# rsinghlab/GNN-Tumor-Seg

Hardware: AMD Instinct MI355X
Metric: supervoxel-graphs/sec training, 7xSAGE-pool-256, 15k-node graphs (higher is better)
Workload: dtype f32; 1 GPU; C2: 7xGraphSAGE-pool-256 (8 SAGEConv), fwd+weighted-CE+bwd+AdamW, 4 x 15000-node/86350-edge lattice graphs per GPU, 4-chan feat, fp32; global_batch=4, nodes_per_batch=60000, edges_per_batch=345400, parallelism=dp1

## Files before the change

### gnn-tumor-seg_amd/csrc/gts_gemm.hip

```cpp
#include "gts_gemm_tiles.h"
#include "gts_gemm_panel.h"
#include "gts_gemm_wgrad.h"
#include "gts_gemm_small.h"

namespace gts {
namespace {

template <bool AKC, bool BKC>
int pick_plain_variant(const GemmArgs& p) {
  int variant = BKC ? g_fwd_variant : g_igrad_variant;
  if (p.rb <= 128 && variant < 9) return 0;
  const bool row_count_invariant = variant == -2;
  if (variant < 0) {
    const int64_t cols = (p.rb + 255) / 256;
    const int64_t big_tiles = static_cast<int64_t>((p.ra + 255) / 256) * cols;
    variant = big_tiles >= 192 ? 8 : 3;
    if constexpr (AKC && BKC) {
      const int h = panel_rows_for(p.ra, cols);
      const int64_t panels = static_cast<int64_t>((p.ra + h - 1) / h) * cols;
      const int64_t rows256 = (big_tiles + 255) / 256 * 256, rows_panel = (panels + 255) / 256 * h;
      if (variant == 8 && rows_panel < rows256 && !row_count_invariant) variant = 10;
      if (variant == 3 && panels >= 192 && panels <= 256 && !row_count_invariant) variant = 10;
    }
  }
  return variant;
}

template <bool BKC>
inline bool skinny_forward(const GemmArgs& p) {
  const bool automatic = BKC ? g_fwd_variant < 0 : g_igrad_variant <= 1;
  return automatic && (p.rb == 4 || p.rb == 8) && p.ldc == p.rb && p.kseg[0] + p.kseg[1] >= 64 && p.mask == nullptr &&
         p.c2 == nullptr && p.sc_l == nullptr && p.bits_out == nullptr &&
         (BKC || (p.ldb[0] == p.rb && (p.kseg[1] == 0 || p.ldb[1] == p.rb)));
}

inline bool tiny_forward(const GemmArgs& p) {
  return (p.rb == 4 || p.rb == 8) && p.ldc == p.rb && p.kseg[0] + p.kseg[1] <= 16 && p.mask == nullptr && p.c2 == nullptr &&
         p.sc_l == nullptr && p.bits_out == nullptr && g_fwd_variant < 0;
}

template <bool AKC, bool BKC>
int launch_plain_tiles(const GemmArgs& p, int variant, hipStream_t st) {
  if constexpr (AKC && BKC) {
    if (tiny_forward(p)) {
      const unsigned blocks = static_cast<unsigned>((p.ra + 255) / 256);
      if (p.rb == 4) tiny_fwd_kernel<4><<<blocks, 256, 0, st>>>(p);
      else tiny_fwd_kernel<8><<<blocks, 256, 0, st>>>(p);
      return launch_status();
    }
  }
  if constexpr (AKC) {
    if (skinny_forward<BKC>(p)) {
      const unsigned blocks = static_cast<unsigned>((p.ra + 15) / 16);
      if (p.rb == 4) skinny_fwd_kernel<4, BKC><<<blocks, 256, 0, st>>>(p);
      else skinny_fwd_kernel<8, BKC><<<blocks, 256, 0, st>>>(p);
      return launch_status();
    }
  }
  if (p.rb <= 64) return launch_tiles<128, 64, 2, 2, AKC, BKC>(p, 1, 1, st);
  if (p.rb <= 128) return launch_tiles<128, 128, 2, 2, AKC, BKC>(p, 1, 1, st);
  switch (variant) {
    case 3: return launch_tiles<64, 256, 2, 4, AKC, BKC>(p, 1, 1, st);
    case 5: return launch_tiles<256, 128, 4, 2, AKC, BKC>(p, 1, 1, st);
    case 8: return launch_tiles<256, 256, 4, 4, AKC, BKC, true>(p, 1, 1, st);
    default: return launch_tiles<128, 256, 2, 4, AKC, BKC>(p, 1, 1, st);
  }
}

template <bool AKC, bool BKC>
int launch_plain(const GemmArgs& p, hipStream_t st) {
  const int variant = pick_plain_variant<AKC, BKC>(p);
  if constexpr (AKC && BKC) {
    if (p.c2 != nullptr && !(variant == 10 && p.rb <= kC240 && p.rb2 <= kC240 && p.rb2 > 128)) {
      GemmArgs first = p, next{};
      first.c2 = nullptr;
      int rc = launch_plain<true, true>(first, st);
      if (rc != GTS_OK) return rc;
      next.a[0] = next.a[1] = p.c, next.b[0] = next.b[1] = p.b2, next.bp[0] = p.bp2;
      first.bp2 = nullptr;
      next.lda[0] = next.lda[1] = p.ldc, next.ldb[0] = next.ldb[1] = p.ldb2;
      next.kseg[0] = p.rb, next.kseg[1] = 0;
      next.ra = p.ra, next.rb = p.rb2, next.c = p.c2, next.ldc = p.ldc2, next.bias = p.bias2, next.relu = p.relu2;
      next.tiles_per_split = (p.rb + kBK - 1) / kBK;
      return launch_plain<true, true>(next, st);
    }
    if (variant == 10) {
      switch (panel_rows_for(p.ra, (p.rb + kC240 - 1) / kC240)) {
        case 144: return launch_panel_direct<3, 4, 1, NoProbe, 144>(p, st);
        case 192: return launch_panel_direct<3, 4, 1, NoProbe, 192>(p, st);
        default: return launch_panel_direct<3, 4, 1>(p, st);
      }
    }
  }
  int rc = launch_plain_tiles<AKC, BKC>(p, variant, st);
  if (rc != GTS_OK || p.bits_out == nullptr) return rc;
  const long long words = static_cast<long long>((p.ra + 3) / 4) * (p.rb >> 6);
  relu_bits_kernel<<<static_cast<unsigned>((words + 3) / 4), 256, 0, st>>>(p.c, p.bits_out, p.ra, p.rb);
  return launch_status();
}

struct PlainProblem {
  const float *a0, *b0, *a1, *b1;
  float* c;
  int64_t m, rb, k0, k1;
  bool missing() const { return !a0 || !b0 || !c || ((a1 == nullptr) != (b1 == nullptr)); }
  bool bad_shape() const {
    return m < 0 || rb <= 0 || k0 <= 0 || k1 < 0 || m >= (1LL << 31) || rb >= (1 << 20) || k0 >= (1 << 20) || k1 >= (1 << 20) ||
           !aligned4(k0) || !aligned4(k1) || (a1 && k1 == 0);
  }
  GemmArgs args(int64_t ldb0, int64_t ldb1, const float* const* packed) const {
    GemmArgs p{};
    p.a[0] = a0, p.b[0] = b0, p.lda[0] = p.kseg[0] = static_cast<int>(k0), p.ldb[0] = static_cast<int>(ldb0);
    p.a[1] = a1 ? a1 : a0, p.b[1] = b1 ? b1 : b0, p.lda[1] = static_cast<int>(k1), p.ldb[1] = static_cast<int>(ldb1);
    p.kseg[1] = a1 ? static_cast<int>(k1) : 0;
    p.ra = static_cast<int>(m), p.rb = static_cast<int>(rb), p.c = c, p.ldc = static_cast<int>(rb);
    p.tiles_per_split = (p.kseg[0] + kBK - 1) / kBK + (p.kseg[1] + kBK - 1) / kBK;
    if (packed != nullptr) p.bp[0] = packed[0], p.bp[1] = a1 ? packed[1] : nullptr;
    return p;
  }
};

void chain_second(GemmArgs* p, const float* b2, const float* bias2, float* c2, int64_t rb2, int relu2,
                  const float* const* packed) {
  p->b2 = b2, p->bias2 = bias2, p->c2 = c2, p->rb2 = static_cast<int>(rb2), p->ldb2 = p->rb;
  p->ldc2 = static_cast<int>(rb2), p->relu2 = relu2;
  if (packed != nullptr) p->bp2 = packed[2];
}

__global__ __launch_bounds__(kBlock) void sum_parts_kernel(const float* __restrict__ in_l, const float* __restrict__ in_r,
                                                           float* __restrict__ out_l, float* __restrict__ out_r,
                                                           int64_t n, int parts) {
  const int64_t i = static_cast<int64_t>(blockIdx.x) * kBlock + threadIdx.x;
  if (i >= n) return;
  float sl = 0.f, sr = 0.f;
  for (int q = 0; q < parts; ++q) sl += in_l[i * parts + q], sr += in_r[i * parts + q];
  out_l[i] = sl, out_r[i] = sr;
}

}
}

extern "C" int32_t gts_linear_fwd_f32(const float* a0, const float* w0, const float* a1, const float* w1, const float* bias,
                                      float* out, int64_t m, int64_t n, int64_t k0, int64_t k1, int32_t relu,
                                      uint64_t* relu_bits, const float* const* packed, void* stream) {
  using namespace gts;
  const PlainProblem q{a0, w0, a1, w1, out, m, n, k0, k1};
  if (q.missing()) return GTS_ERR_NULL;
  if (q.bad_shape() || (relu_bits && n % 64 != 0)) return GTS_ERR_SHAPE;
  if (m == 0) return GTS_OK;
  GemmArgs p = q.args(k0, k1, packed);
  p.bias = bias, p.relu = relu, p.bits_out = reinterpret_cast<unsigned long long*>(relu_bits);
  return launch_plain<true, true>(p, static_cast<hipStream_t>(stream));
}

extern "C" int32_t gts_relu_bits_pay(int64_t m, int64_t n) {
  using namespace gts;
  if (m <= 0 || n <= 0 || n % 64 != 0 || m >= (1LL << 31) || n >= (1 << 20)) return 0;
  GemmArgs p{};
  p.ra = static_cast<int>(m), p.rb = static_cast<int>(n);
  const int variant = pick_plain_variant<true, true>(p);
  return variant >= 10 && variant <= 12 ? 1 : 0;
}

extern "C" int64_t gts_relu_bits_bytes(int64_t m, int64_t n) {
  if (m < 0 || n <= 0 || n % 64 != 0) return 0;
  return (m + 3) / 4 * (n / 64) * 4 * static_cast<int64_t>(sizeof(uint64_t));
}

extern "C" int64_t gts_gat_fc_scores_workspace(int64_t m, int64_t heads, int64_t dim) {
  if (m <= 0 || heads <= 0 || dim <= 0 || dim % 64 != 0) return 0;
  return 2 * m * heads * (dim / 64) * static_cast<int64_t>(sizeof(float));
}

extern "C" int32_t gts_gat_fc_scores_f32(const float* h, const float* w_fc, const float* attn_l, const float* attn_r,
                                         float* ft, float* el, float* er, float* workspace, int64_t workspace_bytes,
                                         int64_t m, int64_t heads, int64_t dim, int64_t k, const float* w_fc_packed,
                                         void* stream) {
  using namespace gts;
  const int64_t n = heads * dim;
  const float* const packed[2] = {w_fc_packed, nullptr};
  const PlainProblem q{h, w_fc, nullptr, nullptr, ft, m, n, k, 0};
  if (q.missing() || !attn_l || !attn_r || !el || !er) return GTS_ERR_NULL;
  if (q.bad_shape() || heads <= 0 || dim <= 0) return GTS_ERR_SHAPE;
  if (m == 0) return GTS_OK;
  GemmArgs p = q.args(k, 0, packed);
  hipStream_t st = static_cast<hipStream_t>(stream);
  const int parts = static_cast<int>(dim / 64);
  const bool fuse = dim % 64 == 0 && pick_plain_variant<true, true>(p) == 10 &&
                    (parts == 1 || (workspace && workspace_bytes >= gts_gat_fc_scores_workspace(m, heads, dim)));
  if (!fuse) {
    const int rc = launch_plain<true, true>(p, st);
    return rc != GTS_OK ? rc : gts_gat_scores_f32(ft, attn_l, attn_r, el, er, m, heads, dim, stream);
  }
  p.sc_l = attn_l, p.sc_r = attn_r;
  p.sc_el = parts == 1 ? el : workspace, p.sc_er = parts == 1 ? er : workspace + m * heads * parts;
  const int rc = launch_plain<true, true>(p, st);
  if (rc != GTS_OK || parts == 1) return rc;
  const int64_t rows = m * heads;
  sum_parts_kernel<<<static_cast<unsigned>((rows + kBlock - 1) / kBlock), kBlock, 0, st>>>(p.sc_el, p.sc_er, el, er, rows, parts);
  return launch_status();
}

extern "C" int32_t gts_linear_fwd_chain_f32(const float* a0, const float* w0, const float* a1, const float* w1,
                                            const float* bias, float* out, const float* w2, const float* bias2, float* out2,
                                            int64_t m, int64_t n, int64_t k0, int64_t k1, int32_t relu, int64_t n2,
                                            int32_t relu2, uint64_t* relu_bits, const float* const* packed, void* stream) {
  using namespace gts;
  const PlainProblem q{a0, w0, a1, w1, out, m, n, k0, k1};
  if (q.missing() || !w2 || !out2) return GTS_ERR_NULL;
  if (q.bad_shape() || n2 <= 0 || n2 >= (1 << 20) || !aligned4(n) || (relu_bits && n % 64 != 0)) return GTS_ERR_SHAPE;
  if (m == 0) return GTS_OK;
  GemmArgs p = q.args(k0, k1, packed);
  p.bias = bias, p.relu = relu, p.bits_out = reinterpret_cast<unsigned long long*>(relu_bits);
  chain_second(&p, w2, bias2, out2, n2, relu2, packed);
  return launch_plain<true, true>(p, static_cast<hipStream_t>(stream));
}

extern "C" int32_t gts_linear_bwd_input_chain_t_f32(const float* g0, const float* w0t, const float* g1, const float* w1t,
                                                    const float* relu_mask, const uint64_t* relu_bits, float* gin,
                                                    const float* w2t, float* gin2, int64_t m, int64_t k, int64_t n0,
                                                    int64_t n1, int64_t k2, const float* const* packed, void* stream) {
  using namespace gts;
  const PlainProblem q{g0, w0t, g1, w1t, gin, m, k, n0, n1};
  if (q.missing() || !w2t || !gin2 || (relu_bits && !relu_mask)) return GTS_ERR_NULL;
  if (q.bad_shape() || k2 <= 0 || k2 >= (1 << 20) || !aligned4(k) || (relu_bits && k % 64 != 0)) return GTS_ERR_SHAPE;
  if (m == 0) return GTS_OK;
  GemmArgs p = q.args(n0, n1, packed);
  p.mask = relu_mask, p.bits_in = reinterpret_cast<const unsigned long long*>(relu_bits);
  chain_second(&p, w2t, nullptr, gin2, k2, 0, packed);
  return launch_plain<true, true>(p, static_cast<hipStream_t>(stream));
}

extern "C" int32_t gts_linear_bwd_input_f32(const float* g0, const float* w0, const float* g1, const float* w1,
                                            const float* relu_mask, float* gin, int64_t m, int64_t k, int64_t n0,
                                            int64_t n1, void* stream) {
  using namespace gts;
  const PlainProblem q{g0, w0, g1, w1, gin, m, k, n0, n1};
  if (q.missing()) return GTS_ERR_NULL;
  if (q.bad_shape() || !aligned4(k)) return GTS_ERR_SHAPE;
  if (m == 0) return GTS_OK;
  GemmArgs p = q.args(k, k, nullptr);
  p.mask = relu_mask;
  return launch_plain<true, false>(p, static_cast<hipStream_t>(stream));
}

extern "C" int32_t gts_linear_bwd_input_t_f32(const float* g0, const float* w0t, const float* g1, const float* w1t,
                                              const float* relu_mask, const uint64_t* relu_bits, float* gin, int64_t m,
                                              int64_t k, int64_t n0, int64_t n1, const float* const* packed, void* stream) {
  using namespace gts;
  const PlainProblem q{g0, w0t, g1, w1t, gin, m, k, n0, n1};
  if (q.missing() || (relu_bits && !relu_mask)) return GTS_ERR_NULL;
  if (q.bad_shape() || !aligned4(k) || (relu_bits && k % 64 != 0)) return GTS_ERR_SHAPE;
  if (m == 0) return GTS_OK;
  GemmArgs p = q.args(n0, n1, packed);
  p.mask = relu_mask, p.bits_in = reinterpret_cast<const unsigned long long*>(relu_bits);
  return launch_plain<true, true>(p, static_cast<hipStream_t>(stream));
}

static bool act_fold_in_epilogue(const gts::GemmArgs& p) {
  return gts::pick_plain_variant<true, true>(p) == 10 && p.rb % gts::kC240 == 0;
}

extern "C" int64_t gts_linear_bwd_input_t_act_workspace(int64_t m, int64_t k) {
  if (m <= 0 || k <= 0) return 0;
  const int64_t row_blocks = (m + 143) / 144 * 3;
  const int64_t pass = gts_gat_reduce_workspace(m, k) / 2;
  const int64_t fold = row_blocks * k * static_cast<int64_t>(sizeof(float));
  return fold > pass ? fold : pass;
}

extern "C" int32_t gts_linear_bwd_input_t_act_f32(const float* g0, const float* w0t, const float* g1, const float* w1t,
                                                  const float* act_out, int32_t activation, float* gin, float* g_bias,
                                                  float* workspace, int64_t workspace_bytes, int64_t m, int64_t k,
                                                  int64_t n0, int64_t n1, const float* const* packed, void* stream) {
  using namespace gts;
  const PlainProblem q{g0, w0t, g1, w1t, gin, m, k, n0, n1};
  if (q.missing() || !act_out || (g_bias && !workspace)) return GTS_ERR_NULL;
  if (activation != 1 && activation != 2) return GTS_ERR_ARGKIND;
  if (q.bad_shape() || !aligned4(k)) return GTS_ERR_SHAPE;
  if (g_bias && workspace_bytes < gts_linear_bwd_input_t_act_workspace(m, k)) return GTS_ERR_SHAPE;
  if (m == 0) return GTS_OK;
  hipStream_t st = static_cast<hipStream_t>(stream);
  GemmArgs p = q.args(n0, n1, packed);
  if (activation == 1 && g_bias && act_fold_in_epilogue(p)) {
    const int rows = panel_rows_for(p.ra, p.rb / kC240);
    const int row_blocks = (p.ra + rows - 1) / rows * 3;
    p.mask = act_out, p.mask_kind = 1, p.col_partial = workspace;
    const int rc = launch_plain<true, true>(p, st);
    if (rc != GTS_OK) return rc;
    return sum_chunks(workspace, g_bias, p.rb, row_blocks, st);
  }
  const int rc = launch_plain<true, true>(p, st);
  if (rc != GTS_OK) return rc;
  return gts_gat_act_bwd_f32(gin, act_out, activation, gin, g_bias, workspace, workspace_bytes, m, k, stream);
}

extern "C" int64_t gts_linear_bwd_weight_workspace(int64_t m, int64_t n, int64_t k, int32_t n_problems) {
  using namespace gts;
  if (m <= 0 || n <= 0 || k <= 0 || n_problems < 1 || n_problems > kMaxProblems) return 0;
  const int64_t splits = wgrad_plan(m, n, k, n_problems).splits;
  const int64_t slabs = n_problems * splits * (n * k + n);
  const int64_t skinny = skinny_workspace_floats(m, n, k) + kSkinnyChunks * (n < k ? n : 0);
  return (slabs > skinny ? slabs : skinny) * static_cast<int64_t>(sizeof(float));
}

extern "C" int32_t gts_linear_bwd_weight_f32(const float* const* g, const float* const* a, float* const* gw,
                                             float* const* gb, int32_t n_problems, float* workspace,
                                             int64_t workspace_bytes, int64_t m, int64_t n, int64_t k, void* stream) {
  using namespace gts;
  if (!g || !a || !gw || !workspace) return GTS_ERR_NULL;
  if (n_problems < 1 || n_problems > kMaxProblems) return GTS_ERR_ARGKIND;
  if (m <= 0 || n <= 0 || k <= 0 || m >= (1LL << 31) || n >= (1 << 20) || k >= (1 << 20) || !aligned4(n) || !aligned4(k))
    return GTS_ERR_SHAPE;
  if (workspace_bytes < gts_linear_bwd_weight_workspace(m, n, k, n_problems)) return GTS_ERR_SHAPE;
  bool any_bias = false;
  for (int q = 0; q < n_problems; ++q) {
    if (!g[q] || !a[q] || !gw[q]) return GTS_ERR_NULL;
    any_bias = any_bias || (gb && gb[q]);
  }
  hipStream_t st = static_cast<hipStream_t>(stream);
  if (skinny_workspace_floats(m, n, k) > 0) {
    for (int q = 0; q < n_problems; ++q)
      skinny_wgrad(g[q], a[q], gw[q], gb ? gb[q] : nullptr, workspace, m, n, k, st);
    return launch_status();
  }
  const WgradPlan plan = wgrad_plan(m, n, k, n_problems);
  const int splits = plan.splits;
  const int tiles = static_cast<int>((m + kBK - 1) / kBK);
  GemmArgs p{};
  for (int q = 0; q < n_problems; ++q) p.pa[q] = g[q], p.pb[q] = a[q];
  p.a[0] = p.a[1] = g[0], p.b[0] = p.b[1] = a[0];
  p.lda[0] = p.lda[1] = static_cast<int>(n), p.ldb[0] = p.ldb[1] = static_cast<int>(k);
  p.kseg[0] = static_cast<int>(m), p.kseg[1] = 0;
  p.ra = static_cast<int>(n), p.rb = static_cast<int>(k);
  p.c = workspace, p.ldc = static_cast<int>(k);
  p.colsum = any_bias ? workspace + static_cast<size_t>(n_problems) * splits * n * k : nullptr;
  for (int q = 0; q < n_problems && any_bias; ++q)
    if (gb[q]) p.colsum_mask |= 1u << q;
  p.n_problems = n_problems, p.n_splits = splits;
  p.tiles_per_split = (tiles + splits - 1) / splits;
  int rc = launch_wgrad(p, plan, st);
  if (rc != GTS_OK) return rc;
  ReduceArgs r{};
  r.splits = splits;
  int jobs = 0;
  for (int q = 0; q < n_problems; ++q, ++jobs) {
    r.slabs[jobs] = workspace + static_cast<size_t>(q) * splits * n * k;
    r.out[jobs] = gw[q], r.n4[jobs] = static_cast<int>(n * k / 4);
  }
  for (int q = 0; q < n_problems && any_bias; ++q) {
    if (!gb[q]) continue;
    r.slabs[jobs] = p.colsum + static_cast<size_t>(q) * splits * n;
    r.out[jobs] = gb[q], r.n4[jobs] = static_cast<int>(n / 4);
    ++jobs;
  }
  reduce_slabs_kernel<<<dim3(static_cast<unsigned>((n * k / 4 + 63) / 64), jobs), kBlock, 0, st>>>(r);
  return launch_status();
}
```

### gnn-tumor-seg_amd/csrc/gts_gemm_wgrad.h

```cpp
#pragma once
#include <type_traits>

#include "gts_gemm_tiles.h"

namespace gts {
namespace {

typedef float v2f __attribute__((ext_vector_type(2)));

template <int O0, int O1>
__device__ __forceinline__ v2f lds_read2st64(unsigned addr) {
  static_assert(O0 >= 0 && O1 <= 255, "ds_read2st64_b32 offsets are 8 bits");
  v2f r;
  asm volatile("ds_read2st64_b32 %0, %1 offset0:%2 offset1:%3" : "=v"(r) : "v"(addr), "n"(O0), "n"(O1));
  return r;
}

template <class Probe = NoProbe>
__global__ __launch_bounds__(1024, 4) void wgrad_stream_kernel(const GemmArgs p) {
  constexpr int BM = 256, BN = 256, WM = 4, WN = 4, WTM = 64, WTN = 64, TM = 2, TN = 2;
  constexpr int kPlane = kBK * BM;
  static_assert(BM == BN && kPlane * 4 == 128 * 256, "image I of an operand sits 128 offset units above image 0");
  __shared__ float lds[4 * kPlane];
  const int lane = threadIdx.x & 63, wave = __builtin_amdgcn_readfirstlane(threadIdx.x >> 6);
  const int wm = wave / WN, wn = wave % WN;
  const int i = lane & 31, h = lane >> 5;
  const int problem = blockIdx.y / p.tiles_n, tile_n = blockIdx.y % p.tiles_n;
  const int m0 = blockIdx.x * BM, n0 = tile_n * BN;
  const float* g = kernarg_entry<const float*>(offsetof(GemmArgs, pa), problem);
  const float* act = kernarg_entry<const float*>(offsetof(GemmArgs, pb), problem);
  const int ldg = p.lda[0], lda = p.ldb[0];
  const int n_tiles_all = (p.kseg[0] + kBK - 1) / kBK;
  const int t_beg = min(n_tiles_all, static_cast<int>(blockIdx.z) * p.tiles_per_split);
  const int t_end = min(n_tiles_all, t_beg + p.tiles_per_split);
  const int row_beg = t_beg * kBK, rows = min(p.kseg[0], t_end * kBK) - row_beg;
  const int n_tiles = t_end - t_beg;
  const bool g_ok = m0 + 4 * lane < p.ra, a_ok = n0 + 4 * lane < p.rb;
  const unsigned vg0 = g_ok ? static_cast<unsigned>(wave * ldg + m0 + 4 * lane) * 4 : kOutOfRange;
  const unsigned vg1 = g_ok ? static_cast<unsigned>((wave + 16) * ldg + m0 + 4 * lane) * 4 : kOutOfRange;
  const unsigned va0 = a_ok ? static_cast<unsigned>(wave * lda + n0 + 4 * lane) * 4 : kOutOfRange;
  const unsigned va1 = a_ok ? static_cast<unsigned>((wave + 16) * lda + n0 + 4 * lane) * 4 : kOutOfRange;
  auto dma = [&](int t, int image) __attribute__((always_inline)) {
    const int r0 = row_beg + t * kBK, nr = min(kBK, rows - t * kBK);
    __amdgpu_buffer_rsrc_t rg = __builtin_amdgcn_make_buffer_rsrc(const_cast<float*>(g + static_cast<size_t>(r0) * ldg), 0,
                                                                  nr * ldg * 4, 0x00020000);
    __amdgpu_buffer_rsrc_t ract = __builtin_amdgcn_make_buffer_rsrc(const_cast<float*>(act + static_cast<size_t>(r0) * lda), 0,
                                                                    nr * lda * 4, 0x00020000);
    float* ia = lds + image * kPlane + wave * BM;
    float* ib = lds + (2 + image) * kPlane + wave * BN;
    __builtin_amdgcn_raw_ptr_buffer_load_lds(rg, ia, 16, vg0, 0, 0, 0);
    __builtin_amdgcn_raw_ptr_buffer_load_lds(rg, ia + 16 * BM, 16, vg1, 0, 0, 0);
    __builtin_amdgcn_raw_ptr_buffer_load_lds(ract, ib, 16, va0, 0, 0, 0);
    __builtin_amdgcn_raw_ptr_buffer_load_lds(ract, ib + 16 * BN, 16, va1, 0, 0, 0);
  };

  v16f acc[TM][TN];
#pragma unroll
  for (int tm = 0; tm < TM; ++tm)
#pragma unroll
    for (int tn = 0; tn < TN; ++tn)
#pragma unroll
      for (int r = 0; r < 16; ++r) acc[tm][tn][r] = 0.f;
  float csum[TM] = {0.f, 0.f};
  const bool want_colsum = p.colsum != nullptr && tile_n == 0 && wn == wm && ((p.colsum_mask >> problem) & 1u) != 0;

  const unsigned lds0 = static_cast<unsigned>(reinterpret_cast<uintptr_t>((__attribute__((address_space(3))) float*)lds));
  const unsigned a_addr0 = lds0 + static_cast<unsigned>(4 * h * BM + wm * WTM + i) * 4, a_addr1 = a_addr0 + 128;
  const unsigned b_addr0 = lds0 + static_cast<unsigned>(2 * kPlane + 4 * h * BN + wn * WTN + i) * 4, b_addr1 = b_addr0 + 128;
  v2f fa[2][TM], fb[2][TN];
  fa[0][0] = fa[0][1] = fa[1][0] = fa[1][1] = v2f{0.f, 0.f};
  fb[0][0] = fb[0][1] = fb[1][0] = fb[1][1] = v2f{0.f, 0.f};

  auto issue = [&](auto img_c, auto pair_c) __attribute__((always_inline)) {
    constexpr int IMG = decltype(img_c)::value, Q = decltype(pair_c)::value;
    constexpr int O = 4 * (8 * (Q / 2) + 2 * (Q % 2)) + 128 * IMG;
    fa[Q & 1][0] = lds_read2st64<O, O + 4>(a_addr0);
    fa[Q & 1][1] = lds_read2st64<O, O + 4>(a_addr1);
    fb[Q & 1][0] = lds_read2st64<O, O + 4>(b_addr0);
    fb[Q & 1][1] = lds_read2st64<O, O + 4>(b_addr1);
  };
  auto multiply = [&](int slot) __attribute__((always_inline)) {
#pragma unroll
    for (int e = 0; e < 2; ++e)
#pragma unroll
      for (int tm = 0; tm < TM; ++tm)
#pragma unroll
        for (int tn = 0; tn < TN; ++tn)
          acc[tm][tn] = __builtin_amdgcn_mfma_f32_32x32x2f32(fa[slot][tm][e], fb[slot][tn][e], acc[tm][tn], 0, 0, 0);
  };
  float half_sum[TM] = {0.f, 0.f};
  auto tile = [&](auto img_c, auto cs_c, int t) __attribute__((always_inline)) {
    constexpr int IMG = decltype(img_c)::value;
    constexpr bool CS = decltype(cs_c)::value;
    auto pair = [&](auto pair_c) __attribute__((always_inline)) {
      constexpr int Q = decltype(pair_c)::value, S = Q & 1;
      if constexpr (Q < 7) {
        issue(img_c, std::integral_constant<int, Q + 1>{});
        asm volatile("s_waitcnt lgkmcnt(4)" : "+v"(fa[S][0]), "+v"(fa[S][1]), "+v"(fb[S][0]), "+v"(fb[S][1]));
      } else {
        asm volatile("s_waitcnt vmcnt(0) lgkmcnt(0)\n\ts_barrier"
                     : "+v"(fa[S][0]), "+v"(fa[S][1]), "+v"(fb[S][0]), "+v"(fb[S][1]) : : "memory");
        if (t + 2 < n_tiles) dma(t + 2, IMG);
        if (t + 1 < n_tiles) issue(std::integral_constant<int, IMG ^ 1>{}, std::integral_constant<int, 0>{});
      }
      if constexpr (Q % 2 == 0) {
        if constexpr (Q == 0) __builtin_amdgcn_s_setprio(3);
        else if constexpr (Q == 2) __builtin_amdgcn_s_setprio(2);
        else if constexpr (Q == 4) __builtin_amdgcn_s_setprio(1);
        else __builtin_amdgcn_s_setprio(0);
      }
      if constexpr (CS) {
#pragma unroll
        for (int tm = 0; tm < TM; ++tm) {
          if constexpr (Q % 2 == 0) {
            asm volatile("v_add_f32 %0, %1, %2" : "=v"(half_sum[tm]) : "v"(fa[S][tm][0]), "v"(fa[S][tm][1]));
          } else {
            float upper;
            asm volatile("v_add_f32 %0, %1, %2" : "=v"(upper) : "v"(fa[S][tm][0]), "v"(fa[S][tm][1]));
            asm volatile("v_add_f32 %0, %1, %2" : "=v"(upper) : "v"(half_sum[tm]), "v"(upper));
            asm volatile("v_add_f32 %0, %1, %2" : "+v"(csum[tm]) : "v"(csum[tm]), "v"(upper));
          }
        }
      }
      multiply(S);
    };
    pair(std::integral_constant<int, 0>{}), pair(std::integral_constant<int, 1>{}), pair(std::integral_constant<int, 2>{}),
        pair(std::integral_constant<int, 3>{}), pair(std::integral_constant<int, 4>{}), pair(std::integral_constant<int, 5>{}),
        pair(std::integral_constant<int, 6>{}), pair(std::integral_constant<int, 7>{});
  };
  auto reduce = [&](auto cs_c) __attribute__((always_inline)) {
    int t = 0;
    for (; t + 1 < n_tiles; t += 2) {
      tile(std::integral_constant<int, 0>{}, cs_c, t);
      tile(std::integral_constant<int, 1>{}, cs_c, t + 1);
    }
    if (t < n_tiles) tile(std::integral_constant<int, 0>{}, cs_c, t);
  };

  Probe::mark(0);
  if (n_tiles > 0) {
    dma(0, 0);
    if (n_tiles > 1) dma(1, 1);
    asm volatile("s_waitcnt vmcnt(0)\n\ts_barrier" ::: "memory");
    issue(std::integral_constant<int, 0>{}, std::integral_constant<int, 0>{});
  }
  Probe::mark(1);
  if (want_colsum) reduce(std::true_type{});
  else reduce(std::false_type{});
  __builtin_amdgcn_s_setprio(0);
  Probe::mark(2);
  const size_t slab = static_cast<size_t>(problem) * p.n_splits + blockIdx.z;
  write_tile<BM, BN, WM, WN>(p, lds, p.c + slab * p.ra * p.ldc, acc, m0, n0);
  Probe::mark(3);
  if (want_colsum) {
#pragma unroll
    for (int tm = 0; tm < TM; ++tm) {
      const float total = csum[tm] + __shfl_xor(csum[tm], 32, kWave);
      const int row = m0 + wm * WTM + tm * 32 + i;
      if (h == 0 && row < p.ra) p.colsum[slab * p.ra + row] = total;
    }
  }
}

struct ReduceArgs {
  const float* slabs[2 * kMaxProblems];
  float* out[2 * kMaxProblems];
  int n4[2 * kMaxProblems];
  int splits;
};

__global__ __launch_bounds__(kBlock) void reduce_slabs_kernel(const ReduceArgs p) {
  __shared__ v4f part[4][64];
  const int col = threadIdx.x & 63, grp = threadIdx.x >> 6;
  const int q = blockIdx.y;
  const float* slabs = kernarg_entry<const float*>(offsetof(ReduceArgs, slabs), q);
  float* out = kernarg_entry<float*>(offsetof(ReduceArgs, out), q);
  const int n4 = kernarg_entry<int>(offsetof(ReduceArgs, n4), q);
  const int i = blockIdx.x * 64 + col;
  if (blockIdx.x * 64 >= n4) return;
  v4f acc = {0.f, 0.f, 0.f, 0.f};
  if (i < n4) {
    const v4f* src = reinterpret_cast<const v4f*>(slabs) + i;
#pragma unroll 8
    for (int s = grp; s < p.splits; s += 4) acc += src[static_cast<size_t>(s) * n4];
  }
  part[grp][col] = acc;
  __syncthreads();
  if (grp == 0 && i < n4) {
    const v4f total = (part[0][col] + part[1][col]) + (part[2][col] + part[3][col]);
    reinterpret_cast<v4f*>(out)[i] = total;
  }
}

constexpr int kSkinnyMax = 9;
constexpr int kSkinnyChunks = 512;

template <int S>
__global__ __launch_bounds__(kBlock) void skinny_wgrad_kernel(const float* __restrict__ skinny, int s_cols,
                                                             const float* __restrict__ wide,
                                                             float* __restrict__ partial, int64_t m,
                                                             int w, int64_t rows_per_chunk) {
  __shared__ v4f red[kBlock];
  const int cols4 = w >> 2;
  const int lanes = cols4 >= kBlock ? 1 : kBlock / cols4;
  const int rl = cols4 >= kBlock ? 0 : threadIdx.x / cols4;
  const int64_t row0 = blockIdx.x * rows_per_chunk, row1 = min(m, row0 + rows_per_chunk);
  for (int q0 = 0; q0 < cols4; q0 += kBlock) {
    const int q = q0 + (cols4 >= kBlock ? threadIdx.x : threadIdx.x % cols4);
    const bool live = q < cols4 && rl < lanes;
    v4f acc[S];
#pragma unroll
    for (int i = 0; i < S; ++i) acc[i] = v4f{0.f, 0.f, 0.f, 0.f};
    if (live) {
#pragma unroll 4
      for (int64_t row = row0 + rl; row < row1; row += lanes) {
        const v4f f = *reinterpret_cast<const v4f*>(wide + static_cast<size_t>(row) * w + 4 * q);
#pragma unroll
        for (int i = 0; i < S; ++i) acc[i] += (i < s_cols ? skinny[row * s_cols + i] : 1.0f) * f;
      }
    }
#pragma unroll
    for (int i = 0; i < S; ++i) {
      v4f total = acc[i];
      if (lanes > 1) {
        __syncthreads();
        red[threadIdx.x] = acc[i];
        __syncthreads();
        if (rl == 0 && live) {
          for (int l = 1; l < lanes; ++l) total += red[l * cols4 + q];
        }
      }
      if (rl == 0 && live)
        *reinterpret_cast<v4f*>(partial + (static_cast<size_t>(blockIdx.x) * S + i) * w + 4 * q) = total;
    }
  }
}

__global__ __launch_bounds__(kBlock) void skinny_sum_kernel(const float* __restrict__ partial,
                                                           float* __restrict__ dst0,
                                                           float* __restrict__ dst1, int rows, int s_cols,
                                                           int w, int chunks, int transposed) {
  __shared__ float part[16][16];
  const int o = threadIdx.x & 15, lane = threadIdx.x >> 4;
  const int idx = blockIdx.x * 16 + o;
  const int total_out = rows * w;
  float acc = 0.f;
  if (idx < total_out) {
#pragma unroll 8
    for (int c = lane; c < chunks; c += 16) acc += partial[static_cast<size_t>(c) * total_out + idx];
  }
  part[lane][o] = acc;
  __syncthreads();
  if (lane != 0 || idx >= total_out) return;
  float sum = part[0][o];
#pragma unroll
  for (int l = 1; l < 16; ++l) sum += part[l][o];
  const int i = idx / w, j = idx - i * w;
  if (i < s_cols)
    dst0[transposed ? j * s_cols + i : i * w + j] = sum;
  else if (dst1 != nullptr)
    dst1[j] = sum;
}

inline int64_t skinny_workspace_floats(int64_t m, int64_t n, int64_t k) {
  const int64_t small = n < k ? n : k, big = n < k ? k : n;
  if (small + 1 > kSkinnyMax || big < 64) return 0;
  return static_cast<int64_t>(kSkinnyChunks) * (small + 1) * big;
}

template <int S>
void launch_skinny(const float* skinny, int s_cols, const float* wide, float* partial, int64_t m, int w,
                   int chunks, int64_t rpc, hipStream_t st) {
  skinny_wgrad_kernel<S><<<chunks, kBlock, 0, st>>>(skinny, s_cols, wide, partial, m, w, rpc);
}

inline bool skinny_wgrad(const float* g, const float* a, float* gw, float* gb, float* workspace, int64_t m,
                  int64_t n, int64_t k, hipStream_t st) {
  if (skinny_workspace_floats(m, n, k) == 0) return false;
  const bool g_is_skinny = n < k;
  const float* skinny = g_is_skinny ? g : a;
  const float* wide = g_is_skinny ? a : g;
  const int s_cols = static_cast<int>(g_is_skinny ? n : k), w = static_cast<int>(g_is_skinny ? k : n);
  const bool ones_row = !g_is_skinny && gb != nullptr;
  const int rows = s_cols + (ones_row ? 1 : 0);
  const int64_t rpc = (m + kSkinnyChunks - 1) / kSkinnyChunks;
  const int chunks = static_cast<int>((m + rpc - 1) / rpc);
  switch (rows) {
    case 1: launch_skinny<1>(skinny, s_cols, wide, workspace, m, w, chunks, rpc, st); break;
    case 2: launch_skinny<2>(skinny, s_cols, wide, workspace, m, w, chunks, rpc, st); break;
    case 3: launch_skinny<3>(skinny, s_cols, wide, workspace, m, w, chunks, rpc, st); break;
    case 4: launch_skinny<4>(skinny, s_cols, wide, workspace, m, w, chunks, rpc, st); break;
    case 5: launch_skinny<5>(skinny, s_cols, wide, workspace, m, w, chunks, rpc, st); break;
    case 6: launch_skinny<6>(skinny, s_cols, wide, workspace, m, w, chunks, rpc, st); break;
    case 7: launch_skinny<7>(skinny, s_cols, wide, workspace, m, w, chunks, rpc, st); break;
    case 8: launch_skinny<8>(skinny, s_cols, wide, workspace, m, w, chunks, rpc, st); break;
    default: launch_skinny<9>(skinny, s_cols, wide, workspace, m, w, chunks, rpc, st); break;
  }
  skinny_sum_kernel<<<(rows * w + 15) / 16, kBlock, 0, st>>>(
      workspace, gw, ones_row ? gb : nullptr, rows, s_cols, w, chunks, g_is_skinny ? 0 : 1);
  if (g_is_skinny && gb != nullptr) {
    float* part = workspace + static_cast<size_t>(chunks) * rows * w;
    skinny_wgrad_kernel<1><<<chunks, kBlock, 0, st>>>(nullptr, 0, g, part, m, static_cast<int>(n), rpc);
    skinny_sum_kernel<<<(static_cast<int>(n) + 15) / 16, kBlock, 0, st>>>(
        part, nullptr, gb, 1, 0, static_cast<int>(n), chunks, 0);
  }
  return true;
}

struct WgradPlan {
  int variant, bm, bn, splits;
};

inline void wgrad_candidate(int variant, int64_t k, int* bm, int* bn, int64_t* slots) {
  *bm = 128, *bn = k <= 64 ? 64 : 128, *slots = 512;
  if (k <= 64) return;
  if (variant == 2) *bn = 256;
  if (variant == 4 || variant == 6) *bm = 256, *bn = 256, *slots = 256;
}

inline WgradPlan wgrad_plan(int64_t m, int64_t n, int64_t k, int n_problems) {
  const int64_t tiles = (m + kBK - 1) / kBK;
  static const int kMany[2] = {6, 2};
  static const int kFewLarge[2] = {6, 1};
  const bool few = n_problems <= 4;
  const bool large = n * k * n_problems >= (1 << 20);
  const int n_candidates = g_wgrad_variant >= 0 || (few && !large) ? 1 : 2;
  WgradPlan best{};
  double best_fill = -1.0;
  for (int c = 0; c < n_candidates; ++c) {
    WgradPlan plan{};
    plan.variant = g_wgrad_variant >= 0 ? g_wgrad_variant : (few ? (large ? kFewLarge[c] : 1) : kMany[c]);
    int64_t slots;
    wgrad_candidate(plan.variant, k, &plan.bm, &plan.bn, &slots);
    const int64_t out_tiles = ((n + plan.bm - 1) / plan.bm) * ((k + plan.bn - 1) / plan.bn) * n_problems;
    int64_t splits = out_tiles >= slots ? 1 : slots / out_tiles;
    if (splits > tiles) splits = tiles;
    plan.splits = static_cast<int>(splits < 1 ? 1 : splits);
    const int64_t groups = out_tiles * plan.splits;
    const int64_t rounds = (groups + slots - 1) / slots;
    const double fill = static_cast<double>(groups) / static_cast<double>(rounds * slots);
    if (fill > best_fill + 1e-9) best = plan, best_fill = fill;
  }
  return best;
}

inline int launch_wgrad(const GemmArgs& p, const WgradPlan& plan, hipStream_t st) {
  const int np = p.n_problems, splits = plan.splits;
  if (p.rb <= 64) return launch_tiles<128, 64, 2, 2, false, false>(p, np, splits, st);
  switch (plan.variant) {
    case 2: return launch_tiles<128, 256, 2, 4, false, false>(p, np, splits, st);
    case 4: return launch_tiles<256, 256, 4, 4, false, false, true>(p, np, splits, st);
    case 6: {
      GemmArgs q = p;
      q.tiles_n = (p.rb + 255) / 256;
      dim3 grid((p.ra + 255) / 256, q.tiles_n * np, splits);
      wgrad_stream_kernel<><<<grid, 1024, 0, st>>>(q);
      return launch_status();
    }
    default: return launch_tiles<128, 128, 2, 4, false, false>(p, np, splits, st);
  }
}

}
}
```

### gnn-tumor-seg_amd/csrc/gts_project.hip

```cpp
#include "gts_rows.h"

namespace gts {
namespace {

template <typename RowT>
__device__ __forceinline__ void store_row(RowT* dst, const RowT& v, int nt) {
  if (!nt) {
    *dst = v;
    return;
  }
  if constexpr (sizeof(RowT) == 16) {
    typedef unsigned u4 __attribute__((ext_vector_type(4)));
    __builtin_nontemporal_store(*reinterpret_cast<const u4*>(&v), reinterpret_cast<u4*>(dst));
  } else if constexpr (sizeof(RowT) == 8) {
    typedef unsigned u2 __attribute__((ext_vector_type(2)));
    __builtin_nontemporal_store(*reinterpret_cast<const u2*>(&v), reinterpret_cast<u2*>(dst));
  } else {
    __builtin_nontemporal_store(v, dst);
  }
}

constexpr int kVoxPerLane = 8;
constexpr int kVoxPerWave = kWave * kVoxPerLane;
constexpr int kVoxPerBlock = kVoxPerWave * kWavesPerBlock;

__device__ __forceinline__ int resolve_row(int id, int n_rows) {
  const int r = id < 0 ? id + n_rows + 1 : id;
  return (r < 0 || r > n_rows) ? n_rows : r;
}

__device__ __forceinline__ void load_tile_ids(const int16_t* __restrict__ svs, int64_t tile_base,
                                              int64_t n_vox, int16_t* lds_wave,
                                              int (&ids)[kVoxPerLane]) {
  const int lane = threadIdx.x & (kWave - 1);
  const int64_t mine = tile_base + static_cast<int64_t>(lane) * kVoxPerLane;
  if (mine + kVoxPerLane <= n_vox && (reinterpret_cast<uintptr_t>(svs + mine) & 15) == 0) {
    *reinterpret_cast<uint4*>(lds_wave + lane * kVoxPerLane) =
        *reinterpret_cast<const uint4*>(svs + mine);
  } else {
#pragma unroll
    for (int j = 0; j < kVoxPerLane; ++j)
      lds_wave[lane * kVoxPerLane + j] = mine + j < n_vox ? svs[mine + j] : int16_t(-1);
  }
  __builtin_amdgcn_wave_barrier();
  __builtin_amdgcn_s_waitcnt(0xC07F);
#pragma unroll
  for (int j = 0; j < kVoxPerLane; ++j) ids[j] = lds_wave[j * kWave + lane];
  __builtin_amdgcn_wave_barrier();
}

template <typename RowT>
__global__ __launch_bounds__(kBlock) void project_rows_kernel(
    const int16_t* __restrict__ svs, const RowT* __restrict__ table,
    const RowT* __restrict__ bg_row, RowT* __restrict__ out, int64_t n_vox, int n_rows, int nt) {
  __shared__ int16_t lds[kVoxPerBlock];
  const int lane = threadIdx.x & (kWave - 1);
  const int wave = threadIdx.x / kWave;
  int16_t* lds_wave = lds + wave * kVoxPerWave;
  const RowT bg = *bg_row;
  const int64_t n_tiles = (n_vox + kVoxPerWave - 1) / kVoxPerWave;
  for (int64_t tile = static_cast<int64_t>(blockIdx.x) * kWavesPerBlock + wave; tile < n_tiles;
       tile += static_cast<int64_t>(gridDim.x) * kWavesPerBlock) {
    const int64_t base = tile * kVoxPerWave;
    int ids[kVoxPerLane];
    load_tile_ids(svs, base, n_vox, lds_wave, ids);
    RowT rows[kVoxPerLane];
#pragma unroll
    for (int j = 0; j < kVoxPerLane; ++j) {
      const int r = resolve_row(ids[j], n_rows);
      rows[j] = r == n_rows ? bg : table[r];
    }
#pragma unroll
    for (int j = 0; j < kVoxPerLane; ++j) {
      const int64_t i = base + j * kWave + lane;
      if (i < n_vox) store_row(out + i, rows[j], nt);
    }
  }
}

__device__ __forceinline__ void store_tile_labels(int16_t* __restrict__ out, int64_t tile_base,
                                                  int64_t n_vox, int16_t* lds_wave,
                                                  const int (&labels)[kVoxPerLane]) {
  const int lane = threadIdx.x & (kWave - 1);
  const int64_t mine = tile_base + static_cast<int64_t>(lane) * kVoxPerLane;
  const bool wide = tile_base + kVoxPerWave <= n_vox &&
                    (reinterpret_cast<uintptr_t>(out + tile_base) & 15) == 0;
  if (wide) {
#pragma unroll
    for (int j = 0; j < kVoxPerLane; ++j) lds_wave[j * kWave + lane] = static_cast<int16_t>(labels[j]);
    __builtin_amdgcn_wave_barrier();
    __builtin_amdgcn_s_waitcnt(0xC07F);
    *reinterpret_cast<uint4*>(out + mine) = *reinterpret_cast<const uint4*>(lds_wave + lane * kVoxPerLane);
    __builtin_amdgcn_wave_barrier();
  } else {
#pragma unroll
    for (int j = 0; j < kVoxPerLane; ++j) {
      const int64_t i = tile_base + j * kWave + lane;
      if (i < n_vox) out[i] = static_cast<int16_t>(labels[j]);
    }
  }
}

template <int CLASSES>
__global__ __launch_bounds__(kBlock) void project_argmax_kernel(
    const int16_t* __restrict__ svs, const float* __restrict__ logits,
    const int16_t* __restrict__ relabel, int16_t* __restrict__ out, int64_t n_vox, int n_rows,
    int n_classes, uint8_t* __restrict__ occ, int dim_x, int dim_y, int dim_z) {
  __shared__ int16_t lds[kVoxPerBlock];
  const int lane = threadIdx.x & (kWave - 1);
  const int wave = threadIdx.x / kWave;
  int16_t* lds_wave = lds + wave * kVoxPerWave;
  const int64_t n_tiles = (n_vox + kVoxPerWave - 1) / kVoxPerWave;
  for (int64_t tile = static_cast<int64_t>(blockIdx.x) * kWavesPerBlock + wave; tile < n_tiles;
       tile += static_cast<int64_t>(gridDim.x) * kWavesPerBlock) {
    const int64_t base = tile * kVoxPerWave;
    int ids[kVoxPerLane];
    load_tile_ids(svs, base, n_vox, lds_wave, ids);
    int labels[kVoxPerLane];
#pragma unroll
    for (int j = 0; j < kVoxPerLane; ++j) {
      const int r = resolve_row(ids[j], n_rows);
      int label = 0;
      if (r != n_rows) {
        if constexpr (CLASSES == 4) {
          const float4 row = reinterpret_cast<const float4*>(logits)[r];
          float best = row.x;
          if (best < row.y) best = row.y, label = 1;
          if (best < row.z) best = row.z, label = 2;
          if (best < row.w) label = 3;
        } else {
          const float* row = logits + static_cast<size_t>(r) * n_classes;
          float best = row[0];
          for (int c = 1; c < n_classes; ++c) {
            const float val = row[c];
            if (best < val) best = val, label = c;
          }
        }
      }
      if (occ != nullptr && label != 0) {
        const unsigned i = static_cast<unsigned>(base) + j * kWave + lane;
        if (i < n_vox) {
          const unsigned plane = i / static_cast<unsigned>(dim_z);
          occ[plane / static_cast<unsigned>(dim_y)] = 1;
          occ[dim_x + plane % static_cast<unsigned>(dim_y)] = 1;
          occ[dim_x + dim_y + i % static_cast<unsigned>(dim_z)] = 1;
        }
      }
      labels[j] = relabel != nullptr ? relabel[label] : label;
    }
    store_tile_labels(out, base, n_vox, lds_wave, labels);
  }
}

inline unsigned stream_grid(int64_t n_vox) {
  const int64_t blocks = (n_vox + kVoxPerBlock - 1) / kVoxPerBlock;
  return static_cast<unsigned>(blocks < 4096 ? (blocks > 0 ? blocks : 1) : 4096);
}

inline void launch_project_argmax(const int16_t* svs, const float* logits, const int16_t* relabel,
                                  int16_t* out, int64_t n_vox, int n_rows, int n_classes,
                                  uint8_t* occ, int dx, int dy, int dz, hipStream_t st) {
  const unsigned grid = stream_grid(n_vox);
  if (n_classes == 4 && (reinterpret_cast<uintptr_t>(logits) & 15) == 0)
    project_argmax_kernel<4><<<grid, kBlock, 0, st>>>(svs, logits, relabel, out, n_vox, n_rows, 4,
                                                      occ, dx, dy, dz);
  else
    project_argmax_kernel<0><<<grid, kBlock, 0, st>>>(svs, logits, relabel, out, n_vox, n_rows,
                                                      n_classes, occ, dx, dy, dz);
}

}
}

extern "C" int32_t gts_abi_version(void) { return 33; }

extern "C" const char* gts_error_string(int32_t code) {
  switch (code) {
    case GTS_OK: return "ok";
    case GTS_ERR_NULL: return "gts: required pointer is NULL";
    case GTS_ERR_SHAPE: return "gts: unsupported or inconsistent shape";
    case GTS_ERR_ARGKIND: return "gts: unsupported arg_bytes/row_bytes/mode";
    default: return code > 0 ? hipGetErrorString(static_cast<hipError_t>(code)) : "gts: unknown error";
  }
}

extern "C" int32_t gts_project_rows_i16(const int16_t* svs, const void* table,
                                        const void* bg_row, void* out, int64_t n_vox,
                                        int64_t n_rows, int32_t row_bytes, void* stream) {
  using namespace gts;
  if (!svs || !bg_row || !out || (n_rows > 0 && !table)) return GTS_ERR_NULL;
  if (n_vox < 0 || n_rows < 0 || n_rows > 32768) return GTS_ERR_SHAPE;
  if (n_vox == 0) return GTS_OK;
  hipStream_t st = static_cast<hipStream_t>(stream);
  const unsigned grid = stream_grid(n_vox);
  const int nr = static_cast<int>(n_rows);
  switch (row_bytes) {
    case 4:
      project_rows_kernel<uint32_t><<<grid, kBlock, 0, st>>>(
          svs, static_cast<const uint32_t*>(table), static_cast<const uint32_t*>(bg_row),
          static_cast<uint32_t*>(out), n_vox, nr, g_project_nt);
      break;
    case 8:
      project_rows_kernel<uint2><<<grid, kBlock, 0, st>>>(
          svs, static_cast<const uint2*>(table), static_cast<const uint2*>(bg_row),
          static_cast<uint2*>(out), n_vox, nr, g_project_nt);
      break;
    case 16:
      project_rows_kernel<uint4><<<grid, kBlock, 0, st>>>(
          svs, static_cast<const uint4*>(table), static_cast<const uint4*>(bg_row),
          static_cast<uint4*>(out), n_vox, nr, g_project_nt);
      break;
    default:
      return GTS_ERR_ARGKIND;
  }
  return launch_status();
}

extern "C" int32_t gts_project_argmax_i16(const int16_t* svs, const float* logits,
                                          const int16_t* relabel, int16_t* out, int64_t n_vox,
                                          int64_t n_rows, int64_t n_classes, void* stream) {
  using namespace gts;
  if (!svs || !out || (n_rows > 0 && !logits)) return GTS_ERR_NULL;
  if (n_vox < 0 || n_rows < 0 || n_rows > 32768 || n_classes < 1 || n_classes > 1024)
    return GTS_ERR_SHAPE;
  if (n_vox == 0) return GTS_OK;
  launch_project_argmax(svs, logits, relabel, out, n_vox, static_cast<int>(n_rows),
                        static_cast<int>(n_classes), nullptr, 1, 1, 1,
                        static_cast<hipStream_t>(stream));
  return launch_status();
}

extern "C" int32_t gts_project_argmax_occupancy_i16(const int16_t* svs, const float* logits,
                                                    int16_t* out, uint8_t* occupancy,
                                                    int64_t dim_x, int64_t dim_y, int64_t dim_z,
                                                    int64_t n_rows, int64_t n_classes,
                                                    void* stream) {
  using namespace gts;
  if (!svs || !out || !occupancy || (n_rows > 0 && !logits)) return GTS_ERR_NULL;
  if (dim_x < 0 || dim_y < 0 || dim_z < 0 || dim_x > 32768 || dim_y > 32768 || dim_z > 32768 ||
      n_rows < 0 || n_rows > 32768 || n_classes < 1 || n_classes > 1024)
    return GTS_ERR_SHAPE;
  const int64_t n_vox = dim_x * dim_y * dim_z;
  if (n_vox >= (1LL << 31)) return GTS_ERR_SHAPE;
  if (n_vox == 0) return GTS_OK;
  launch_project_argmax(svs, logits, nullptr, out, n_vox, static_cast<int>(n_rows),
                        static_cast<int>(n_classes), occupancy, static_cast<int>(dim_x),
                        static_cast<int>(dim_y), static_cast<int>(dim_z),
                        static_cast<hipStream_t>(stream));
  return launch_status();
}
```

### gnn-tumor-seg_amd/csrc/gts_stack.hip

```cpp
#include <algorithm>
#include <vector>

#include "gts_gemm_args.h"

namespace {

constexpr int kMaxLayers = 64;

inline int64_t align256(int64_t bytes) { return (bytes + 255) & ~255LL; }

inline bool bad_stack(int64_t n_rows, const int64_t* widths, int32_t n_layers) {
  if (!widths || n_layers < 1 || n_layers > kMaxLayers || n_rows < 0 || n_rows >= (1LL << 31)) return true;
  for (int i = 0; i <= n_layers; ++i)
    if (widths[i] <= 0 || widths[i] % 4 != 0 || widths[i] >= (1 << 20)) return true;
  return false;
}

struct FwdPlan {
  int64_t m[kMaxLayers], arg[kMaxLayers], out[kMaxLayers], bits[kMaxLayers];
  int64_t p[2];
  int64_t wp[kMaxLayers][3];
  int64_t counters;
  int64_t total;
};

inline bool packs(int64_t out_cols) { return out_cols > 128; }

inline FwdPlan plan_forward(int64_t n, const int64_t* w, int n_layers, bool training, int arg_bytes, bool relu_bits) {
  FwdPlan p{};
  int64_t at = 0, widest = 0;
  auto take = [&](int64_t bytes) { const int64_t o = at; at += align256(bytes); return o; };
  for (int i = 0; i < n_layers; ++i) {
    const bool last = i == n_layers - 1;
    widest = std::max(widest, w[i]);
    p.m[i] = take(4 * n * w[i]);
    p.arg[i] = training ? take(static_cast<int64_t>(arg_bytes) * n * w[i]) : -1;
    p.out[i] = take(4 * n * w[i + 1]);
    const bool bits = relu_bits && training && !last && gts_relu_bits_pay(n, w[i + 1]) == 1;
    p.bits[i] = bits ? take(gts_relu_bits_bytes(n, w[i + 1])) : -1;
  }
  p.p[0] = take(4 * n * widest);
  p.p[1] = take(4 * n * widest);
  for (int i = 0; i < n_layers; ++i) {
    p.wp[i][0] = packs(w[i]) ? take(4 * gts_packed_weight_floats(w[i], w[i])) : -1;
    p.wp[i][1] = packs(w[i + 1]) ? take(4 * gts_packed_weight_floats(w[i + 1], w[i])) : -1;
    p.wp[i][2] = packs(w[i + 1]) ? take(4 * gts_packed_weight_floats(w[i + 1], w[i])) : -1;
  }
  p.counters = take(4 * GTS_CLUSTER_COUNTER_WORDS);
  p.total = at;
  return p;
}

inline bool chainable(int64_t n, int64_t k0, int64_t k1, int64_t n2) {
  return n % 4 == 0 && k0 % 4 == 0 && k1 % 4 == 0 && n <= 256 && n2 <= 256;
}

inline bool turns(int64_t rows, int64_t cols) { return cols >= 128 && rows % 4 == 0 && cols % 4 == 0; }

struct BwdPlan {
  int64_t wt[kMaxLayers][3];
  int64_t wtp[kMaxLayers][3];
  int64_t g[kMaxLayers], gp[kMaxLayers];
  int64_t gm[2];
  int64_t workspace, workspace_bytes;
  int64_t counters;
  int64_t total;
};

struct ByShape {
  struct Group {
    int64_t rows, cols;
    std::vector<const float*> in[2];
    std::vector<float*> out[2];
    int count() const { return static_cast<int>(in[0].size()); }
  };
  std::vector<Group> groups;
  void add(int64_t rows, int64_t cols, const float* in0, const float* in1, float* out0, float* out1) {
    auto it = std::find_if(groups.begin(), groups.end(), [&](const Group& c) { return c.rows == rows && c.cols == cols; });
    if (it == groups.end()) it = groups.insert(it, Group{rows, cols, {}, {}});
    it->in[0].push_back(in0), it->in[1].push_back(in1), it->out[0].push_back(out0), it->out[1].push_back(out1);
  }
};

constexpr int kWeightSlot[3] = {0, 2, 3};
inline int64_t weight_rows(const int64_t* w, int i, int q) { return q == 0 ? w[i] : w[i + 1]; }

inline BwdPlan plan_backward(int64_t n, const int64_t* w, int n_layers) {
  BwdPlan p{};
  int64_t at = 0, widest = 0;
  auto take = [&](int64_t bytes) { const int64_t o = at; at += align256(bytes); return o; };
  ByShape wgrads;
  for (int i = 0; i < n_layers; ++i) {
    const int64_t fin = w[i];
    widest = std::max(widest, fin);
    for (int q = 0; q < 3; ++q) p.wt[i][q] = turns(weight_rows(w, i, q), fin) ? take(4 * weight_rows(w, i, q) * fin) : -1;
    for (int q = 0; q < 3; ++q)
      p.wtp[i][q] = p.wt[i][q] >= 0 ? take(4 * gts_packed_weight_floats(fin, weight_rows(w, i, q))) : -1;
    p.g[i] = i > 0 ? take(4 * n * fin) : -1;
    p.gp[i] = take(4 * n * fin);
    for (int q = 0; q < 3; ++q) wgrads.add(weight_rows(w, i, q), fin, nullptr, nullptr, nullptr, nullptr);
  }
  p.gm[0] = take(4 * n * widest);
  p.gm[1] = take(4 * n * widest);
  int64_t ws = 0;
  if (n > 0)
    for (const auto& grp : wgrads.groups)
      for (int first = 0; first < grp.count(); first += gts::kMaxProblems)
        ws = std::max(ws, gts_linear_bwd_weight_workspace(n, grp.rows, grp.cols, std::min(gts::kMaxProblems, grp.count() - first)));
  p.workspace_bytes = ws;
  p.workspace = take(ws);
  p.counters = take(4 * GTS_CLUSTER_COUNTER_WORDS);
  p.total = at;
  return p;
}

inline int32_t zero_counters(const int32_t* sched_rec, int64_t clusters, int32_t rows, int32_t srcs, int32_t loc_words,
                             int32_t backward, void* at, void* stream, uint32_t** counters) {
  *counters = nullptr;
  if (sched_rec == nullptr || gts_cluster_uses_counters(clusters, rows, srcs, loc_words, backward) == 0) return GTS_OK;
  if (hipMemsetAsync(at, 0, 4 * GTS_CLUSTER_COUNTER_WORDS, static_cast<hipStream_t>(stream)) != hipSuccess) return gts::launch_status();
  *counters = static_cast<uint32_t*>(at);
  return GTS_OK;
}

#define GTS_TRY(call)                    \
  do {                                   \
    const int32_t code_ = (call);        \
    if (code_ != GTS_OK) return code_;   \
  } while (0)

}

extern "C" int64_t gts_sage_pool_stack_fwd_arena(int64_t n_rows, const int64_t* widths, int32_t n_layers, int32_t training,
                                                 int32_t arg_bytes, int32_t relu_bits, int64_t* offsets) {
  if (bad_stack(n_rows, widths, n_layers) || (training && arg_bytes != 1 && arg_bytes != 4)) return -1;
  const FwdPlan p = plan_forward(n_rows, widths, n_layers, training != 0, arg_bytes, relu_bits != 0);
  if (offsets != nullptr) {
    for (int i = 0; i < n_layers; ++i)
      offsets[4 * i] = p.m[i], offsets[4 * i + 1] = p.arg[i], offsets[4 * i + 2] = p.out[i], offsets[4 * i + 3] = p.bits[i];
    offsets[4 * n_layers] = p.p[0], offsets[4 * n_layers + 1] = p.p[1];
  }
  return p.total;
}

extern "C" int32_t gts_sage_pool_stack_fwd_f32(const int32_t* indptr, const int32_t* indices, const int32_t* sched_rec,
                                               int64_t sched_clusters, int32_t sched_rows, int32_t sched_srcs,
                                               int32_t sched_loc_words, const float* x, const float* const* params,
                                               int64_t n_rows, const int64_t* widths, int32_t n_layers, int32_t training,
                                               int32_t arg_bytes, int32_t relu_bits, void* arena, int64_t arena_bytes,
                                               void* stream) {
  if (!indptr || !x || !params || !arena) return GTS_ERR_NULL;
  if (bad_stack(n_rows, widths, n_layers)) return GTS_ERR_SHAPE;
  if (training && arg_bytes != 1 && arg_bytes != 4) return GTS_ERR_ARGKIND;
  for (int i = 0; i < 5 * n_layers; ++i)
    if (!params[i]) return GTS_ERR_NULL;
  const bool train = training != 0;
  const FwdPlan plan = plan_forward(n_rows, widths, n_layers, train, arg_bytes, relu_bits != 0);
  if (arena_bytes < plan.total) return GTS_ERR_SHAPE;
  if (n_rows == 0) return GTS_OK;
  char* base = static_cast<char*>(arena);
  auto f32 = [&](int64_t off) { return reinterpret_cast<float*>(base + off); };
  uint32_t* counters;
  GTS_TRY(zero_counters(sched_rec, sched_clusters, sched_rows, sched_srcs, sched_loc_words, 0, base + plan.counters, stream, &counters));
  {
    ByShape packs;
    for (int i = 0; i < n_layers; ++i)
      for (int q = 0; q < 3; ++q)
        if (plan.wp[i][q] >= 0)
          packs.add(weight_rows(widths, i, q), widths[i], params[5 * i + kWeightSlot[q]], nullptr, f32(plan.wp[i][q]), nullptr);
    for (const auto& b : packs.groups)
      GTS_TRY(gts_pack_weights_f32(b.in[0].data(), b.out[0].data(), nullptr, b.count(), b.rows, b.cols, 0, stream));
  }
  auto wp = [&](int i, int q) -> const float* { return plan.wp[i][q] >= 0 ? f32(plan.wp[i][q]) : nullptr; };
  const float* h = x;
  float* p = nullptr;
  int cur = 0;
  for (int i = 0; i < n_layers; ++i) {
    const float* w_pool = params[5 * i];
    const float* b_pool = params[5 * i + 1];
    const float* w_self = params[5 * i + 2];
    const float* w_neigh = params[5 * i + 3];
    const float* bias = params[5 * i + 4];
    const int64_t fin = widths[i], fout = widths[i + 1];
    const bool last = i == n_layers - 1;
    if (p == nullptr) {
      p = f32(plan.p[cur]);
      const float* packed[2] = {wp(i, 0), nullptr};
      GTS_TRY(gts_linear_fwd_f32(h, w_pool, nullptr, nullptr, b_pool, p, n_rows, fin, fin, 0, 1, nullptr, packed, stream));
    }
    float* m = f32(plan.m[i]);
    void* arg = train ? static_cast<void*>(base + plan.arg[i]) : nullptr;
    const int ab = train ? arg_bytes : 0;
    if (sched_rec != nullptr && fin == 256 && ab != 4 && n_rows * 1024 < (1LL << 32)) {
      GTS_TRY(gts_spmm_max_fwd_cluster_f32(sched_rec, sched_clusters, sched_rows, sched_srcs, sched_loc_words, p, m, arg, ab,
                                           1, n_rows, fin, counters, stream));
    } else {
      GTS_TRY(gts_spmm_max_fwd_f32(indptr, indices, p, m, arg, ab, 1, n_rows, fin, stream));
    }
    uint64_t* bits = plan.bits[i] >= 0 ? reinterpret_cast<uint64_t*>(base + plan.bits[i]) : nullptr;
    float* out = f32(plan.out[i]);
    if (!last && chainable(fout, fin, fin, fout)) {
      float* p_next = f32(plan.p[cur ^ 1]);
      const float* packed[3] = {wp(i, 1), wp(i, 2), wp(i + 1, 0)};
      GTS_TRY(gts_linear_fwd_chain_f32(h, w_self, m, w_neigh, bias, out, params[5 * (i + 1)], params[5 * (i + 1) + 1], p_next,
                                       n_rows, fout, fin, fin, 1, fout, 1, bits, packed, stream));
      p = p_next, cur ^= 1;
    } else {
      const float* packed[2] = {wp(i, 1), wp(i, 2)};
      GTS_TRY(gts_linear_fwd_f32(h, w_self, m, w_neigh, bias, out, n_rows, fout, fin, fin, last ? 0 : 1, bits, packed, stream));
      p = nullptr;
    }
    h = out;
  }
  return GTS_OK;
}

extern "C" int64_t gts_sage_pool_stack_bwd_scratch(int64_t n_rows, const int64_t* widths, int32_t n_layers,
                                                   int32_t ) {
  if (bad_stack(n_rows, widths, n_layers)) return -1;
  return plan_backward(n_rows, widths, n_layers).total;
}

extern "C" int32_t gts_sage_pool_stack_bwd_f32(const int32_t* t_indptr, const int32_t* t_indices, const int32_t* t_slot,
                                               const int32_t* sched_rec, int64_t sched_clusters, int32_t sched_rows,
                                               int32_t sched_srcs, int32_t sched_loc_words, const float* gout, const float* x,
                                               const float* const* params, int64_t n_rows, const int64_t* widths,
                                               int32_t n_layers, int32_t arg_bytes, int32_t relu_bits, const void* fwd_arena,
                                               float* const* grads, float* gx, void* scratch, int64_t scratch_bytes,
                                               void* stream) {
  if (!t_indptr || !gout || !x || !params || !fwd_arena || !grads || !scratch) return GTS_ERR_NULL;
  if (bad_stack(n_rows, widths, n_layers)) return GTS_ERR_SHAPE;
  if (arg_bytes != 1 && arg_bytes != 4) return GTS_ERR_ARGKIND;
  for (int i = 0; i < 5 * n_layers; ++i)
    if (!params[i] || !grads[i]) return GTS_ERR_NULL;
  hipStream_t st = static_cast<hipStream_t>(stream);
  if (n_rows == 0) {
    for (int i = 0; i < n_layers; ++i) {
      const int64_t fin = widths[i], fout = widths[i + 1];
      const int64_t sizes[5] = {fin * fin, fin, fout * fin, fout * fin, fout};
      for (int q = 0; q < 5; ++q)
        if (hipMemsetAsync(grads[5 * i + q], 0, 4 * sizes[q], st) != hipSuccess) return gts::launch_status();
    }
    return GTS_OK;
  }
  const FwdPlan fwd = plan_forward(n_rows, widths, n_layers, true, arg_bytes, relu_bits != 0);
  const BwdPlan plan = plan_backward(n_rows, widths, n_layers);
  if (scratch_bytes < plan.total) return GTS_ERR_SHAPE;
  const char* acts = static_cast<const char*>(fwd_arena);
  char* base = static_cast<char*>(scratch);
  auto f32 = [&](int64_t off) { return reinterpret_cast<float*>(base + off); };
  uint32_t* counters;
  GTS_TRY(zero_counters(sched_rec, sched_clusters, sched_rows, sched_srcs, sched_loc_words, 1, base + plan.counters, stream, &counters));
  auto act = [&](int64_t off) { return reinterpret_cast<const float*>(acts + off); };
  auto input_of = [&](int i) { return i == 0 ? x : act(fwd.out[i - 1]); };

  {
    ByShape turned;
    for (int i = 0; i < n_layers; ++i)
      for (int q = 0; q < 3; ++q)
        if (plan.wt[i][q] >= 0)
          turned.add(weight_rows(widths, i, q), widths[i], params[5 * i + kWeightSlot[q]], nullptr, f32(plan.wt[i][q]),
                     f32(plan.wtp[i][q]));
    for (const auto& b : turned.groups)
      GTS_TRY(gts_pack_weights_f32(b.in[0].data(), b.out[1].data(), b.out[0].data(), b.count(), b.rows, b.cols, 1, stream));
  }
  auto wt = [&](int i, int q) -> const float* { return plan.wt[i][q] >= 0 ? f32(plan.wt[i][q]) : nullptr; };
  auto wtp = [&](int i, int q) -> const float* { return plan.wtp[i][q] >= 0 ? f32(plan.wtp[i][q]) : nullptr; };

  auto igrad = [&](const float* g0, const float* w0, const float* w0t, int64_t n0, const float* g1, const float* w1,
                   const float* w1t, int64_t n1, const float* relu_mask, const uint64_t* relu_bits, float* gin,
                   int64_t k, const float* w0tp, const float* w1tp) -> int32_t {
    if (w0t != nullptr && (g1 == nullptr || w1t != nullptr)) {
      const float* packed[2] = {w0tp, g1 ? w1tp : nullptr};
      return gts_linear_bwd_input_t_f32(g0, w0t, g1, g1 ? w1t : nullptr, relu_mask, relu_mask ? relu_bits : nullptr, gin,
                                        n_rows, k, n0, g1 ? n1 : 0, packed, stream);
    }
    return gts_linear_bwd_input_f32(g0, w0, g1, g1 ? w1 : nullptr, relu_mask, gin, n_rows, k, n0, g1 ? n1 : 0, stream);
  };

  ByShape wgrads;

  const float* g = gout;
  const float* gm = nullptr;
  int cur = 0;
  for (int i = n_layers - 1; i >= 0; --i) {
    const float* w_pool = params[5 * i];
    const float* w_self = params[5 * i + 2];
    const float* w_neigh = params[5 * i + 3];
    const int64_t fin = widths[i], fout = widths[i + 1];
    const float* h = input_of(i);
    const float* m = act(fwd.m[i]);
    const void* arg = acts + fwd.arg[i];
    if (gm == nullptr) {
      float* buf = f32(plan.gm[cur]);
      GTS_TRY(igrad(g, w_neigh, wt(i, 2), fout, nullptr, nullptr, nullptr, 0, nullptr, nullptr, buf, fin, wtp(i, 2), nullptr));
      gm = buf;
    }
    float* gp = f32(plan.gp[i]);
    if (sched_rec != nullptr && fin == 256 && arg_bytes == 1 && n_rows * 1024 < (1LL << 32)) {
      GTS_TRY(gts_spmm_max_bwd_cluster_f32(sched_rec, sched_clusters, sched_rows, sched_srcs, sched_loc_words, gm, arg, 1, gp,
                                           n_rows, fin, counters, stream));
    } else {
      GTS_TRY(gts_spmm_max_bwd_f32(t_indptr, t_indices, t_slot, gm, arg, arg_bytes, nullptr, gp, n_rows, fin, stream));
    }
    gm = nullptr;
    wgrads.add(fin, fin, gp, h, grads[5 * i], grads[5 * i + 1]);
    wgrads.add(fout, fin, g, h, grads[5 * i + 2], grads[5 * i + 4]);
    wgrads.add(fout, fin, g, m, grads[5 * i + 3], nullptr);
    if (i > 0) {
      const int64_t below_in = widths[i - 1];
      const uint64_t* hbits = fwd.bits[i - 1] >= 0 ? reinterpret_cast<const uint64_t*>(acts + fwd.bits[i - 1]) : nullptr;
      float* g_next = f32(plan.g[i]);
      const float* below_t = wt(i - 1, 2);
      if (wt(i, 1) && wt(i, 0) && below_t && chainable(fin, fout, fin, below_in)) {
        float* gm_next = f32(plan.gm[cur ^ 1]);
        const float* packed[3] = {wtp(i, 1), wtp(i, 0), wtp(i - 1, 2)};
        GTS_TRY(gts_linear_bwd_input_chain_t_f32(g, wt(i, 1), gp, wt(i, 0), h, hbits, g_next, below_t, gm_next, n_rows, fin,
                                                 fout, fin, below_in, packed, stream));
        gm = gm_next, cur ^= 1;
      } else {
        GTS_TRY(igrad(g, w_self, wt(i, 1), fout, gp, w_pool, wt(i, 0), fin, h, hbits, g_next, fin, wtp(i, 1), wtp(i, 0)));
      }
      g = g_next;
    } else if (gx != nullptr) {
      GTS_TRY(igrad(g, w_self, wt(i, 1), fout, gp, w_pool, wt(i, 0), fin, nullptr, nullptr, gx, fin, wtp(i, 1), wtp(i, 0)));
    }
  }
  for (const auto& grp : wgrads.groups)
    for (int first = 0; first < grp.count(); first += gts::kMaxProblems)
      GTS_TRY(gts_linear_bwd_weight_f32(grp.in[0].data() + first, grp.in[1].data() + first, grp.out[0].data() + first,
                                        grp.out[1].data() + first, std::min(gts::kMaxProblems, grp.count() - first),
                                        f32(plan.workspace), plan.workspace_bytes, n_rows, grp.rows, grp.cols, stream));
  return GTS_OK;
}
```

### gnn-tumor-seg_amd/gts/_lib.py

```python
import ctypes
import os
import re

_HERE = os.path.dirname(os.path.abspath(__file__))
LIB_PATH = os.environ.get("GTS_LIB_PATH") or os.path.join(_HERE, "libgts_hip.so")
HEADER_PATH = os.path.join(os.path.dirname(os.path.dirname(_HERE)), "include", "gts_hip.h")
ABI_VERSION = 33

_p = ctypes.c_void_p
_i32 = ctypes.c_int32
_i64 = ctypes.c_int64


class GtsError(RuntimeError):
    pass


_BY_VALUE = {"int32_t": ctypes.c_int32, "int64_t": ctypes.c_int64, "uint32_t": ctypes.c_uint32,
             "uint64_t": ctypes.c_uint64, "float": ctypes.c_float, "double": ctypes.c_double}
_DEFINE = re.compile(r"^[ \t]*#[ \t]*define[ \t]+(GTS_\w+)[ \t]+\(?[ \t]*(-?\d+)[ \t]*\)?[ \t]*$", re.M)
_STRUCT = re.compile(r"\btypedef\s+struct\b[^{;]*\{[^{}]*\}\s*\w+\s*;")
_PROTOTYPE = re.compile(r"(?P<ret>[\w\s*]+?)\b(?P<name>\w+)\s*\((?P<args>[^()]*)\)")


def _ctype(decl, statement, returned=False):
    words = decl.replace("*", " * ").split()
    if "*" in words:
        return ctypes.c_char_p if returned and words == ["const", "char", "*"] else _p
    words = [w for w in words if w != "const"]
    if returned and words == ["void"]:
        return None
    if not returned and len(words) > 1:
        words = words[:-1]
    if len(words) == 1 and words[0] in _BY_VALUE:
        return _BY_VALUE[words[0]]
    raise GtsError(f"gts_hip.h: cannot bind `{decl.strip()}` of `{statement}`: by value only "
                   f"{', '.join(_BY_VALUE)} are taken (a struct goes by pointer)")


def parse_header(text):
    text = re.sub(r"/\*.*?\*/", " ", text, flags=re.S)
    text = re.sub(r"//[^\n]*", " ", text)
    constants = {name: int(value) for name, value in _DEFINE.findall(text)}
    text = re.sub(r"^[ \t]*#[^\n]*$", " ", text, flags=re.M)
    text = _STRUCT.sub(" ", text)
    text = re.sub(r'\bextern\s+"C"\s*\{', " ", text)
    *statements, tail = text.split(";")
    if tail.strip() not in ("", "}"):
        raise GtsError(f"gts_hip.h: cannot parse `{' '.join(tail.split())}`")
    signatures = {}
    for statement in statements:
        statement = " ".join(statement.split())
        m = _PROTOTYPE.fullmatch(statement)
        if m is None:
            raise GtsError(f"gts_hip.h: cannot parse `{statement}`")
        params = [a.strip() for a in m["args"].split(",")]
        if params in ([""], ["void"]):
            params = []
        if "..." in params or "" in params or "[" in m["args"]:
            raise GtsError(f"gts_hip.h: cannot bind `{statement}`: variadic, array or empty parameter")
        signatures[m["name"]] = (_ctype(m["ret"], statement, returned=True), [_ctype(a, statement) for a in params])
    return signatures, constants


_parsed = {}


def _header(path):
    if path not in _parsed:
        with open(path) as f:
            _parsed[path] = parse_header(f.read())
    return _parsed[path]


def signatures(header_path=HEADER_PATH):
    return _header(header_path)[0]


def const(name):
    try:
        return _header(HEADER_PATH)[1][name]
    except KeyError:
        raise GtsError(f"gts_hip.h defines no integer constant {name}") from None


def declared_symbols(header_path=HEADER_PATH):
    return sorted(signatures(header_path))


COLLATE_MAX_SCHEDULES = const("GTS_COLLATE_MAX_SCHEDULES")


class CollateMember(ctypes.Structure):
    _fields_ = [("n_nodes", _i64), ("n_edges", _i64),
                ("indptr", _p), ("indices", _p), ("t_indptr", _p), ("t_indices", _p), ("t_slot", _p), ("t_pos", _p),
                ("features", _p), ("labels", _p), ("feat_bytes", _i32), ("label_bytes", _i32),
                ("sched_rec", _p * COLLATE_MAX_SCHEDULES), ("sched_clusters", _i64 * COLLATE_MAX_SCHEDULES),
                ("sched_loc_words", _i32 * COLLATE_MAX_SCHEDULES)]


class CollateKind(ctypes.Structure):
    _fields_ = [("max_rows", _i32), ("max_srcs", _i32), ("tagged", _i32), ("reserved", _i32)]


class CollatePlan(ctypes.Structure):
    _fields_ = [("total_bytes", _i64), ("n_nodes", _i64), ("n_edges", _i64), ("features", _i64), ("labels", _i64),
                ("csr", _i64 * 8), ("sched", _i64 * COLLATE_MAX_SCHEDULES),
                ("sched_clusters", _i64 * COLLATE_MAX_SCHEDULES), ("sched_loc_words", _i32 * COLLATE_MAX_SCHEDULES),
                ("sched_record_words", _i32 * COLLATE_MAX_SCHEDULES)]


_lib = None


def load():
    global _lib
    if _lib is not None:
        return _lib
    if not os.path.exists(LIB_PATH):
        raise GtsError(
            f"{LIB_PATH} is missing: build it with `python __graft_entry__.py` (hipcc, gfx950). "
            "The gts operators have no CPU or PyTorch fallback.")
    lib = ctypes.CDLL(LIB_PATH)
    for name, (restype, argtypes) in signatures().items():
        fn = getattr(lib, name)
        fn.argtypes, fn.restype = argtypes, restype
    if lib.gts_abi_version() != ABI_VERSION:
        raise GtsError(f"libgts_hip.so ABI {lib.gts_abi_version()} != expected {ABI_VERSION}: rebuild")
    for pair in filter(None, os.environ.get("GTS_OPTIONS", "").split(",")):
        opt, val = pair.split("=")
        if lib.gts_set_option(int(opt), int(val)) != 0:
            raise GtsError(f"GTS_OPTIONS: unknown option {opt}")
    _lib = lib
    return lib


def check(code, what):
    if code != 0:
        msg = load().gts_error_string(code)
        raise GtsError(f"{what} failed with code {code}: {msg.decode() if msg else '?'}")


def require_device(*tensors):
    dev = None
    for t in tensors:
        if t is None:
            continue
        if not t.is_cuda:
            raise GtsError("gts operators run on MI355X only: got a CPU tensor "
                           "(there is no CPU fallback; use the oracle in tests)")
        if not t.is_contiguous():
            raise GtsError("gts operators need contiguous tensors")
        if dev is None:
            dev = t.device
        elif t.device != dev:
            raise GtsError(f"tensors on different devices: {dev} vs {t.device}")
    return dev


def ptr(t):
    return None if t is None else t.data_ptr()


def current_stream():
    import torch

    return torch.cuda.current_stream().cuda_stream
```

### gnn-tumor-seg_amd/gts/dense.py

```python
import torch
import torch.nn.functional as F

from . import _lib
from ._lib import check, current_stream, ptr, require_device
from ._operands import StreamBuffers, f32

GEMM_TIMER = None
_OPT_GEMM_TILE = _lib.const("GTS_OPT_GEMM_TILE")


class row_count_invariant:

    _depth = 0
    _saved = -1
    _lock = __import__("threading").Lock()

    def __enter__(self):
        with row_count_invariant._lock:
            if row_count_invariant._depth == 0:
                lib = _lib.load()
                row_count_invariant._saved = int(lib.gts_get_option(_OPT_GEMM_TILE))
                check(lib.gts_set_option(_OPT_GEMM_TILE, -2), "gts_set_option")
            row_count_invariant._depth += 1
        return self

    def __exit__(self, *exc):
        with row_count_invariant._lock:
            row_count_invariant._depth -= 1
            if row_count_invariant._depth == 0:
                check(_lib.load().gts_set_option(_OPT_GEMM_TILE, row_count_invariant._saved), "gts_set_option")
        return False


def _timed(kind, flops, launch):
    return GEMM_TIMER(kind, flops, launch) if GEMM_TIMER is not None else launch()


_gemm_ws = StreamBuffers()


def _pad4_cols(t):
    pad = (-t.shape[1]) % 4
    return t.contiguous() if pad == 0 else F.pad(t, (0, pad)).contiguous()


def _pad4_rows(t):
    pad = (-t.shape[0]) % 4
    return t.contiguous() if pad == 0 else F.pad(t, (0, 0, 0, pad)).contiguous()


def _mat(t, name):
    if t.dim() != 2:
        raise _lib.GtsError(f"{name} must be a matrix, got shape {tuple(t.shape)}")
    return t


def _same(a, b, what):
    if a != b:
        raise _lib.GtsError(f"shapes do not match: {what} ({a} vs {b})")


def _operands(*tensors):
    f32(*tensors)
    return require_device(*tensors)


def _dense(*tensors):
    return tuple(t if t is None or t.is_contiguous() else t.contiguous() for t in tensors)


def relu_bits_empty(m, n, device):
    nbytes = _lib.load().gts_relu_bits_bytes(m, n)
    if nbytes == 0 and m > 0:
        raise _lib.GtsError(f"relu bits need a width that is a multiple of 64, got {n}")
    return torch.empty(nbytes // 8, dtype=torch.int64, device=device)


def relu_bits_pay(m, n):
    return _lib.load().gts_relu_bits_pay(m, n) == 1


def _chk_bits(bits, m, n, what):
    if bits is None:
        return
    if bits.dtype != torch.int64 or not bits.is_contiguous() or bits.numel() * 8 != _lib.load().gts_relu_bits_bytes(m, n):
        raise _lib.GtsError(f"shapes do not match: {what} must come from relu_bits_empty({m}, {n})")


def unpack_relu_bits(bits, m, n):
    words = bits.view(n // 64, (m + 3) // 4, 4)
    lanes = torch.arange(64, device=bits.device, dtype=torch.int64)
    on = ((words.unsqueeze(-1) >> lanes) & 1).bool()
    on = on.view(n // 64, -1, 4, 4, 16).permute(1, 3, 0, 4, 2)
    return on.reshape(-1, n)[:m]


def _packed_array(packed, weights):
    import ctypes

    if packed is None or all(q is None for q in packed):
        return None
    if len(packed) != len(weights):
        raise _lib.GtsError(f"packed= takes one entry per weight operand ({len(weights)}), got {len(packed)}")
    for q, w in zip(packed, weights):
        if q is None:
            continue
        if w is None:
            raise _lib.GtsError("a fragment-order copy was passed for a weight operand that is absent")
        want = _lib.load().gts_packed_weight_floats(w.shape[0], w.shape[1])
        if q.dtype != torch.float32 or not q.is_contiguous() or q.numel() != want or q.device != w.device:
            raise _lib.GtsError(f"shapes do not match: fragment-order copy of a {tuple(w.shape)} operand holds {want} floats")
    return (ctypes.c_void_p * len(packed))(*[ptr(q) for q in packed])


def pack_weights(mats, transposed=False, want_plain=False):
    import ctypes

    if not mats:
        return ([], []) if want_plain else []
    rows, cols = mats[0].shape
    mats = [m.contiguous() for m in mats]
    dev = _operands(*mats)
    for m in mats:
        _same(tuple(m.shape), (rows, cols), "matrices of one pack batch")
    lib = _lib.load()
    n, k = (cols, rows) if transposed else (rows, cols)
    each = lib.gts_packed_weight_floats(n, k)
    out = torch.empty((len(mats), each), dtype=torch.float32, device=dev)
    plain = torch.empty((len(mats), cols, rows), dtype=torch.float32, device=dev) if (want_plain and transposed) else None
    arr = ctypes.c_void_p * len(mats)
    check(lib.gts_pack_weights_f32(arr(*[ptr(m) for m in mats]), arr(*[ptr(out[q]) for q in range(len(mats))]),
                                   arr(*[ptr(plain[q]) for q in range(len(mats))]) if plain is not None else None,
                                   len(mats), rows, cols, 1 if transposed else 0, current_stream()), "gts_pack_weights_f32")
    packed = list(out.unbind(0))
    return (list(plain.unbind(0)), packed) if plain is not None else packed


def linear_fwd(a0, w0, a1=None, w1=None, bias=None, relu=False, relu_bits=None, packed=None):
    _same(_mat(a0, "a0").shape[1], _mat(w0, "w0").shape[1], "inner dims of a0 @ w0^T")
    if (a1 is None) != (w1 is None):
        raise _lib.GtsError("a1 and w1 go together")
    if a1 is not None:
        _same(_mat(a1, "a1").shape[1], _mat(w1, "w1").shape[1], "inner dims of a1 @ w1^T")
        _same(a1.shape[0], a0.shape[0], "rows of a0 / a1")
        _same(w1.shape[0], w0.shape[0], "rows of w0 / w1")
    if bias is not None:
        _same(tuple(bias.shape), (w0.shape[0],), "bias vs output columns")
    a0, w0 = _pad4_cols(a0), _pad4_cols(w0)
    if a1 is not None:
        a1, w1 = _pad4_cols(a1), _pad4_cols(w1)
    dev = _operands(a0, w0, a1, w1, bias)
    m, n = a0.shape[0], w0.shape[0]
    _chk_bits(relu_bits, m, n, "relu_bits")
    out = torch.empty((m, n), dtype=torch.float32, device=dev)
    k0, k1 = a0.shape[1], a1.shape[1] if a1 is not None else 0
    bias = bias.contiguous() if bias is not None else None
    table = _packed_array(packed, (w0, w1))

    def launch():
        check(_lib.load().gts_linear_fwd_f32(ptr(a0), ptr(w0), ptr(a1), ptr(w1), ptr(bias), ptr(out),
                                             m, n, k0, k1, 1 if relu else 0, ptr(relu_bits), table, current_stream()),
              "gts_linear_fwd_f32")

    _timed("fwd", 2.0 * m * n * (k0 + k1), launch)
    return out


def linear_fwd_chain(a0, w0, a1, w1, bias, relu, w2, bias2, relu2, relu_bits=None, packed=None):
    _same(_mat(a0, "a0").shape[1], _mat(w0, "w0").shape[1], "inner dims of a0 @ w0^T")
    if (a1 is None) != (w1 is None):
        raise _lib.GtsError("a1 and w1 go together")
    if a1 is not None:
        _same(_mat(a1, "a1").shape[1], _mat(w1, "w1").shape[1], "inner dims of a1 @ w1^T")
        _same(a1.shape[0], a0.shape[0], "rows of a0 / a1")
        _same(w1.shape[0], w0.shape[0], "rows of w0 / w1")
    m, n, n2 = a0.shape[0], w0.shape[0], w2.shape[0]
    _same(_mat(w2, "w2").shape[1], n, "inner dims of out @ w2^T")
    if bias is not None:
        _same(tuple(bias.shape), (n,), "bias vs output columns")
    if bias2 is not None:
        _same(tuple(bias2.shape), (n2,), "bias2 vs output columns")
    k0, k1 = a0.shape[1], a1.shape[1] if a1 is not None else 0
    if n % 4 or k0 % 4 or k1 % 4:
        raise _lib.GtsError("linear_fwd_chain needs widths that are multiples of 4")
    a0, w0, a1, w1, bias, w2, bias2 = _dense(a0, w0, a1, w1, bias, w2, bias2)
    dev = _operands(a0, w0, a1, w1, bias, w2, bias2)
    _chk_bits(relu_bits, m, n, "relu_bits")
    out = torch.empty((m, n), dtype=torch.float32, device=dev)
    out2 = torch.empty((m, n2), dtype=torch.float32, device=dev)
    table = _packed_array(packed, (w0, w1, w2))
    _timed("fwd", 2.0 * m * n * (k0 + k1) + 2.0 * m * n2 * n, lambda: check(
        _lib.load().gts_linear_fwd_chain_f32(ptr(a0), ptr(w0), ptr(a1), ptr(w1), ptr(bias), ptr(out), ptr(w2),
                                             ptr(bias2), ptr(out2), m, n, k0, k1, 1 if relu else 0, n2,
                                             1 if relu2 else 0, ptr(relu_bits), table, current_stream()),
        "gts_linear_fwd_chain_f32"))
    return out, out2


def linear_bwd_input_chain_t(g0, w0t, g1, w1t, relu_mask, w2t, relu_bits=None, packed=None):
    _same(_mat(g0, "g0").shape[1], _mat(w0t, "w0t").shape[1], "inner dims of g0 @ w0t^T")
    if (g1 is None) != (w1t is None):
        raise _lib.GtsError("g1 and w1t go together")
    if g1 is not None:
        _same(_mat(g1, "g1").shape[1], _mat(w1t, "w1t").shape[1], "inner dims of g1 @ w1t^T")
        _same(g1.shape[0], g0.shape[0], "rows of g0 / g1")
        _same(w1t.shape[0], w0t.shape[0], "rows of w0t / w1t")
    m, k, k2 = g0.shape[0], w0t.shape[0], w2t.shape[0]
    _same(_mat(w2t, "w2t").shape[1], k, "inner dims of gin @ w2t^T")
    if relu_mask is not None:
        _same(tuple(relu_mask.shape), (m, k), "relu_mask vs result")
    n0, n1 = g0.shape[1], g1.shape[1] if g1 is not None else 0
    if k % 4 or n0 % 4 or n1 % 4:
        raise _lib.GtsError("linear_bwd_input_chain_t needs widths that are multiples of 4")
    g0, w0t, g1, w1t, relu_mask, w2t = _dense(g0, w0t, g1, w1t, relu_mask, w2t)
    dev = _operands(g0, w0t, g1, w1t, relu_mask, w2t)
    _chk_bits(relu_bits if relu_mask is not None else None, m, k, "relu_bits")
    relu_bits = relu_bits if relu_mask is not None else None
    gin = torch.empty((m, k), dtype=torch.float32, device=dev)
    gin2 = torch.empty((m, k2), dtype=torch.float32, device=dev)
    table = _packed_array(packed, (w0t, w1t, w2t))
    _timed("igrad", 2.0 * m * k * (n0 + n1) + 2.0 * m * k2 * k, lambda: check(
        _lib.load().gts_linear_bwd_input_chain_t_f32(ptr(g0), ptr(w0t), ptr(g1), ptr(w1t), ptr(relu_mask),
                                                     ptr(relu_bits), ptr(gin), ptr(w2t), ptr(gin2), m, k, n0, n1, k2,
                                                     table, current_stream()),
        "gts_linear_bwd_input_chain_t_f32"))
    return gin, gin2


def linear_bwd_input(g0, w0, g1=None, w1=None, relu_mask=None):
    _same(_mat(g0, "g0").shape[1], _mat(w0, "w0").shape[0], "inner dims of g0 @ w0")
    if (g1 is None) != (w1 is None):
        raise _lib.GtsError("g1 and w1 go together")
    if g1 is not None:
        _same(_mat(g1, "g1").shape[1], _mat(w1, "w1").shape[0], "inner dims of g1 @ w1")
        _same(g1.shape[0], g0.shape[0], "rows of g0 / g1")
        _same(w1.shape[1], w0.shape[1], "columns of w0 / w1")
    if relu_mask is not None:
        _same(tuple(relu_mask.shape), (g0.shape[0], w0.shape[1]), "relu_mask vs result")
    k = w0.shape[1]
    kp = k + (-k) % 4
    g0, w0 = _pad4_cols(g0), _pad4_cols(_pad4_rows(w0))
    if g1 is not None:
        g1, w1 = _pad4_cols(g1), _pad4_cols(_pad4_rows(w1))
    if relu_mask is not None:
        relu_mask = _pad4_cols(relu_mask)
    dev = _operands(g0, w0, g1, w1, relu_mask)
    m = g0.shape[0]
    gin = torch.empty((m, kp), dtype=torch.float32, device=dev)
    n0, n1 = g0.shape[1], g1.shape[1] if g1 is not None else 0
    _timed("igrad", 2.0 * m * kp * (n0 + n1), lambda: check(
        _lib.load().gts_linear_bwd_input_f32(ptr(g0), ptr(w0), ptr(g1), ptr(w1), ptr(relu_mask), ptr(gin),
                                             m, kp, n0, n1, current_stream()), "gts_linear_bwd_input_f32"))
    return gin if kp == k else gin[:, :k].contiguous()


def transpose_batch(mats):
    import ctypes

    if not mats:
        return []
    rows, cols = mats[0].shape
    mats = [m.contiguous() for m in mats]
    dev = _operands(*mats)
    for m in mats:
        _same(tuple(m.shape), (rows, cols), "matrices of one transpose batch")
    out = torch.empty((len(mats), cols, rows), dtype=torch.float32, device=dev)
    arr = ctypes.c_void_p * len(mats)
    check(_lib.load().gts_transpose_batch_f32(arr(*[ptr(m) for m in mats]), arr(*[ptr(out[q]) for q in range(len(mats))]),
                                              len(mats), rows, cols, current_stream()), "gts_transpose_batch_f32")
    return list(out.unbind(0))


def linear_bwd_input_t(g0, w0t, g1=None, w1t=None, relu_mask=None, relu_bits=None, packed=None):
    _same(_mat(g0, "g0").shape[1], _mat(w0t, "w0t").shape[1], "inner dims of g0 @ w0t^T")
    if (g1 is None) != (w1t is None):
        raise _lib.GtsError("g1 and w1t go together")
    if g1 is not None:
        _same(_mat(g1, "g1").shape[1], _mat(w1t, "w1t").shape[1], "inner dims of g1 @ w1t^T")
        _same(g1.shape[0], g0.shape[0], "rows of g0 / g1")
        _same(w1t.shape[0], w0t.shape[0], "rows of w0t / w1t")
    m, k = g0.shape[0], w0t.shape[0]
    if relu_mask is not None:
        _same(tuple(relu_mask.shape), (m, k), "relu_mask vs result")
    n0, n1 = g0.shape[1], g1.shape[1] if g1 is not None else 0
    if k % 4 or n0 % 4 or n1 % 4:
        raise _lib.GtsError("linear_bwd_input_t needs widths that are multiples of 4 (use linear_bwd_input)")
    g0, w0t, g1, w1t, relu_mask = _dense(g0, w0t, g1, w1t, relu_mask)
    dev = _operands(g0, w0t, g1, w1t, relu_mask)
    relu_bits = relu_bits if relu_mask is not None else None
    _chk_bits(relu_bits, m, k, "relu_bits")
    gin = torch.empty((m, k), dtype=torch.float32, device=dev)
    table = _packed_array(packed, (w0t, w1t))
    _timed("igrad", 2.0 * m * k * (n0 + n1), lambda: check(
        _lib.load().gts_linear_bwd_input_t_f32(ptr(g0), ptr(w0t), ptr(g1), ptr(w1t), ptr(relu_mask), ptr(relu_bits),
                                               ptr(gin), m, k, n0, n1, table, current_stream()), "gts_linear_bwd_input_t_f32"))
    return gin


def linear_bwd_input_t_act(g0, w0t, act_out, activation, g1=None, w1t=None, want_bias_grad=True, packed=None):
    _same(_mat(g0, "g0").shape[1], _mat(w0t, "w0t").shape[1], "inner dims of g0 @ w0t^T")
    if (g1 is None) != (w1t is None):
        raise _lib.GtsError("g1 and w1t go together")
    if g1 is not None:
        _same(_mat(g1, "g1").shape[1], _mat(w1t, "w1t").shape[1], "inner dims of g1 @ w1t^T")
        _same(g1.shape[0], g0.shape[0], "rows of g0 / g1")
        _same(w1t.shape[0], w0t.shape[0], "rows of w0t / w1t")
    m, k = g0.shape[0], w0t.shape[0]
    _same(tuple(_mat(act_out, "act_out").shape), (m, k), "act_out vs result")
    n0, n1 = g0.shape[1], g1.shape[1] if g1 is not None else 0
    if k % 4 or n0 % 4 or n1 % 4:
        raise _lib.GtsError("linear_bwd_input_t_act needs widths that are multiples of 4")
    g0, w0t, g1, w1t, act_out = _dense(g0, w0t, g1, w1t, act_out)
    dev = _operands(g0, w0t, g1, w1t, act_out)
    lib = _lib.load()
    gin = torch.empty((m, k), dtype=torch.float32, device=dev)
    g_bias = torch.empty(k, dtype=torch.float32, device=dev) if want_bias_grad else None
    nbytes = lib.gts_linear_bwd_input_t_act_workspace(m, k) if want_bias_grad else 0
    ws = _gemm_ws.get(dev, nbytes) if want_bias_grad else None
    table = _packed_array(packed, (w0t, w1t))
    _timed("igrad", 2.0 * m * k * (n0 + n1), lambda: check(
        lib.gts_linear_bwd_input_t_act_f32(ptr(g0), ptr(w0t), ptr(g1), ptr(w1t), ptr(act_out), activation, ptr(gin),
                                           ptr(g_bias), ptr(ws), nbytes, m, k, n0, n1, table, current_stream()),
        "gts_linear_bwd_input_t_act_f32"))
    return gin, g_bias


MAX_WGRAD_PROBLEMS = 32


def linear_bwd_weight_multi(problems):
    import ctypes

    if len(problems) > MAX_WGRAD_PROBLEMS:
        return (linear_bwd_weight_multi(problems[:MAX_WGRAD_PROBLEMS])
                + linear_bwd_weight_multi(problems[MAX_WGRAD_PROBLEMS:]))

    n, k = problems[0][0].shape[1], problems[0][1].shape[1]
    gs = [_pad4_cols(g) for g, _, _ in problems]
    acts = [_pad4_cols(a) for _, a, _ in problems]
    dev = _operands(*gs, *acts)
    m, n_p, k_p = gs[0].shape[0], gs[0].shape[1], acts[0].shape[1]
    for g, a in zip(gs, acts):
        if g.shape != (m, n_p) or a.shape != (m, k_p):
            raise _lib.GtsError("batched weight gradients need identical shapes")
    q = len(problems)
    gws = [torch.empty((n_p, k_p), dtype=torch.float32, device=dev) for _ in range(q)]
    gbs = [torch.empty(n_p, dtype=torch.float32, device=dev) if want else None for _, _, want in problems]
    if m == 0:
        for t in gws + [b for b in gbs if b is not None]:
            t.zero_()
    else:
        lib = _lib.load()
        nbytes = lib.gts_linear_bwd_weight_workspace(m, n_p, k_p, q)
        ws = _gemm_ws.get(dev, nbytes)
        arr = ctypes.c_void_p * q
        _timed("wgrad", 2.0 * m * n_p * k_p * q, lambda: check(
            lib.gts_linear_bwd_weight_f32(arr(*[ptr(t) for t in gs]), arr(*[ptr(t) for t in acts]),
                                          arr(*[ptr(t) for t in gws]), arr(*[ptr(t) for t in gbs]), q,
                                          ptr(ws), ws.numel() * 4, m, n_p, k_p, current_stream()),
            "gts_linear_bwd_weight_f32"))
    out = []
    for gw, gb in zip(gws, gbs):
        if (n_p, k_p) != (n, k):
            gw = gw[:n, :k].contiguous()
            gb = gb[:n].contiguous() if gb is not None else None
        out.append((gw, gb))
    return out


def linear_bwd_weight(g, a, want_bias_grad=False):
    return linear_bwd_weight_multi([(g, a, want_bias_grad)])[0]


def relu_bwd(g, out):
    return g * (out > 0)


class _Linear(torch.autograd.Function):

    @staticmethod
    def forward(ctx, x, w, bias):
        ctx.save_for_backward(x, w)
        ctx.has_bias = bias is not None
        return linear_fwd(x, w, bias=bias)

    @staticmethod
    def backward(ctx, gy):
        x, w = ctx.saved_tensors
        gy = gy.contiguous()
        gx = linear_bwd_input(gy, w) if ctx.needs_input_grad[0] else None
        gw = gb = None
        if ctx.needs_input_grad[1] or (ctx.has_bias and ctx.needs_input_grad[2]):
            gw, gb = linear_bwd_weight(gy, x, want_bias_grad=ctx.has_bias)
        return gx, gw, gb if ctx.has_bias else None


def linear(x, w, bias=None):
    return _Linear.apply(x, w, bias)
```

### gnn-tumor-seg_amd/gts/nn.py

```python
import os

import torch
import torch.nn as nn
import torch.nn.functional as F

from . import dense, ops
from .graph import _DeviceSchedule


class GraphError(RuntimeError):
    """Counterpart of dgl.DGLError for the checks the layers make."""


def _is_relu(fn):
    return fn in (F.relu, torch.relu, torch.nn.functional.relu)


class _SagePoolLayer(torch.autograd.Function):

    @staticmethod
    def forward(ctx, g, h, w_pool, b_pool, w_self, w_neigh, bias, relu_out, need_bwd):
        h = h.contiguous()
        p = dense.linear_fwd(h, w_pool, bias=b_pool, relu=True)
        m, arg = ops.spmm_max_fwd(g, p, want_arg=need_bwd, relu_input=True)
        out = dense.linear_fwd(h, w_self, m, w_neigh, bias=bias, relu=relu_out)
        if need_bwd:
            ctx.g, ctx.relu_out = g, relu_out
            ctx.save_for_backward(h, m, arg, out if relu_out else None, w_pool, w_self, w_neigh)
        return out

    @staticmethod
    def backward(ctx, gout):
        h, m, arg, out, w_pool, w_self, w_neigh = ctx.saved_tensors
        if not ctx.relu_out:
            g = gout.contiguous()
        elif out.shape[1] % 4 == 0 and out.shape[0] > 0:
            g, _ = ops.gat_act_bwd(gout.contiguous(), out, 2, want_bias_grad=False)
        else:
            g = dense.relu_bwd(gout, out)
        need = ctx.needs_input_grad
        gm = dense.linear_bwd_input(g, w_neigh)
        gp = ops.spmm_max_bwd(ctx.g, gm, arg)
        g_ws, g_wn, g_wp, g_bias, g_bp = _pool_layer_weight_grads(g, gp, h, m, w_pool, w_self)
        gh = dense.linear_bwd_input(g, w_self, gp, w_pool) if need[1] else None
        return None, gh, g_wp, g_bp, g_ws, g_wn, g_bias, None, None


class _SageSumLayer(torch.autograd.Function):

    @staticmethod
    def forward(ctx, g, h, w_self, w_neigh, bias, mode, relu_out, need_bwd):
        h = h.contiguous()
        d = g.dev()
        fin, fout = w_neigh.shape[1], w_neigh.shape[0]
        lin_first = fin > fout
        div = d.deg_clamped if mode == "mean" else d.deg_plus1
        src = dense.linear_fwd(h, w_neigh) if lin_first else h
        neigh = ops.spmm_sum_raw(g, src, div_out=div, add_self=(mode == "gcn"))
        last_w = _identity(fout, h.device) if lin_first else w_neigh
        if w_self is not None:
            out = dense.linear_fwd(h, w_self, neigh, last_w, bias=bias, relu=relu_out)
        else:
            out = dense.linear_fwd(neigh, last_w, bias=bias, relu=relu_out)
        if need_bwd:
            ctx.g, ctx.mode, ctx.relu_out, ctx.lin_first = g, mode, relu_out, lin_first
            ctx.has_bias = bias is not None
            ctx.save_for_backward(h, neigh if not lin_first else None, out if relu_out else None, w_self, w_neigh)
        return out

    @staticmethod
    def backward(ctx, gout):
        h, neigh, out, w_self, w_neigh = ctx.saved_tensors
        g, mode = ctx.g, ctx.mode
        d = g.dev()
        div = d.deg_clamped if mode == "mean" else d.deg_plus1
        need = ctx.needs_input_grad
        g_pre, g_bias = ops.gat_act_bwd(gout.contiguous(), out, 2 if ctx.relu_out else 0, want_bias_grad=ctx.has_bias)

        def reduce_bwd(t, accum=None):
            return ops.spmm_sum_raw(g, t, transposed=True, div_in=div, add_self=(mode == "gcn"), accum=accum)

        g_ws = None
        if ctx.lin_first:
            gt = reduce_bwd(g_pre)
            if w_self is not None:
                (g_ws, _), (g_wn, _) = dense.linear_bwd_weight_multi([(g_pre, h, False), (gt, h, False)])
                gh = dense.linear_bwd_input(g_pre, w_self, gt, w_neigh) if need[1] else None
            else:
                g_wn, _ = dense.linear_bwd_weight(gt, h)
                gh = dense.linear_bwd_input(gt, w_neigh) if need[1] else None
        else:
            if w_self is not None:
                (g_ws, _), (g_wn, _) = dense.linear_bwd_weight_multi([(g_pre, h, False), (g_pre, neigh, False)])
            else:
                g_wn, _ = dense.linear_bwd_weight(g_pre, neigh)
            gh = None
            if need[1]:
                gneigh = dense.linear_bwd_input(g_pre, w_neigh)
                gself = dense.linear_bwd_input(g_pre, w_self) if w_self is not None else None
                gh = reduce_bwd(gneigh, accum=gself)
        return None, gh, g_ws, g_wn, g_bias, None, None, None


_identities = {}


def _identity(n, device):
    key = (n, device)
    if key not in _identities:
        _identities[key] = torch.eye(n, dtype=torch.float32, device=device)
    return _identities[key]


RELU_MASK_BITS = os.environ.get("GTS_RELU_BITS", "1") != "0"


def _chainable(a0, w0, a1, w2):
    n, k0, k1, n2 = w0.shape[0], a0.shape[1], a1.shape[1], w2.shape[0]
    return n % 4 == 0 and k0 % 4 == 0 and k1 % 4 == 0 and n <= 256 and n2 <= 256 and w2.shape[1] == n


def _pool_layer_weight_grads(g, gp, h, m, w_pool, w_self):
    if w_pool.shape == w_self.shape:
        (g_ws, g_bias), (g_wn, _), (g_wp, g_bp) = dense.linear_bwd_weight_multi(
            [(g, h, True), (g, m, False), (gp, h, True)])
    else:
        (g_ws, g_bias), (g_wn, _) = dense.linear_bwd_weight_multi([(g, h, True), (g, m, False)])
        g_wp, g_bp = dense.linear_bwd_weight(gp, h, want_bias_grad=True)
    return g_ws, g_wn, g_wp, g_bias, g_bp


def _pack_by_shape(weights, transposed, want_plain=False):
    by_shape, plain, fragment = {}, {}, {}
    for w in weights:
        by_shape.setdefault(tuple(w.shape), []).append(w)
    for ws in by_shape.values():
        copies = dense.pack_weights(ws, transposed=transposed, want_plain=want_plain)
        if want_plain:
            plain.update((id(w), wt) for w, wt in zip(ws, copies[0]))
            copies = copies[1]
        fragment.update((id(w), wp) for w, wp in zip(ws, copies))
    return (plain, fragment) if want_plain else fragment


class _SagePoolStack(torch.autograd.Function):

    @staticmethod
    def forward(ctx, g, x, need_bwd, *params):
        n_layers = len(params) // 5
        h = x.contiguous()
        saved = []
        hbits = None
        p = None
        fragment = _pack_by_shape([w for i in range(n_layers) for w in (params[5 * i], params[5 * i + 2], params[5 * i + 3])
                                   if w.shape[0] > 128 and w.shape[1] % 4 == 0], transposed=False)
        for i in range(n_layers):
            w_pool, b_pool, w_self, w_neigh, bias = params[5 * i:5 * i + 5]
            last = i == n_layers - 1
            if p is None:
                p = dense.linear_fwd(h, w_pool, bias=b_pool, relu=True, packed=(fragment.get(id(w_pool)), None))
            m, arg = ops.spmm_max_fwd(g, p, want_arg=need_bwd, relu_input=True)
            p = None
            nxt = params[5 * (i + 1):5 * (i + 1) + 2] if not last else None
            obits = dense.relu_bits_empty(h.shape[0], w_self.shape[0], h.device) \
                if RELU_MASK_BITS and need_bwd and not last and dense.relu_bits_pay(h.shape[0], w_self.shape[0]) else None
            if nxt is not None and _chainable(h, w_self, m, nxt[0]):
                out, p = dense.linear_fwd_chain(h, w_self, m, w_neigh, bias, True, nxt[0], nxt[1], True, relu_bits=obits,
                                                packed=(fragment.get(id(w_self)), fragment.get(id(w_neigh)), fragment.get(id(nxt[0]))))
            else:
                out = dense.linear_fwd(h, w_self, m, w_neigh, bias=bias, relu=not last, relu_bits=obits,
                                       packed=(fragment.get(id(w_self)), fragment.get(id(w_neigh))))
            saved += [h, m, arg, hbits]
            h, hbits = out, obits
        if need_bwd:
            ctx.g, ctx.n_layers = g, n_layers
            ctx.save_for_backward(*saved, *params)
        return h

    @staticmethod
    def backward(ctx, gout):
        n = ctx.n_layers
        tensors = ctx.saved_tensors
        acts, params = tensors[:4 * n], tensors[4 * n:]
        grads = [None] * (5 * n)
        g = gout.contiguous()
        gx = None
        deferred = {}

        turned, turned_fragment = _pack_by_shape(
            [w for w in (params[5 * i + j] for i in range(n) for j in (0, 2, 3))
             if w.shape[1] >= 128 and w.shape[0] % 4 == 0 and w.shape[1] % 4 == 0], transposed=True, want_plain=True)

        def igrad(g0, w0, g1=None, w1=None, relu_mask=None, relu_bits=None):
            if id(w0) in turned and (w1 is None or id(w1) in turned) and g0.is_contiguous():
                return dense.linear_bwd_input_t(g0, turned[id(w0)], g1, turned[id(w1)] if w1 is not None else None,
                                                relu_mask=relu_mask, relu_bits=relu_bits,
                                                packed=(turned_fragment[id(w0)], turned_fragment[id(w1)] if w1 is not None else None))
            return dense.linear_bwd_input(g0, w0, g1, w1, relu_mask=relu_mask)

        def defer(grad_out, act, slot, bias_slot):
            key = (grad_out.shape[1], act.shape[1])
            deferred.setdefault(key, []).append((grad_out, act, bias_slot is not None, slot, bias_slot))

        gm = None
        for i in reversed(range(n)):
            h, m, arg, hbits = acts[4 * i:4 * i + 4]
            w_pool, _b_pool, w_self, w_neigh, _bias = params[5 * i:5 * i + 5]
            if gm is None:
                gm = igrad(g, w_neigh)
            gp = ops.spmm_max_bwd(ctx.g, gm, arg)
            gm = None
            defer(gp, h, 5 * i, 5 * i + 1)
            defer(g, h, 5 * i + 2, 5 * i + 4)
            defer(g, m, 5 * i + 3, None)
            if i > 0:
                below = params[5 * (i - 1) + 3]
                if all(id(w) in turned for w in (w_self, w_pool, below)) and _chainable(g, w_self.t(), gp, below.t()):
                    g, gm = dense.linear_bwd_input_chain_t(g, turned[id(w_self)], gp, turned[id(w_pool)], h,
                                                           turned[id(below)], relu_bits=hbits,
                                                           packed=(turned_fragment[id(w_self)], turned_fragment[id(w_pool)],
                                                                   turned_fragment[id(below)]))
                else:
                    g = igrad(g, w_self, gp, w_pool, relu_mask=h, relu_bits=hbits)
            elif ctx.needs_input_grad[1]:
                gx = igrad(g, w_self, gp, w_pool)
        for problems in deferred.values():
            results = dense.linear_bwd_weight_multi([(go, act, want) for go, act, want, _, _ in problems])
            for (gw, gb), (_, _, _, slot, bias_slot) in zip(results, problems):
                grads[slot] = gw
                if bias_slot is not None:
                    grads[bias_slot] = gb
        return (None, gx, None, *grads)


STACK_IN_ONE_CALL = os.environ.get("GTS_STACK_C", "1") != "0"


class GradSink:

    def __init__(self, params, extra=0):
        self.params = list(params)
        self.offsets, at = {}, 0
        for p in self.params:
            self.offsets[id(p)] = at
            at += p.numel()
        self.n, self.extra = at, int(extra)
        self.flat, self.filled = None, False

    def new_buffer(self):
        self.flat = torch.empty(self.n + self.extra, dtype=torch.float32, device=self.params[0].device)
        self.filled = False
        return self.flat


_active_sink = None


class grad_sink:
    def __init__(self, sink):
        self.sink = sink

    def __enter__(self):
        global _active_sink
        self.previous, _active_sink = _active_sink, self.sink
        return self.sink

    def __exit__(self, *exc):
        global _active_sink
        _active_sink = self.previous
        return False


_stack_tables = {}


def _stack_table(params, in_feats):
    import ctypes

    ptrs = [p.data_ptr() for p in params]
    key = (in_feats, *ptrs, *[tuple(p.shape) for p in params])
    hit = _stack_tables.get(key)
    if hit is None:
        n_layers = len(params) // 5
        widths = [in_feats] + [params[5 * i + 2].shape[0] for i in range(n_layers)]
        hit = ((ctypes.c_void_p * (5 * n_layers))(*ptrs), (ctypes.c_int64 * (n_layers + 1))(*widths), widths)
        if len(_stack_tables) > 64:
            _stack_tables.clear()
        _stack_tables[key] = hit
    return hit


class _SagePoolStackCall(torch.autograd.Function):

    @staticmethod
    def forward(ctx, g, x, need_bwd, *params):
        import ctypes

        from . import _lib
        from ._lib import check, current_stream, ptr

        lib = _lib.load()
        x = x.contiguous()
        n, n_layers = x.shape[0], len(params) // 5
        table, c_widths, widths = _stack_table(params, x.shape[1])
        relu_bits, ab = 1 if RELU_MASK_BITS else 0, g.arg_bytes
        d = g.dev()
        offsets = (ctypes.c_int64 * (4 * n_layers + 2))()
        total = lib.gts_sage_pool_stack_fwd_arena(n, c_widths, n_layers, 1 if need_bwd else 0, ab, relu_bits, offsets)
        if total < 0:
            raise _lib.GtsError("gts_sage_pool_stack_fwd_arena rejected the stack's shape")
        arena = torch.empty(max(int(total), 16), dtype=torch.uint8, device=x.device)
        ds = ops._cluster_schedule(g, "in", n, 256, ab if need_bwd else 0) if 256 in widths[:-1] else None
        check(lib.gts_sage_pool_stack_fwd_f32(
            ptr(d.indptr), ptr(d.indices), *_DeviceSchedule.launch_args(ds), ptr(x), table, n, c_widths, n_layers,
            1 if need_bwd else 0, ab, relu_bits, arena.data_ptr(), int(total), current_stream()),
            "gts_sage_pool_stack_fwd_f32")
        at = int(offsets[4 * (n_layers - 1) + 2])
        out = arena[at:at + 4 * n * widths[-1]].view(torch.float32).view(n, widths[-1])
        if need_bwd:
            ctx.g, ctx.widths, ctx.relu_bits, ctx.ab = g, widths, relu_bits, ab
            ctx.param_ids = [id(p) for p in params]
            ctx.save_for_backward(x, arena, *params)
        return out

    @staticmethod
    def backward(ctx, gout):
        import ctypes

        from . import _lib
        from ._lib import check, current_stream, ptr

        lib = _lib.load()
        x, arena, *params = ctx.saved_tensors
        g, widths, relu_bits, ab = ctx.g, ctx.widths, ctx.relu_bits, ctx.ab
        n, n_layers = x.shape[0], len(params) // 5
        gout = gout.contiguous()
        d = g.dev()
        sink = _active_sink
        if sink is not None and (len(ctx.param_ids) != len(sink.params) or
                                 not all(i in sink.offsets for i in ctx.param_ids)):
            sink = None
        sizes = [p.numel() for p in params]
        if sink is not None:
            flat, starts = sink.flat, [sink.offsets[i] for i in ctx.param_ids]
        else:
            flat = torch.empty(sum(sizes), dtype=torch.float32, device=x.device)
            starts = [0] * len(sizes)
            for q in range(1, len(sizes)):
                starts[q] = starts[q - 1] + sizes[q - 1]
        base = flat.data_ptr()
        grads = (ctypes.c_void_p * (5 * n_layers))(*[base + 4 * s for s in starts])
        table, c_widths, _ = _stack_table(params, x.shape[1])
        need = lib.gts_sage_pool_stack_bwd_scratch(n, c_widths, n_layers, relu_bits)
        scratch = torch.empty(max(int(need), 16), dtype=torch.uint8, device=x.device)
        gx = torch.empty_like(x) if ctx.needs_input_grad[1] else None
        ds = ops._cluster_schedule(g, "out", n, 256, ab) if 256 in widths[:-1] else None
        check(lib.gts_sage_pool_stack_bwd_f32(
            ptr(d.t_indptr), ptr(d.t_indices), ptr(d.t_slot), *_DeviceSchedule.launch_args(ds), ptr(gout), ptr(x), table, n,
            c_widths, n_layers, ab, relu_bits, arena.data_ptr(), grads, ptr(gx), scratch.data_ptr(), int(need),
            current_stream()), "gts_sage_pool_stack_bwd_f32")
        if sink is not None:
            sink.filled = True
            return (None, gx, None, *([None] * len(params)))
        return (None, gx, None, *[flat[s:s + k].view_as(p) for s, k, p in zip(starts, sizes, params)])


def sage_pool_stack(graph, features, layers):
    for i, layer in enumerate(layers):
        last = i == len(layers) - 1
        if not isinstance(layer, SAGEConv) or layer._aggre_type != "pool" or layer.bias is None \
                or layer.norm is not None or (layer.feat_drop.p > 0 and layer.training):
            return None
        if (layer.activation is not None) if last else (not _is_relu(layer.activation)):
            return None
    params = []
    for layer in layers:
        params += [layer.fc_pool.weight, layer.fc_pool.bias, layer.fc_self.weight,
                   layer.fc_neigh.weight, layer.bias]
    need_bwd = torch.is_grad_enabled() and (features.requires_grad or any(p.requires_grad for p in params))
    one_call = STACK_IN_ONE_CALL and not ops.INSTRUMENTED and features.shape[1] % 4 == 0 \
        and all(p.shape[-1] % 4 == 0 and p.shape[0] % 4 == 0 and p.is_contiguous() for p in params) \
        and features.dtype == torch.float32 and features.is_cuda
    return (_SagePoolStackCall if one_call else _SagePoolStack).apply(graph, features, need_bwd, *params)


class SAGEConv(nn.Module):

    def __init__(self, in_feats, out_feats, aggregator_type, feat_drop=0.0, bias=True, norm=None,
                 activation=None):
        super().__init__()
        if aggregator_type not in ("mean", "gcn", "pool"):
            raise KeyError(f"Invalid aggregator_type. Must be one of mean, gcn, pool. "
                           f"But got {aggregator_type!r} instead.")
        self._in_src_feats = self._in_dst_feats = int(in_feats)
        self._out_feats = int(out_feats)
        self._aggre_type = aggregator_type
        self.norm = norm
        self.feat_drop = nn.Dropout(feat_drop)
        self.activation = activation
        if aggregator_type == "pool":
            self.fc_pool = nn.Linear(in_feats, in_feats)
        if aggregator_type != "gcn":
            self.fc_self = nn.Linear(in_feats, out_feats, bias=False)
        self.fc_neigh = nn.Linear(in_feats, out_feats, bias=False)
        if bias:
            self.bias = nn.Parameter(torch.zeros(out_feats))
        else:
            self.register_buffer("bias", None)
        self.reset_parameters()

    def reset_parameters(self):
        gain = nn.init.calculate_gain("relu")
        if self._aggre_type == "pool":
            nn.init.xavier_uniform_(self.fc_pool.weight, gain=gain)
        if self._aggre_type != "gcn":
            nn.init.xavier_uniform_(self.fc_self.weight, gain=gain)
        nn.init.xavier_uniform_(self.fc_neigh.weight, gain=gain)

    def _load_from_state_dict(self, state_dict, prefix, *args, **kwargs):
        legacy = [prefix + "fc_self.bias", prefix + "fc_neigh.bias"]
        if prefix + "bias" not in state_dict and any(k in state_dict for k in legacy):
            folded = sum(state_dict.pop(k) for k in legacy if k in state_dict)
            state_dict[prefix + "bias"] = folded
        super()._load_from_state_dict(state_dict, prefix, *args, **kwargs)

    def forward(self, graph, feat):
        h = self.feat_drop(feat)
        fused_relu = _is_relu(self.activation)
        if self._aggre_type == "pool":
            bias = self.bias if self.bias is not None else torch.zeros(
                self._out_feats, dtype=h.dtype, device=h.device)
            need_bwd = torch.is_grad_enabled() and (
                h.requires_grad or any(p.requires_grad for p in self.parameters()))
            rst = _SagePoolLayer.apply(graph, h, self.fc_pool.weight, self.fc_pool.bias,
                                       self.fc_self.weight, self.fc_neigh.weight, bias,
                                       fused_relu, need_bwd)
        elif self._out_feats % 4 == 0 and h.shape[0] > 0:
            need_bwd = torch.is_grad_enabled() and (
                h.requires_grad or any(p.requires_grad for p in self.parameters()))
            w_self = self.fc_self.weight if self._aggre_type != "gcn" else None
            rst = _SageSumLayer.apply(graph, h, w_self, self.fc_neigh.weight, self.bias, self._aggre_type,
                                      fused_relu, need_bwd)
        else:
            lin_before_mp = self._in_src_feats > self._out_feats
            src = dense.linear(h, self.fc_neigh.weight) if lin_before_mp else h
            neigh = ops.spmm_reduce(graph, src, self._aggre_type)
            if not lin_before_mp:
                neigh = dense.linear(neigh, self.fc_neigh.weight)
            rst = neigh if self._aggre_type == "gcn" else dense.linear(h, self.fc_self.weight) + neigh
            if self.bias is not None:
                rst = rst + self.bias
            if fused_relu:
                rst = torch.relu(rst)
        if self.activation is not None and not fused_relu:
            rst = self.activation(rst)
        if self.norm is not None:
            rst = self.norm(rst)
        return rst


FUSE_GAT_LAYER = os.environ.get("GTS_FUSE_GAT", "1") != "0"
FUSE_GAT_SCORES = os.environ.get("GTS_FUSE_GAT_SCORES", "1") != "0"


FOLD_GAT_ACT_BWD = os.environ.get("GTS_FOLD_GAT_ACT", "1") != "0"


PACK_GAT_WEIGHTS = os.environ.get("GTS_PACK_GAT", "1") != "0"


def _turn(ws):
    if PACK_GAT_WEIGHTS:
        plain, packed = dense.pack_weights(ws, transposed=True, want_plain=True)
        return plain, tuple(packed) if len(packed) > 1 else (packed[0], None)
    return dense.transpose_batch(ws), (None, None)


class ActLink:
    __slots__ = ("folded", "g_bias", "armed")

    def __init__(self):
        self.folded, self.g_bias, self.armed = False, None, 0


class _GATLayer(torch.autograd.Function):

    @staticmethod
    def forward(ctx, g, h, w_fc, attn_l, attn_r, bias, w_res, identity_res, slope, act_code, heads, dim,
                need_bwd, below=None, above=None):
        h = h.contiguous()
        n = h.shape[0]
        al, ar = attn_l.reshape(heads, dim), attn_r.reshape(heads, dim)
        if FUSE_GAT_SCORES and h.shape[1] % 4 == 0:
            ft, el, er = ops.gat_fc_scores(h, w_fc, al, ar, heads, dim)
        else:
            ft = dense.linear_fwd(h, w_fc).view(n, heads, dim)
            el, er = ops.gat_scores(ft, al, ar)
        if w_res is not None:
            res = dense.linear_fwd(h, w_res)
        elif identity_res:
            res = h
        else:
            res = None
        out, attn = ops._gat_fwd(g, ft, el, er, slope, bias, res, act_code)
        if need_bwd:
            ctx.g, ctx.slope, ctx.act, ctx.identity_res = g, slope, act_code, identity_res
            ctx.save_for_backward(h, ft, el, er, attn, out if act_code else None, w_fc, al, ar, w_res)
            ctx.attn_shape = attn_l.shape
            ctx.below, ctx.above = below, above if act_code == 1 else None
            if ctx.above is not None:
                ctx.above.armed = act_code
        return out

    @staticmethod
    def backward(ctx, gout):
        h, ft, el, er, attn, out, w_fc, al, ar, w_res = ctx.saved_tensors
        n, heads, dim = ft.shape
        need = ctx.needs_input_grad
        if ctx.above is not None and ctx.above.folded:
            g_pre, g_bias = gout.reshape(n, heads * dim), ctx.above.g_bias if need[5] else None
            ctx.above.folded, ctx.above.g_bias, ctx.above.armed = False, None, 0
        else:
            g_pre, g_bias = ops.gat_act_bwd(gout.reshape(n, heads * dim),
                                            out.view(n, heads * dim) if out is not None else None, ctx.act,
                                            want_bias_grad=need[5])
        gft, gel, ger = ops._gat_bwd(ctx.g, ft, el, er, attn, g_pre.view(n, heads, dim), ctx.slope, al, ar)
        g_al, g_ar = ops.gat_param_grad(ft, gel, ger)
        gft2 = gft.view(n, heads * dim)
        g_wres = None
        turn = need[1] and w_fc.shape[1] >= 128 and w_fc.shape[0] % 4 == 0 \
            and w_fc.shape[1] % 4 == 0 and n >= 4096
        fold = turn and ctx.below is not None and ctx.below.armed == 1 and not ctx.identity_res and FOLD_GAT_ACT_BWD
        act_below = ctx.below.armed if fold else 0
        if w_res is not None:
            (g_wfc, _), (g_wres, _) = dense.linear_bwd_weight_multi([(gft2, h, False), (g_pre, h, False)])
            if fold:
                wt, wtp = _turn([w_fc, w_res])
                gh, ctx.below.g_bias = dense.linear_bwd_input_t_act(gft2, wt[0], h, act_below, g_pre, wt[1], packed=wtp)
                ctx.below.folded = True
            elif turn:
                wt, wtp = _turn([w_fc, w_res])
                gh = dense.linear_bwd_input_t(gft2, wt[0], g_pre, wt[1], packed=wtp)
            else:
                gh = dense.linear_bwd_input(gft2, w_fc, g_pre, w_res) if need[1] else None
        else:
            g_wfc, _ = dense.linear_bwd_weight(gft2, h)
            if fold:
                wt, wtp = _turn([w_fc])
                gh, ctx.below.g_bias = dense.linear_bwd_input_t_act(gft2, wt[0], h, act_below, packed=(wtp[0], None))
                ctx.below.folded = True
            elif turn:
                wt, wtp = _turn([w_fc])
                gh = dense.linear_bwd_input_t(gft2, wt[0], packed=(wtp[0], None))
            else:
                gh = dense.linear_bwd_input(gft2, w_fc) if need[1] else None
            if gh is not None and ctx.identity_res:
                gh = gh + g_pre
        return (None, gh, g_wfc, g_al.view(ctx.attn_shape), g_ar.view(ctx.attn_shape), g_bias, g_wres,
                None, None, None, None, None, None, None, None)


class GATConv(nn.Module):

    def __init__(self, in_feats, out_feats, num_heads, feat_drop=0.0, attn_drop=0.0,
                 negative_slope=0.2, residual=False, activation=None,
                 allow_zero_in_degree=False, bias=True):
        super().__init__()
        self._in_feats, self._out_feats, self._num_heads = int(in_feats), int(out_feats), int(num_heads)
        self._allow_zero_in_degree = allow_zero_in_degree
        self.fc = nn.Linear(in_feats, out_feats * num_heads, bias=False)
        self.attn_l = nn.Parameter(torch.empty(1, num_heads, out_feats))
        self.attn_r = nn.Parameter(torch.empty(1, num_heads, out_feats))
        self.feat_drop = nn.Dropout(feat_drop)
        self.attn_drop = nn.Dropout(attn_drop)
        self.negative_slope = negative_slope
        if bias:
            self.bias = nn.Parameter(torch.empty(num_heads * out_feats))
        else:
            self.register_buffer("bias", None)
        if residual:
            if in_feats != out_feats * num_heads:
                self.res_fc = nn.Linear(in_feats, num_heads * out_feats, bias=False)
            else:
                self.res_fc = nn.Identity()
        else:
            self.register_buffer("res_fc", None)
        self.activation = activation
        self.reset_parameters()

    def reset_parameters(self):
        gain = nn.init.calculate_gain("relu")
        nn.init.xavier_normal_(self.fc.weight, gain=gain)
        nn.init.xavier_normal_(self.attn_l, gain=gain)
        nn.init.xavier_normal_(self.attn_r, gain=gain)
        if self.bias is not None:
            nn.init.constant_(self.bias, 0)
        if isinstance(self.res_fc, nn.Linear):
            nn.init.xavier_normal_(self.res_fc.weight, gain=gain)

    def forward(self, graph, feat, below=None, above=None):
        if not self._allow_zero_in_degree and graph.min_in_degree == 0:
            raise GraphError(
                "There are 0-in-degree nodes in the graph, output for those nodes will be invalid. "
                "Adding self-loop on the input graph resolves the issue; setting "
                "allow_zero_in_degree=True suppresses the check.")
        if self.attn_drop.p > 0 and self.training:
            raise NotImplementedError("attention dropout is not built (the reference never sets it: "
                                      "model/networks.py:77-78 passes no dropout to GAT)")
        n = feat.shape[0]
        h = self.feat_drop(feat)
        if above is not None:
            above.armed = 0
        act_code = 0 if self.activation is None else 1 if self.activation in (F.elu, torch.nn.functional.elu) else -1
        if FUSE_GAT_LAYER and act_code >= 0 and self._out_feats % 4 == 0 and feat.dim() == 2:
            w_res = self.res_fc.weight if isinstance(self.res_fc, nn.Linear) else None
            identity_res = isinstance(self.res_fc, nn.Identity)
            need_bwd = torch.is_grad_enabled() and (
                h.requires_grad or any(p.requires_grad for p in self.parameters()))
            if self.feat_drop.p > 0 and self.training:
                below = None
            return _GATLayer.apply(graph, h, self.fc.weight, self.attn_l, self.attn_r, self.bias, w_res,
                                   identity_res, self.negative_slope, act_code, self._num_heads,
                                   self._out_feats, need_bwd, below, above)
        ft = dense.linear(h, self.fc.weight).view(n, self._num_heads, self._out_feats)
        el = (ft * self.attn_l).sum(dim=-1)
        er = (ft * self.attn_r).sum(dim=-1)
        rst = ops.gat_aggregate(graph, ft, el, er, self.negative_slope)
        if self.res_fc is not None:
            res = dense.linear(h, self.res_fc.weight) if isinstance(self.res_fc, nn.Linear) else h
            rst = rst + res.view(n, -1, self._out_feats)
        if self.bias is not None:
            rst = rst + self.bias.view(1, self._num_heads, self._out_feats)
        if self.activation is not None:
            rst = self.activation(rst)
        return rst
```

### include/gts_hip.h

```cpp
#ifndef GTS_HIP_H
#define GTS_HIP_H

#include <stdint.h>

#ifdef __cplusplus
extern "C" {
#endif

#define GTS_OK 0
#define GTS_ERR_NULL (-1)
#define GTS_ERR_SHAPE (-2)
#define GTS_ERR_ARGKIND (-3)

int32_t gts_abi_version(void);
const char* gts_error_string(int32_t code);

int32_t gts_spmm_max_fwd_f32(const int32_t* indptr, const int32_t* indices, const float* x,
                             float* out, void* arg, int32_t arg_bytes, int32_t relu_input,
                             int64_t n_dst, int64_t n_feat, void* stream);

int32_t gts_spmm_max_bwd_f32(const int32_t* t_indptr, const int32_t* t_indices,
                             const int32_t* t_slot, const float* gout, const void* arg,
                             int32_t arg_bytes, const float* relu_src, float* gx,
                             int64_t n_src, int64_t n_feat, void* stream);

int64_t gts_cluster_record_words(int32_t max_rows, int32_t max_srcs, int32_t loc_words, int32_t with_tag);
int32_t gts_cluster_schedule(const int32_t* indptr, const int32_t* indices, const int32_t* t_indptr,
                             const int32_t* t_indices, const int32_t* edge_tag, int64_t n_rows,
                             int32_t max_rows, int32_t max_srcs, int32_t max_edges, int32_t* rec,
                             int64_t rec_capacity, int64_t* n_clusters, int64_t* n_staged,
                             int32_t* max_cluster_edges);
int64_t gts_cluster_lds_bytes(int32_t max_rows, int32_t max_srcs, int32_t loc_words, int32_t kind);
int32_t gts_spmm_max_fwd_cluster_f32(const int32_t* rec, int64_t n_clusters, int32_t max_rows, int32_t max_srcs,
                                     int32_t loc_words, const float* x, float* out, void* arg,
                                     int32_t arg_bytes, int32_t relu_input, int64_t n_rows, int64_t n_feat,
                                     uint32_t* counters, void* stream);
int32_t gts_spmm_max_bwd_cluster_f32(const int32_t* rec, int64_t n_clusters, int32_t max_rows, int32_t max_srcs,
                                     int32_t loc_words, const float* gout, const void* arg, int32_t arg_bytes,
                                     float* gx, int64_t n_rows, int64_t n_feat, uint32_t* counters, void* stream);
#define GTS_CLUSTER_COUNTER_WORDS 256
int32_t gts_cluster_uses_counters(int64_t n_clusters, int32_t max_rows, int32_t max_srcs, int32_t loc_words, int32_t backward);

int32_t gts_spmm_sum_f32(const int32_t* indptr, const int32_t* indices, const float* x,
                         float* out, const float* div_in, const float* div_out, const float* accum,
                         int32_t add_self, int64_t n_out, int64_t n_feat, void* stream);

int32_t gts_gat_fwd_f32(const int32_t* indptr, const int32_t* indices, const float* ft,
                        const float* el, const float* er, float negative_slope, const float* bias,
                        const float* residual, int32_t activation, float* out, float* attn,
                        int64_t n, int64_t heads, int64_t dim, void* stream);
int32_t gts_gat_scores_f32(const float* ft, const float* attn_l, const float* attn_r, float* el,
                           float* er, int64_t n, int64_t heads, int64_t dim, void* stream);

int32_t gts_gat_bwd_edge_f32(const int32_t* indptr, const int32_t* indices, const float* ft,
                             const float* el, const float* er, const float* attn,
                             const float* gout, float negative_slope, float* ge, float* ger,
                             int64_t n, int64_t heads, int64_t dim, void* stream);
int32_t gts_gat_bwd_src_f32(const int32_t* t_indptr, const int32_t* t_indices,
                            const int32_t* t_pos, const float* attn, const float* ge,
                            const float* gout, const float* attn_l, const float* attn_r,
                            const float* ger, float* gft, float* gel, int64_t n, int64_t heads,
                            int64_t dim, void* stream);
int64_t gts_gat_reduce_workspace(int64_t n, int64_t cols);
int32_t gts_gat_act_bwd_f32(const float* gout, const float* out, int32_t activation, float* g_pre,
                            float* g_bias, float* workspace, int64_t workspace_bytes, int64_t n,
                            int64_t cols, void* stream);
int32_t gts_gat_param_grad_f32(const float* ft, const float* gel, const float* ger, float* g_attn_l,
                               float* g_attn_r, float* workspace, int64_t workspace_bytes, int64_t n,
                               int64_t heads, int64_t dim, void* stream);

int64_t gts_gat_cluster_workspace(int64_t n_clusters, int32_t max_rows, int32_t loc_words, int64_t heads, int32_t backward);
int32_t gts_gat_attn_f32(const int32_t* indptr, const int32_t* indices, const float* el, const float* er,
                         float negative_slope, float* attn, int64_t n, int64_t heads, int64_t max_degree, void* stream);
int32_t gts_gat_fwd_cluster_f32(const int32_t* indptr, const int32_t* indices, const int32_t* rec, int64_t n_clusters,
                                int32_t max_rows, int32_t max_srcs, int32_t loc_words, int32_t tagged, const float* ft,
                                const float* el, const float* er, float negative_slope, const float* bias,
                                int32_t activation, float* out, float* attn, float* workspace, int64_t workspace_bytes,
                                int64_t n, int64_t heads, int64_t dim, int64_t max_degree, void* stream);
int32_t gts_gat_bwd_edge_cluster_f32(const int32_t* indptr, const int32_t* indices, const int32_t* rec, int64_t n_clusters,
                                     int32_t max_rows, int32_t max_srcs, int32_t loc_words, int32_t tagged, const float* ft,
                                     const float* el, const float* er, const float* attn, const float* gout,
                                     float negative_slope, float* ge, float* ger, float* workspace, int64_t workspace_bytes,
                                     int64_t n, int64_t heads, int64_t dim, int64_t max_degree, void* stream);
int32_t gts_gat_bwd_src_cluster_f32(const int32_t* t_indptr, const int32_t* t_pos, const int32_t* rec, int64_t n_clusters,
                                    int32_t max_rows, int32_t max_srcs, int32_t loc_words, int32_t tagged,
                                    const float* attn, const float* ge, const float* gout, const float* attn_lr,
                                    const float* ger, float* gft, float* gel, float* workspace, int64_t workspace_bytes,
                                    int64_t n, int64_t heads, int64_t dim, int64_t max_degree, void* stream);

int32_t gts_project_rows_i16(const int16_t* svs, const void* table, const void* bg_row,
                             void* out, int64_t n_vox, int64_t n_rows, int32_t row_bytes,
                             void* stream);
int32_t gts_project_argmax_i16(const int16_t* svs, const float* logits, const int16_t* relabel,
                               int16_t* out, int64_t n_vox, int64_t n_rows, int64_t n_classes,
                               void* stream);

int32_t gts_project_argmax_occupancy_i16(const int16_t* svs, const float* logits, int16_t* out,
                                         uint8_t* occupancy, int64_t dim_x, int64_t dim_y,
                                         int64_t dim_z, int64_t n_rows, int64_t n_classes,
                                         void* stream);

int32_t gts_crop_concat_f32(const float* img, const int16_t* svs, const float* table,
                            const float* bg_row, const int32_t* xs, const int32_t* ys,
                            const int32_t* zs, float* out, int64_t cx, int64_t cy, int64_t cz,
                            int64_t dim_y, int64_t dim_z, int64_t n_rows, int64_t img_channels,
                            int64_t row_channels, void* stream);
int32_t gts_argmax_scatter_i16(const float* scores, const int16_t* relabel, const int32_t* xs,
                               const int32_t* ys, const int32_t* zs, int16_t* out, int64_t cx,
                               int64_t cy, int64_t cz, int64_t dim_y, int64_t dim_z,
                               int64_t n_classes, void* stream);
int32_t gts_crop_concat_rows_f32(const float* img, const int16_t* svs, const float* table,
                                 const float* bg_row, const int32_t* xs, const int32_t* ys,
                                 const int32_t* zs, float* out, int64_t cx, int64_t cy, int64_t cz,
                                 int64_t dim_y, int64_t dim_z, int64_t n_rows, int64_t img_channels,
                                 int64_t row_channels, void* stream);
int32_t gts_crop_concat_rows_bwd_f32(const float* dx, const int32_t* list_ptr, const int32_t* list_vox,
                                     const int32_t* inv_x, const int32_t* inv_y, const int32_t* inv_z,
                                     float* d_table, int64_t cx, int64_t cy, int64_t cz, int64_t dim_x,
                                     int64_t dim_y, int64_t dim_z, int64_t n_rows, int64_t img_channels,
                                     int64_t row_channels, void* stream);

int32_t gts_adamw_f32(float* param, const float* grad, float* exp_avg, float* exp_avg_sq, int64_t n,
                      double lr, double beta1, double beta2, double eps, double weight_decay,
                      int64_t step, void* stream);

int64_t gts_label_confusion_workspace(int64_t n);
int32_t gts_label_confusion_i16(const int16_t* pred, const int16_t* truth, int64_t* counts,
                                void* workspace, int64_t workspace_bytes, int64_t n, void* stream);

int64_t gts_relu_bits_bytes(int64_t m, int64_t n);
int32_t gts_relu_bits_pay(int64_t m, int64_t n);
int32_t gts_linear_fwd_f32(const float* a0, const float* w0, const float* a1, const float* w1,
                           const float* bias, float* out, int64_t m, int64_t n, int64_t k0,
                           int64_t k1, int32_t relu, uint64_t* relu_bits, const float* const* packed,
                           void* stream);
int64_t gts_packed_weight_floats(int64_t n, int64_t k);
int32_t gts_pack_weights_f32(const float* const* src, float* const* dst, float* const* plain_t, int32_t n_mats,
                             int64_t rows, int64_t cols, int32_t transposed, void* stream);
int32_t gts_linear_bwd_input_f32(const float* g0, const float* w0, const float* g1, const float* w1,
                                 const float* relu_mask, float* gin, int64_t m, int64_t k,
                                 int64_t n0, int64_t n1, void* stream);
int32_t gts_linear_bwd_input_t_f32(const float* g0, const float* w0t, const float* g1, const float* w1t,
                                   const float* relu_mask, const uint64_t* relu_bits, float* gin, int64_t m,
                                   int64_t k, int64_t n0, int64_t n1, const float* const* packed, void* stream);
int64_t gts_linear_bwd_input_t_act_workspace(int64_t m, int64_t k);
int32_t gts_linear_bwd_input_t_act_f32(const float* g0, const float* w0t, const float* g1, const float* w1t,
                                       const float* act_out, int32_t activation, float* gin, float* g_bias,
                                       float* workspace, int64_t workspace_bytes, int64_t m, int64_t k,
                                       int64_t n0, int64_t n1, const float* const* packed,
                                       void* stream);
int64_t gts_gat_fc_scores_workspace(int64_t m, int64_t heads, int64_t dim);
int32_t gts_gat_fc_scores_f32(const float* h, const float* w_fc, const float* attn_l, const float* attn_r,
                              float* ft, float* el, float* er, float* workspace, int64_t workspace_bytes,
                              int64_t m, int64_t heads, int64_t dim, int64_t k, const float* w_fc_packed, void* stream);
int32_t gts_linear_fwd_chain_f32(const float* a0, const float* w0, const float* a1, const float* w1,
                                 const float* bias, float* out, const float* w2, const float* bias2,
                                 float* out2, int64_t m, int64_t n, int64_t k0, int64_t k1, int32_t relu,
                                 int64_t n2, int32_t relu2, uint64_t* relu_bits, const float* const* packed,
                                 void* stream);
int32_t gts_linear_bwd_input_chain_t_f32(const float* g0, const float* w0t, const float* g1,
                                         const float* w1t, const float* relu_mask, const uint64_t* relu_bits,
                                         float* gin, const float* w2t, float* gin2, int64_t m, int64_t k,
                                         int64_t n0, int64_t n1, int64_t k2, const float* const* packed,
                                         void* stream);
int32_t gts_transpose_batch_f32(const float* const* src, float* const* dst, int32_t n_mats,
                                int64_t rows, int64_t cols, void* stream);
int64_t gts_linear_bwd_weight_workspace(int64_t m, int64_t n, int64_t k, int32_t n_problems);
int32_t gts_linear_bwd_weight_f32(const float* const* g, const float* const* a, float* const* gw,
                                  float* const* gb, int32_t n_problems, float* workspace,
                                  int64_t workspace_bytes, int64_t m, int64_t n, int64_t k,
                                  void* stream);

int64_t gts_sage_pool_stack_fwd_arena(int64_t n_rows, const int64_t* widths, int32_t n_layers, int32_t training,
                                      int32_t arg_bytes, int32_t relu_bits, int64_t* offsets);
int32_t gts_sage_pool_stack_fwd_f32(const int32_t* indptr, const int32_t* indices, const int32_t* sched_rec,
                                    int64_t sched_clusters, int32_t sched_rows, int32_t sched_srcs,
                                    int32_t sched_loc_words, const float* x, const float* const* params,
                                    int64_t n_rows, const int64_t* widths, int32_t n_layers, int32_t training,
                                    int32_t arg_bytes, int32_t relu_bits, void* arena, int64_t arena_bytes, void* stream);
int64_t gts_sage_pool_stack_bwd_scratch(int64_t n_rows, const int64_t* widths, int32_t n_layers, int32_t relu_bits);
int32_t gts_sage_pool_stack_bwd_f32(const int32_t* t_indptr, const int32_t* t_indices, const int32_t* t_slot,
                                    const int32_t* sched_rec, int64_t sched_clusters, int32_t sched_rows,
                                    int32_t sched_srcs, int32_t sched_loc_words, const float* gout, const float* x,
                                    const float* const* params, int64_t n_rows, const int64_t* widths,
                                    int32_t n_layers, int32_t arg_bytes, int32_t relu_bits, const void* fwd_arena,
                                    float* const* grads, float* gx, void* scratch, int64_t scratch_bytes,
                                    void* stream);

int64_t gts_weighted_ce_workspace(int64_t n);
int32_t gts_weighted_ce_f32(const float* logits, const int64_t* labels, const float* class_w,
                            float* grad_unscaled, float* workspace, int64_t workspace_bytes,
                            float* out3, int64_t n, int64_t n_classes, void* stream);

#define GTS_DICE_CE_MAX_GROUPS 8
#define GTS_DICE_CE_STATS_FLOATS 40
#define GTS_DICE_CE_STATS_LOSS 0
#define GTS_DICE_CE_STATS_CE 1
#define GTS_DICE_CE_STATS_LDICE 2
#define GTS_DICE_CE_STATS_CE_NUM 3
#define GTS_DICE_CE_STATS_CE_DEN 4
#define GTS_DICE_CE_STATS_DICE 8
#define GTS_DICE_CE_STATS_I 16
#define GTS_DICE_CE_STATS_S 24
#define GTS_DICE_CE_STATS_T 32
int64_t gts_dice_ce_workspace(int64_t n, int32_t n_groups);
int32_t gts_dice_ce_fwd_f32(const float* logits, const int64_t* labels, const float* class_w,
                            const uint32_t* group_masks, int32_t n_groups, double ce_weight,
                            double dice_weight, double smooth, float* stats, void* workspace,
                            int64_t workspace_bytes, int64_t n, int64_t n_classes, void* stream);
int32_t gts_dice_ce_bwd_f32(const float* logits, const int64_t* labels, const float* class_w,
                            const uint32_t* group_masks, int32_t n_groups, double ce_weight,
                            double dice_weight, double smooth, const float* stats,
                            const float* grad_scale, float* grad, int64_t n, int64_t n_classes,
                            void* stream);

int32_t gts_augment_crop_f32(const float* x, const int64_t* labels, const float* params, float* x_out,
                             int64_t* labels_out, int64_t cx, int64_t cy, int64_t cz, int64_t channels,
                             int64_t image_channels, int32_t flip_mask, uint64_t seed, uint64_t step,
                             void* stream);
int32_t gts_augment_features_f32(const float* feats, const int64_t* row_ptr, const int64_t* row_ptr_host,
                                 const float* params, float* out, int64_t n_rows, int64_t n_feats,
                                 int64_t modalities, int64_t n_graphs, double sigma, uint64_t seed,
                                 uint64_t step, void* stream);

int32_t gts_augment_spatial_f32(const float* x, const int64_t* labels, const float* params,
                                const double* matrix, float* x_out, int64_t* labels_out, int64_t cx,
                                int64_t cy, int64_t cz, int64_t channels, int64_t image_channels,
                                int32_t flip_mask, uint64_t seed, uint64_t step, void* stream);
int32_t gts_augment_spatial_bwd_f32(const float* dy, const double* matrix, float* dx, int64_t cx, int64_t cy,
                                    int64_t cz, int64_t channels, int32_t flip_mask, void* stream);

#define GTS_OPT_GEMM_TILE 1
#define GTS_OPT_WGRAD_TILE 2
#define GTS_OPT_IGRAD_TILE 3
#define GTS_OPT_PROJECT_STREAMING 6
#define GTS_OPT_SPMM_ROWS_PER_WAVE 4
#define GTS_OPT_SPMM_STREAMING 5
#define GTS_OPT_GEMM_SCHED 7
#define GTS_OPT_CLUSTER_STREAMING 8
#define GTS_OPT_GAT_WALK 14
#define GTS_OPT_GAT_CLUSTER_WAVES 15
#define GTS_OPT_GAT_CLUSTER_GROUP 16
#define GTS_OPT_GAT_CLUSTER_DEALING 17
#define GTS_OPT_CLUSTER_DEALING 18
#define GTS_OPT_PANEL_ROWS 13
#define GTS_OPT_CLUSTER_RING 10
#define GTS_OPT_CLUSTER_PER_CU 11
#define GTS_OPT_CLUSTER_CONSUMERS 12
int32_t gts_set_option(int32_t option, int32_t value);
int32_t gts_get_option(int32_t option);

#define GTS_COLLATE_MAX_SCHEDULES 6
typedef struct {
  int64_t n_nodes, n_edges;
  const int32_t *indptr, *indices, *t_indptr, *t_indices, *t_slot, *t_pos;
  const void* features;
  const void* labels;
  int32_t feat_bytes;
  int32_t label_bytes;
  const int32_t* sched_rec[GTS_COLLATE_MAX_SCHEDULES];
  int64_t sched_clusters[GTS_COLLATE_MAX_SCHEDULES];
  int32_t sched_loc_words[GTS_COLLATE_MAX_SCHEDULES];
} gts_collate_member_t;
typedef struct {
  int32_t max_rows, max_srcs, tagged, reserved;
} gts_collate_kind_t;
typedef struct {
  int64_t total_bytes, n_nodes, n_edges;
  int64_t features, labels;
  int64_t csr[8];
  int64_t sched[GTS_COLLATE_MAX_SCHEDULES];
  int64_t sched_clusters[GTS_COLLATE_MAX_SCHEDULES];
  int32_t sched_loc_words[GTS_COLLATE_MAX_SCHEDULES];
  int32_t sched_record_words[GTS_COLLATE_MAX_SCHEDULES];
} gts_collate_plan_t;
int32_t gts_collate_plan(const gts_collate_member_t* members, int32_t n_members, int64_t feat_width,
                         const gts_collate_kind_t* kinds, int32_t n_kinds, gts_collate_plan_t* plan);
int32_t gts_collate_batch(const gts_collate_member_t* members, int32_t n_members, int64_t feat_width,
                          const gts_collate_kind_t* kinds, int32_t n_kinds, void* dst, int64_t dst_bytes,
                          int32_t n_threads, gts_collate_plan_t* plan);

#define GTS_GG_MAX_SV 32767
#define GTS_GG_MAX_K 32
#define GTS_GG_MAX_RADIUS 16
int32_t gts_gg_gaussian_f64(const double* in, double* out, double* tmp, const double* weights, int32_t radius,
                            double scale, int64_t d, int64_t h, int64_t w, int64_t c, void* stream);
int32_t gts_gg_slic_assign_f64(const double* img, const double* centres, int32_t n_centres, int64_t d, int64_t h,
                               int64_t w, int64_t c, int32_t step_z, int32_t step_y, int32_t step_x,
                               double spatial_weight, int32_t* labels, uint64_t* best, uint32_t* winner,
                               void* stream);
int32_t gts_gg_slic_update_f64(const double* img, const int32_t* labels, double* centres, int32_t n_centres,
                               int64_t d, int64_t h, int64_t w, int64_t c, int32_t* bbox, void* stream);
int32_t gts_gg_enforce_connectivity(const int32_t* labels, int32_t* out, int64_t d, int64_t h, int64_t w,
                                    int64_t min_size, int64_t max_size, int64_t* queue, int32_t* n_labels);
int64_t gts_gg_sv_stats_workspace(int64_t n_vox, int32_t n_sv);
int32_t gts_gg_sv_stats(const int32_t* partition, const float* intensities, const int16_t* vox_labels, int64_t d,
                        int64_t h, int64_t w, int64_t c, int32_t n_sv, double* feats, double* centroids,
                        int32_t* sv_labels, void* scratch, void* stream);
int32_t gts_gg_discard_f64(const double* feats, const double* centroids, const int32_t* sv_labels, int32_t n_sv,
                           int32_t n_feat, const int32_t* partition, int64_t n_vox, int32_t* remap, int32_t* keep,
                           double* node_feats, double* node_centroids, int32_t* node_labels, int16_t* new_partition,
                           int32_t* n_nodes, void* stream);
int32_t gts_gg_knn_candidates_f64(const double* positions, int32_t n, int32_t k, int32_t* cand, void* stream);
int32_t gts_gg_knn_greedy(const int32_t* cand, int32_t n, int32_t k, int32_t* picks, int32_t* got, int64_t* n_edges);
int64_t gts_gg_touching_workspace(int32_t n);
int32_t gts_gg_touching_count_i16(const int16_t* partition, int64_t d, int64_t h, int64_t w, int32_t n, void* scratch,
                                  int32_t* indptr, void* stream);
int32_t gts_gg_touching_emit(const void* scratch, int32_t n, const int32_t* indptr, int32_t* cols, void* stream);

int64_t gts_conv3d_fwd_workspace(int32_t cin, int32_t cout);
int32_t gts_conv3d_fwd_f32(const float* x, const float* w, const float* bias, float* y, int64_t cx, int64_t cy,
                           int64_t cz, int32_t cin, int32_t cout, int32_t relu, void* workspace,
                           int64_t workspace_bytes, void* stream);
int64_t gts_conv3d_bwd_data_workspace(int64_t cx, int64_t cy, int64_t cz, int32_t cin, int32_t cout);
int32_t gts_conv3d_bwd_data_f32(const float* dy, const float* w, const float* h, float* dx, int64_t cx, int64_t cy,
                                int64_t cz, int32_t cin, int32_t cout, void* workspace, int64_t workspace_bytes,
                                void* stream);
int64_t gts_conv3d_bwd_weight_workspace(int64_t cx, int64_t cy, int64_t cz, int32_t cin, int32_t cout);
int32_t gts_conv3d_bwd_weight_f32(const float* x, const float* dy, float* dw, float* db, int64_t cx, int64_t cy,
                                  int64_t cz, int32_t cin, int32_t cout, void* workspace, int64_t workspace_bytes,
                                  void* stream);

int64_t gts_hd95_workspace(int64_t X, int64_t Y, int64_t Z);
int32_t gts_hd95_order_stats_i16(const int16_t* pred, const int16_t* truth, int64_t X, int64_t Y, int64_t Z,
                                 int32_t all_border, int64_t* out, void* workspace, int64_t workspace_bytes,
                                 void* stream);

int64_t gts_surface_workspace(int64_t X, int64_t Y, int64_t Z, const int64_t* units);
int32_t gts_surface_stats_i16(const int16_t* pred, const int16_t* truth, int64_t X, int64_t Y, int64_t Z,
                              int32_t all_border, const int64_t* units, const int64_t* thresholds,
                              int32_t n_thresholds, int64_t* out, void* workspace, int64_t workspace_bytes,
                              void* stream);

int64_t gts_components_workspace(int64_t X, int64_t Y, int64_t Z);
int32_t gts_components_roots_i16(const int16_t* labels, int64_t X, int64_t Y, int64_t Z, int32_t connectivity,
                                 int32_t* roots_out, void* workspace, int64_t workspace_bytes, void* stream);
int32_t gts_components_filter_i16(const int16_t* labels_in, int64_t X, int64_t Y, int64_t Z, int32_t connectivity,
                                  int64_t min_voxels, int32_t et_label, int64_t et_min_voxels, int32_t et_replacement,
                                  int16_t* labels_out, int64_t* stats, void* workspace, int64_t workspace_bytes,
                                  void* stream);

int64_t gts_lesionwise_workspace(int64_t X, int64_t Y, int64_t Z);
int64_t gts_lesionwise_table_ints(int64_t X, int64_t Y, int64_t Z);
int32_t gts_lesionwise_dilate_i16(const int16_t* labels, int64_t X, int64_t Y, int64_t Z, int32_t region,
                                  int32_t dilation, int16_t* mask_out, void* workspace, int64_t workspace_bytes,
                                  void* stream);
int32_t gts_lesionwise_tables_i16(const int16_t* truth, const int32_t* pred_roots, const int32_t* dilated_roots,
                                  int64_t X, int64_t Y, int64_t Z, int32_t region, int32_t* tables_out,
                                  int64_t tables_ints, void* workspace, int64_t workspace_bytes, void* stream);
int32_t gts_lesionwise_masks_i16(const int16_t* truth, const int32_t* pred_roots, const int32_t* dilated_roots,
                                 int64_t X, int64_t Y, int64_t Z, int32_t region, int32_t lesion_root,
                                 const int32_t* matched_roots, int64_t n_matched, const int64_t* box, int16_t* mask_m,
                                 int16_t* mask_g, void* stream);

int32_t gts_intake_occupancy(const void* src, int32_t dtype, int64_t X, int64_t Y, int64_t Z, int32_t* flag_x,
                             int32_t* flag_y, int32_t* flag_z, uint64_t* nonfinite, void* stream);
int64_t gts_intake_select_workspace(void);
int32_t gts_intake_order_stats(const void* src, int32_t dtype, int64_t X, int64_t Y, int64_t Z, const int32_t* xs,
                               int64_t cx, const int32_t* ys, int64_t cy, const int32_t* zs, int64_t cz,
                               int64_t rank_lo, int64_t rank_hi, float* out, void* workspace, int64_t workspace_bytes,
                               void* stream);
int32_t gts_intake_standardize(const void* src, int32_t dtype, int64_t X, int64_t Y, int64_t Z, const int32_t* xs,
                               int64_t cx, const int32_t* ys, int64_t cy, const int32_t* zs, int64_t cz,
                               const float* params, float* out, void* stream);

int64_t gts_dataset_stats_workspace(int64_t X, int64_t Y, int64_t Z);
int32_t gts_dataset_stats_mask(const void* src, int32_t dtype, const int16_t* labels, int64_t X, int64_t Y, int64_t Z,
                               uint64_t* counts, void* workspace, int64_t workspace_bytes, void* stream);
int32_t gts_dataset_stats_order_stats(const void* src, int32_t dtype, int64_t X, int64_t Y, int64_t Z, int64_t n,
                                      int64_t rank_lo, int64_t rank_hi, float* out, void* workspace,
                                      int64_t workspace_bytes, void* stream);
int32_t gts_dataset_stats_moments(const void* src, int32_t dtype, int64_t X, int64_t Y, int64_t Z, int64_t n,
                                  const float* top, double* out, void* workspace, int64_t workspace_bytes,
                                  void* stream);

int32_t gts_conform_gather(const void* src, int32_t dtype, int64_t C, int64_t X, int64_t Y, int64_t Z, int32_t axis0,
                           int32_t axis1, int32_t axis2, int64_t OX, int64_t OY, int64_t OZ, const int32_t* idx0,
                           const int32_t* idx1, const double* t, int32_t mode, void* dst, void* stream);

int32_t gts_softmax_accumulate_f32(const float* const* sets, int64_t n_sets, float* acc, int64_t rows,
                                   int64_t classes, int32_t overwrite, void* stream);
int32_t gts_argmax_scatter_rows_i16(const float* scores, const int16_t* relabel, const int32_t* xs,
                                    const int32_t* ys, const int32_t* zs, int16_t* out, int64_t cx, int64_t cy,
                                    int64_t cz, int64_t dim_y, int64_t dim_z, int64_t n_classes, void* stream);

#ifdef __cplusplus
}
#endif
#endif
```

Before: 957.5 graphs/s.

## Fuse narrow weight gradients into wide wgrad stream kernel as rider work

Adds a stacked weight-gradient entry point that runs the narrow problems (the 4-channel input layer and the final class projection) on idle slots of the wide wgrad stream kernel. It also merges the split-slab reduction and the narrow partial reduction into a single finish kernel. The goal is to cut separate launches and to use SM capacity left idle by the big 256x256 wgrad tiles. In exchange the wgrad kernel becomes more complex, rider work may unbalance the tiles, and a heuristic byte threshold decides when to fall back to a standalone narrow kernel.

```diff
diff --git a/gnn-tumor-seg_amd/csrc/gts_gemm.hip b/gnn-tumor-seg_amd/csrc/gts_gemm.hip
--- a/gnn-tumor-seg_amd/csrc/gts_gemm.hip
+++ b/gnn-tumor-seg_amd/csrc/gts_gemm.hip
@@ -295,37 +295,11 @@
   return gts_gat_act_bwd_f32(gin, act_out, activation, gin, g_bias, workspace, workspace_bytes, m, k, stream);
 }
 
-extern "C" int64_t gts_linear_bwd_weight_workspace(int64_t m, int64_t n, int64_t k, int32_t n_problems) {
-  using namespace gts;
-  if (m <= 0 || n <= 0 || k <= 0 || n_problems < 1 || n_problems > kMaxProblems) return 0;
-  const int64_t splits = wgrad_plan(m, n, k, n_problems).splits;
-  const int64_t slabs = n_problems * splits * (n * k + n);
-  const int64_t skinny = skinny_workspace_floats(m, n, k) + kSkinnyChunks * (n < k ? n : 0);
-  return (slabs > skinny ? slabs : skinny) * static_cast<int64_t>(sizeof(float));
-}
-
-extern "C" int32_t gts_linear_bwd_weight_f32(const float* const* g, const float* const* a, float* const* gw,
-                                             float* const* gb, int32_t n_problems, float* workspace,
-                                             int64_t workspace_bytes, int64_t m, int64_t n, int64_t k, void* stream) {
-  using namespace gts;
-  if (!g || !a || !gw || !workspace) return GTS_ERR_NULL;
-  if (n_problems < 1 || n_problems > kMaxProblems) return GTS_ERR_ARGKIND;
-  if (m <= 0 || n <= 0 || k <= 0 || m >= (1LL << 31) || n >= (1 << 20) || k >= (1 << 20) || !aligned4(n) || !aligned4(k))
-    return GTS_ERR_SHAPE;
-  if (workspace_bytes < gts_linear_bwd_weight_workspace(m, n, k, n_problems)) return GTS_ERR_SHAPE;
+static gts::GemmArgs wgrad_args(const float* const* g, const float* const* a, float* const* gb, int n_problems, float* workspace,
+                                int64_t m, int64_t n, int64_t k, int splits) {
+  using namespace gts;
   bool any_bias = false;
-  for (int q = 0; q < n_problems; ++q) {
-    if (!g[q] || !a[q] || !gw[q]) return GTS_ERR_NULL;
-    any_bias = any_bias || (gb && gb[q]);
-  }
-  hipStream_t st = static_cast<hipStream_t>(stream);
-  if (skinny_workspace_floats(m, n, k) > 0) {
-    for (int q = 0; q < n_problems; ++q)
-      skinny_wgrad(g[q], a[q], gw[q], gb ? gb[q] : nullptr, workspace, m, n, k, st);
-    return launch_status();
-  }
-  const WgradPlan plan = wgrad_plan(m, n, k, n_problems);
-  const int splits = plan.splits;
+  for (int q = 0; q < n_problems; ++q) any_bias = any_bias || (gb && gb[q]);
   const int tiles = static_cast<int>((m + kBK - 1) / kBK);
   GemmArgs p{};
   for (int q = 0; q < n_problems; ++q) p.pa[q] = g[q], p.pb[q] = a[q];
@@ -339,21 +313,172 @@
     if (gb[q]) p.colsum_mask |= 1u << q;
   p.n_problems = n_problems, p.n_splits = splits;
   p.tiles_per_split = (tiles + splits - 1) / splits;
+  return p;
+}
+
+template <class Jobs>
+static int wgrad_slab_jobs(const gts::GemmArgs& p, float* const* gw, float* const* gb, int64_t n, int64_t k, Jobs* r) {
+  const int n_problems = p.n_problems, splits = p.n_splits;
+  r->splits = splits;
+  int jobs = 0;
+  for (int q = 0; q < n_problems; ++q, ++jobs) {
+    r->slabs[jobs] = p.c + static_cast<size_t>(q) * splits * n * k;
+    r->out[jobs] = gw[q], r->n4[jobs] = static_cast<int>(n * k / 4);
+  }
+  for (int q = 0; q < n_problems && p.colsum != nullptr; ++q) {
+    if (!gb[q]) continue;
+    r->slabs[jobs] = p.colsum + static_cast<size_t>(q) * splits * n;
+    r->out[jobs] = gb[q], r->n4[jobs] = static_cast<int>(n / 4);
+    ++jobs;
+  }
+  return jobs;
+}
+
+extern "C" int64_t gts_linear_bwd_weight_workspace(int64_t m, int64_t n, int64_t k, int32_t n_problems) {
+  using namespace gts;
+  if (m <= 0 || n <= 0 || k <= 0 || n_problems < 1 || n_problems > kMaxProblems) return 0;
+  const int64_t splits = wgrad_plan(m, n, k, n_problems).splits;
+  const int64_t slabs = n_problems * splits * (n * k + n);
+  const int64_t skinny = skinny_workspace_floats(m, n, k) + kSkinnyChunks * (n < k ? n : 0);
+  return (slabs > skinny ? slabs : skinny) * static_cast<int64_t>(sizeof(float));
+}
+
+extern "C" int32_t gts_linear_bwd_weight_f32(const float* const* g, const float* const* a, float* const* gw,
+                                             float* const* gb, int32_t n_problems, float* workspace,
+                                             int64_t workspace_bytes, int64_t m, int64_t n, int64_t k, void* stream) {
+  using namespace gts;
+  if (!g || !a || !gw || !workspace) return GTS_ERR_NULL;
+  if (n_problems < 1 || n_problems > kMaxProblems) return GTS_ERR_ARGKIND;
+  if (m <= 0 || n <= 0 || k <= 0 || m >= (1LL << 31) || n >= (1 << 20) || k >= (1 << 20) || !aligned4(n) || !aligned4(k))
+    return GTS_ERR_SHAPE;
+  if (workspace_bytes < gts_linear_bwd_weight_workspace(m, n, k, n_problems)) return GTS_ERR_SHAPE;
+  for (int q = 0; q < n_problems; ++q)
+    if (!g[q] || !a[q] || !gw[q]) return GTS_ERR_NULL;
+  hipStream_t st = static_cast<hipStream_t>(stream);
+  if (skinny_workspace_floats(m, n, k) > 0) {
+    for (int q = 0; q < n_problems; ++q)
+      skinny_wgrad(g[q], a[q], gw[q], gb ? gb[q] : nullptr, workspace, m, n, k, st);
+    return launch_status();
+  }
+  const WgradPlan plan = wgrad_plan(m, n, k, n_problems);
+  const int splits = plan.splits;
+  const GemmArgs p = wgrad_args(g, a, gb, n_problems, workspace, m, n, k, splits);
   int rc = launch_wgrad(p, plan, st);
   if (rc != GTS_OK) return rc;
   ReduceArgs r{};
-  r.splits = splits;
-  int jobs = 0;
-  for (int q = 0; q < n_problems; ++q, ++jobs) {
-    r.slabs[jobs] = workspace + static_cast<size_t>(q) * splits * n * k;
-    r.out[jobs] = gw[q], r.n4[jobs] = static_cast<int>(n * k / 4);
-  }
-  for (int q = 0; q < n_problems && any_bias; ++q) {
-    if (!gb[q]) continue;
-    r.slabs[jobs] = p.colsum + static_cast<size_t>(q) * splits * n;
-    r.out[jobs] = gb[q], r.n4[jobs] = static_cast<int>(n / 4);
-    ++jobs;
-  }
+  const int jobs = wgrad_slab_jobs(p, gw, gb, n, k, &r);
   reduce_slabs_kernel<<<dim3(static_cast<unsigned>((n * k / 4 + 63) / 64), jobs), kBlock, 0, st>>>(r);
   return launch_status();
 }
+
+namespace {
+
+constexpr int64_t kRiderBytesPerRow = 5000;
+
+struct StackWgrad {
+  gts::WgradPlan wide;
+  gts::NarrowPlan narrow;
+  int wide_groups, riders;
+  int64_t wide_floats;
+};
+
+int32_t plan_stack_wgrad(int64_t m, int64_t n, int64_t k, int32_t n_wide, const float* const* ng, const float* const* na,
+                         float* const* ngw, float* const* ngb, const int64_t* nn, const int64_t* nk, int32_t n_narrow,
+                         StackWgrad* s) {
+  using namespace gts;
+  if (n_narrow > 0 && (!ng || !na || !nn || !nk)) return GTS_ERR_NULL;
+  if (n_wide < 0 || n_wide > kMaxProblems || n_narrow < 0 || n_narrow > kNarrowMax || n_wide + n_narrow == 0)
+    return GTS_ERR_ARGKIND;
+  if (m <= 0 || m >= (1LL << 31)) return GTS_ERR_SHAPE;
+  if (n_wide > 0 && (n <= 0 || k <= 0 || n >= (1 << 20) || k >= (1 << 20) || !aligned4(n) || !aligned4(k) || narrow_problem(n, k)))
+    return GTS_ERR_SHAPE;
+  for (int q = 0; q < n_narrow; ++q) {
+    if (nn[q] <= 0 || nk[q] <= 0 || nn[q] >= (1 << 20) || nk[q] >= (1 << 20) || !aligned4(nn[q]) || !aligned4(nk[q]) ||
+        !narrow_problem(nn[q], nk[q]))
+      return GTS_ERR_SHAPE;
+    if (!ng[q] || !na[q]) return GTS_ERR_NULL;
+  }
+  *s = StackWgrad{};
+  plan_narrow(ng, na, ngw, ngb, nn, nk, n_narrow, m, &s->narrow);
+  if (n_wide > 0) {
+    s->wide = wgrad_plan(m, n, k, n_wide);
+    s->wide_floats = static_cast<int64_t>(n_wide) * s->wide.splits * (n * k + n);
+    GemmArgs shape{};
+    shape.ra = static_cast<int>(n), shape.rb = static_cast<int>(k), shape.n_problems = n_wide;
+    int free_slots;
+    s->wide_groups = stream_tile_groups(shape, s->wide, &free_slots);
+    s->riders = free_slots < s->narrow.run.n_quads ? free_slots : s->narrow.run.n_quads;
+    if (s->riders > 0) {
+      int64_t stream_bytes = 0;
+      for (int q = 0; q < s->narrow.n_passes; ++q) stream_bytes += m * s->narrow.run.w[q] * static_cast<int64_t>(sizeof(float));
+      const int64_t tiles = (m + kBK - 1) / kBK;
+      const int64_t rows_per_split = (tiles + s->wide.splits - 1) / s->wide.splits * kBK;
+      if (stream_bytes > kRiderBytesPerRow * rows_per_split * s->riders) s->riders = 0;
+    }
+  }
+  return GTS_OK;
+}
+
+}
+
+extern "C" int64_t gts_wgrad_stack_workspace(int64_t m, int64_t n, int64_t k, int32_t n_wide, const int64_t* narrow_n,
+                                             const int64_t* narrow_k, int32_t n_narrow) {
+  using namespace gts;
+  if (m <= 0 || n_wide < 0 || n_wide > kMaxProblems || n_narrow < 0 || n_narrow > kNarrowMax) return 0;
+  if (n_narrow > 0 && (!narrow_n || !narrow_k)) return 0;
+  int64_t floats = 0;
+  if (n_wide > 0) {
+    if (n <= 0 || k <= 0) return 0;
+    floats += static_cast<int64_t>(n_wide) * wgrad_plan(m, n, k, n_wide).splits * (n * k + n);
+  }
+  for (int q = 0; q < n_narrow; ++q) {
+    if (narrow_n[q] <= 0 || narrow_k[q] <= 0) return 0;
+    floats += narrow_workspace_floats(m, narrow_n[q], narrow_k[q]);
+  }
+  return floats * static_cast<int64_t>(sizeof(float));
+}
+
+extern "C" int32_t gts_wgrad_stack_plan(int64_t m, int64_t n, int64_t k, int32_t n_wide, const float* const* narrow_g,
+                                        const float* const* narrow_a, float* const* narrow_gb, const int64_t* narrow_n,
+                                        const int64_t* narrow_k, int32_t n_narrow, int32_t* plan) {
+  if (!plan) return GTS_ERR_NULL;
+  StackWgrad s;
+  const int32_t rc = plan_stack_wgrad(m, n, k, n_wide, narrow_g, narrow_a, nullptr, narrow_gb, narrow_n, narrow_k, n_narrow, &s);
+  if (rc != GTS_OK) return rc;
+  plan[0] = s.riders, plan[1] = s.narrow.n_passes, plan[2] = s.narrow.run.n_quads, plan[3] = s.wide_groups;
+  return GTS_OK;
+}
+
+extern "C" int32_t gts_wgrad_stack_f32(const float* const* g, const float* const* a, float* const* gw, float* const* gb,
+                                       int32_t n_wide, int64_t n, int64_t k, const float* const* narrow_g,
+                                       const float* const* narrow_a, float* const* narrow_gw, float* const* narrow_gb,
+                                       const int64_t* narrow_n, const int64_t* narrow_k, int32_t n_narrow, float* workspace,
+                                       int64_t workspace_bytes, int64_t m, void* stream) {
+  using namespace gts;
+  if (!workspace || (n_wide > 0 && (!g || !a || !gw)) || (n_narrow > 0 && !narrow_gw)) return GTS_ERR_NULL;
+  StackWgrad s;
+  const int32_t bad = plan_stack_wgrad(m, n, k, n_wide, narrow_g, narrow_a, narrow_gw, narrow_gb, narrow_n, narrow_k, n_narrow, &s);
+  if (bad != GTS_OK) return bad;
+  if (workspace_bytes < gts_wgrad_stack_workspace(m, n, k, n_wide, narrow_n, narrow_k, n_narrow)) return GTS_ERR_SHAPE;
+  for (int q = 0; q < n_wide; ++q)
+    if (!g[q] || !a[q] || !gw[q]) return GTS_ERR_NULL;
+  for (int q = 0; q < n_narrow; ++q)
+    if (!narrow_gw[q]) return GTS_ERR_NULL;
+  hipStream_t st = static_cast<hipStream_t>(stream);
+  s.narrow.bind(workspace + s.wide_floats);
+  FinishArgs& fin = s.narrow.finish;
+  if (n_wide > 0) {
+    const GemmArgs p = wgrad_args(g, a, gb, n_wide, workspace, m, n, k, s.wide.splits);
+    const int rc = launch_wgrad(p, s.wide, st, &s.narrow.run, s.riders);
+    if (rc != GTS_OK) return rc;
+    const int jobs = wgrad_slab_jobs(p, gw, gb, n, k, &fin);
+    fin.slab_blocks_x = static_cast<int>((n * k / 4 + 63) / 64), fin.slab_blocks = fin.slab_blocks_x * jobs;
+  }
+  if (s.narrow.n_passes > 0 && s.riders == 0) {
+    narrow_wgrad_kernel<<<s.narrow.run.n_quads, kNarrowThreads, 0, st>>>(s.narrow.run);
+    const int rc = launch_status();
+    if (rc != GTS_OK) return rc;
+  }
+  wgrad_finish_kernel<<<fin.slab_blocks + fin.first_block[s.narrow.n_passes], kBlock, 0, st>>>(fin);
+  return launch_status();
+}
diff --git a/gnn-tumor-seg_amd/csrc/gts_gemm_wgrad.h b/gnn-tumor-seg_amd/csrc/gts_gemm_wgrad.h
--- a/gnn-tumor-seg_amd/csrc/gts_gemm_wgrad.h
+++ b/gnn-tumor-seg_amd/csrc/gts_gemm_wgrad.h
@@ -5,6 +5,114 @@
 
 namespace gts {
 namespace {
+
+constexpr int kSkinnyMax = 9;
+constexpr int kSkinnyChunks = 512;
+constexpr int kNarrowMax = GTS_WGRAD_MAX_NARROW;
+constexpr int kNarrowPasses = 2 * kNarrowMax;
+constexpr int kNarrowThreads = 1024;
+
+struct NarrowArgs {
+  const float* wide[kNarrowPasses];
+  const float* col[kNarrowPasses * kSkinnyMax];
+  int stride[kNarrowPasses * kSkinnyMax];
+  float* partial[kNarrowPasses];
+  int w[kNarrowPasses], rows[kNarrowPasses], loaded[kNarrowPasses];
+  long long m, rows_per_chunk;
+  int chunks, quads_per_pass, n_quads;
+};
+
+template <int S, bool UNIFORM_ROWS>
+__device__ __forceinline__ void skinny_chunk(const float* __restrict__ wide, int w, const float* const (&col)[S],
+                                             const int (&stride)[S], bool ones, float* __restrict__ partial, int64_t row0,
+                                             int64_t row1, bool in_range, int tid, v4f* red) {
+  const int cols4 = w >> 2;
+  const int lanes = cols4 >= kBlock ? 1 : kBlock / cols4;
+  const int rl = cols4 >= kBlock ? 0 : tid / cols4;
+  for (int q0 = 0; q0 < cols4; q0 += kBlock) {
+    const int q = q0 + (cols4 >= kBlock ? tid : tid % cols4);
+    const bool live = q < cols4 && rl < lanes && in_range;
+    v4f acc[S];
+#pragma unroll
+    for (int i = 0; i < S; ++i) acc[i] = v4f{0.f, 0.f, 0.f, 0.f};
+    if (UNIFORM_ROWS && live && (cols4 & (kWave - 1)) == 0) {
+      const int first = __builtin_amdgcn_readfirstlane(rl);
+      constexpr int kRowsInFlight = S <= 4 ? 4 : 2;
+#pragma unroll kRowsInFlight
+      for (int64_t row = row0 + first; row < row1; row += lanes) {
+        const v4f f = *reinterpret_cast<const v4f*>(wide + static_cast<size_t>(row) * w + 4 * q);
+#pragma unroll
+        for (int i = 0; i < S; ++i) acc[i] += (i + 1 < S || !ones ? col[i][row * stride[i]] : 1.0f) * f;
+      }
+    } else if (live) {
+      constexpr int kRowsInFlight = UNIFORM_ROWS ? 1 : 4;
+#pragma unroll kRowsInFlight
+      for (int64_t row = row0 + rl; row < row1; row += lanes) {
+        const v4f f = *reinterpret_cast<const v4f*>(wide + static_cast<size_t>(row) * w + 4 * q);
+#pragma unroll
+        for (int i = 0; i < S; ++i) acc[i] += (i + 1 < S || !ones ? col[i][row * stride[i]] : 1.0f) * f;
+      }
+    }
+#pragma unroll
+    for (int i = 0; i < S; ++i) {
+      v4f total = acc[i];
+      if (lanes > 1) {
+        __syncthreads();
+        red[tid] = acc[i];
+        __syncthreads();
+        if (rl == 0 && live) {
+          for (int l = 1; l < lanes; ++l) total += red[l * cols4 + q];
+        }
+      }
+      if (rl == 0 && live) *reinterpret_cast<v4f*>(partial + static_cast<size_t>(i) * w + 4 * q) = total;
+    }
+  }
+}
+
+template <int S, int BASE>
+__device__ __forceinline__ void narrow_chunk(int pass, int64_t chunk, int64_t m, int64_t rows_per_chunk, int chunks, v4f* red) {
+  const float* wide = kernarg_entry<const float*>(BASE + offsetof(NarrowArgs, wide), pass);
+  float* partial = kernarg_entry<float*>(BASE + offsetof(NarrowArgs, partial), pass);
+  const int w = kernarg_entry<int>(BASE + offsetof(NarrowArgs, w), pass);
+  const bool ones = kernarg_entry<int>(BASE + offsetof(NarrowArgs, loaded), pass) < S;
+  const float* col[S];
+  int stride[S];
+#pragma unroll
+  for (int i = 0; i < S; ++i) {
+    col[i] = kernarg_entry<const float*>(BASE + offsetof(NarrowArgs, col), pass * kSkinnyMax + i);
+    stride[i] = kernarg_entry<int>(BASE + offsetof(NarrowArgs, stride), pass * kSkinnyMax + i);
+  }
+  const int tid = threadIdx.x & (kBlock - 1);
+  const bool in_range = chunk < chunks;
+  const int64_t row0 = chunk * rows_per_chunk, row1 = in_range ? min(m, row0 + rows_per_chunk) : row0;
+  skinny_chunk<S, true>(wide, w, col, stride, ones, partial + static_cast<size_t>(chunk) * S * w, row0, row1, in_range, tid,
+                        red + (threadIdx.x - tid));
+}
+
+template <int BASE>
+__device__ __forceinline__ void narrow_role(const NarrowArgs& nw, int worker, int n_workers, v4f* red) {
+  const int quarter = __builtin_amdgcn_readfirstlane(threadIdx.x / kBlock);
+  for (int u = worker; u < nw.n_quads; u += n_workers) {
+    const int pass = u / nw.quads_per_pass;
+    const int64_t chunk = static_cast<int64_t>(u - pass * nw.quads_per_pass) * (kNarrowThreads / kBlock) + quarter;
+    switch (kernarg_entry<int>(BASE + offsetof(NarrowArgs, rows), pass)) {
+      case 1: narrow_chunk<1, BASE>(pass, chunk, nw.m, nw.rows_per_chunk, nw.chunks, red); break;
+      case 2: narrow_chunk<2, BASE>(pass, chunk, nw.m, nw.rows_per_chunk, nw.chunks, red); break;
+      case 3: narrow_chunk<3, BASE>(pass, chunk, nw.m, nw.rows_per_chunk, nw.chunks, red); break;
+      case 4: narrow_chunk<4, BASE>(pass, chunk, nw.m, nw.rows_per_chunk, nw.chunks, red); break;
+      case 5: narrow_chunk<5, BASE>(pass, chunk, nw.m, nw.rows_per_chunk, nw.chunks, red); break;
+      case 6: narrow_chunk<6, BASE>(pass, chunk, nw.m, nw.rows_per_chunk, nw.chunks, red); break;
+      case 7: narrow_chunk<7, BASE>(pass, chunk, nw.m, nw.rows_per_chunk, nw.chunks, red); break;
+      case 8: narrow_chunk<8, BASE>(pass, chunk, nw.m, nw.rows_per_chunk, nw.chunks, red); break;
+      default: narrow_chunk<9, BASE>(pass, chunk, nw.m, nw.rows_per_chunk, nw.chunks, red); break;
+    }
+  }
+}
+
+__global__ __launch_bounds__(kNarrowThreads) void narrow_wgrad_kernel(const NarrowArgs nw) {
+  __shared__ v4f red[kNarrowThreads];
+  narrow_role<0>(nw, blockIdx.x, gridDim.x, red);
+}
 
 typedef float v2f __attribute__((ext_vector_type(2)));
 
@@ -17,21 +125,28 @@
 }
 
 template <class Probe = NoProbe>
-__global__ __launch_bounds__(1024, 4) void wgrad_stream_kernel(const GemmArgs p) {
+__global__ __launch_bounds__(1024, 4) void wgrad_stream_kernel(const GemmArgs p, const NarrowArgs nw) {
   constexpr int BM = 256, BN = 256, WM = 4, WN = 4, WTM = 64, WTN = 64, TM = 2, TN = 2;
   constexpr int kPlane = kBK * BM;
   static_assert(BM == BN && kPlane * 4 == 128 * 256, "image I of an operand sits 128 offset units above image 0");
   __shared__ float lds[4 * kPlane];
+  const int tiles_m = (p.ra + BM - 1) / BM, tiles_y = p.tiles_n * p.n_problems;
+  const int wide_groups = tiles_m * tiles_y * p.n_splits;
+  if (static_cast<int>(blockIdx.x) >= wide_groups) {
+    narrow_role<sizeof(GemmArgs)>(nw, blockIdx.x - wide_groups, gridDim.x - wide_groups, reinterpret_cast<v4f*>(lds));
+    return;
+  }
+  const int block_y = (blockIdx.x / tiles_m) % tiles_y, block_z = blockIdx.x / (tiles_m * tiles_y);
   const int lane = threadIdx.x & 63, wave = __builtin_amdgcn_readfirstlane(threadIdx.x >> 6);
   const int wm = wave / WN, wn = wave % WN;
   const int i = lane & 31, h = lane >> 5;
-  const int problem = blockIdx.y / p.tiles_n, tile_n = blockIdx.y % p.tiles_n;
-  const int m0 = blockIdx.x * BM, n0 = tile_n * BN;
+  const int problem = block_y / p.tiles_n, tile_n = block_y % p.tiles_n;
+  const int m0 = (blockIdx.x % tiles_m) * BM, n0 = tile_n * BN;
   const float* g = kernarg_entry<const float*>(offsetof(GemmArgs, pa), problem);
   const float* act = kernarg_entry<const float*>(offsetof(GemmArgs, pb), problem);
   const int ldg = p.lda[0], lda = p.ldb[0];
   const int n_tiles_all = (p.kseg[0] + kBK - 1) / kBK;
-  const int t_beg = min(n_tiles_all, static_cast<int>(blockIdx.z) * p.tiles_per_split);
+  const int t_beg = min(n_tiles_all, block_z * p.tiles_per_split);
   const int t_end = min(n_tiles_all, t_beg + p.tiles_per_split);
   const int row_beg = t_beg * kBK, rows = min(p.kseg[0], t_end * kBK) - row_beg;
   const int n_tiles = t_end - t_beg;
@@ -149,7 +264,7 @@
   else reduce(std::false_type{});
   __builtin_amdgcn_s_setprio(0);
   Probe::mark(2);
-  const size_t slab = static_cast<size_t>(problem) * p.n_splits + blockIdx.z;
+  const size_t slab = static_cast<size_t>(problem) * p.n_splits + block_z;
   write_tile<BM, BN, WM, WN>(p, lds, p.c + slab * p.ra * p.ldc, acc, m0, n0);
   Probe::mark(3);
   if (want_colsum) {
@@ -169,20 +284,15 @@
   int splits;
 };
 
-__global__ __launch_bounds__(kBlock) void reduce_slabs_kernel(const ReduceArgs p) {
-  __shared__ v4f part[4][64];
+__device__ __forceinline__ void reduce_slabs(const float* slabs, float* out, int n4, int splits, int block, v4f (*part)[64]) {
   const int col = threadIdx.x & 63, grp = threadIdx.x >> 6;
-  const int q = blockIdx.y;
-  const float* slabs = kernarg_entry<const float*>(offsetof(ReduceArgs, slabs), q);
-  float* out = kernarg_entry<float*>(offsetof(ReduceArgs, out), q);
-  const int n4 = kernarg_entry<int>(offsetof(ReduceArgs, n4), q);
-  const int i = blockIdx.x * 64 + col;
-  if (blockIdx.x * 64 >= n4) return;
+  const int i = block * 64 + col;
+  if (block * 64 >= n4) return;
   v4f acc = {0.f, 0.f, 0.f, 0.f};
   if (i < n4) {
     const v4f* src = reinterpret_cast<const v4f*>(slabs) + i;
 #pragma unroll 8
-    for (int s = grp; s < p.splits; s += 4) acc += src[static_cast<size_t>(s) * n4];
+    for (int s = grp; s < splits; s += 4) acc += src[static_cast<size_t>(s) * n4];
   }
   part[grp][col] = acc;
   __syncthreads();
@@ -192,8 +302,12 @@
   }
 }
 
-constexpr int kSkinnyMax = 9;
-constexpr int kSkinnyChunks = 512;
+__global__ __launch_bounds__(kBlock) void reduce_slabs_kernel(const ReduceArgs p) {
+  __shared__ v4f part[4][64];
+  const int q = blockIdx.y;
+  reduce_slabs(kernarg_entry<const float*>(offsetof(ReduceArgs, slabs), q), kernarg_entry<float*>(offsetof(ReduceArgs, out), q),
+               kernarg_entry<int>(offsetof(ReduceArgs, n4), q), p.splits, blockIdx.x, part);
+}
 
 template <int S>
 __global__ __launch_bounds__(kBlock) void skinny_wgrad_kernel(const float* __restrict__ skinny, int s_cols,
@@ -201,39 +315,31 @@
                                                              float* __restrict__ partial, int64_t m,
                                                              int w, int64_t rows_per_chunk) {
   __shared__ v4f red[kBlock];
-  const int cols4 = w >> 2;
-  const int lanes = cols4 >= kBlock ? 1 : kBlock / cols4;
-  const int rl = cols4 >= kBlock ? 0 : threadIdx.x / cols4;
-  const int64_t row0 = blockIdx.x * rows_per_chunk, row1 = min(m, row0 + rows_per_chunk);
-  for (int q0 = 0; q0 < cols4; q0 += kBlock) {
-    const int q = q0 + (cols4 >= kBlock ? threadIdx.x : threadIdx.x % cols4);
-    const bool live = q < cols4 && rl < lanes;
-    v4f acc[S];
-#pragma unroll
-    for (int i = 0; i < S; ++i) acc[i] = v4f{0.f, 0.f, 0.f, 0.f};
-    if (live) {
-#pragma unroll 4
-      for (int64_t row = row0 + rl; row < row1; row += lanes) {
-        const v4f f = *reinterpret_cast<const v4f*>(wide + static_cast<size_t>(row) * w + 4 * q);
-#pragma unroll
-        for (int i = 0; i < S; ++i) acc[i] += (i < s_cols ? skinny[row * s_cols + i] : 1.0f) * f;
-      }
-    }
-#pragma unroll
-    for (int i = 0; i < S; ++i) {
-      v4f total = acc[i];
-      if (lanes > 1) {
-        __syncthreads();
-        red[threadIdx.x] = acc[i];
-        __syncthreads();
-        if (rl == 0 && live) {
-          for (int l = 1; l < lanes; ++l) total += red[l * cols4 + q];
-        }
-      }
-      if (rl == 0 && live)
-        *reinterpret_cast<v4f*>(partial + (static_cast<size_t>(blockIdx.x) * S + i) * w + 4 * q) = total;
-    }
-  }
+  const float* col[S];
+  int stride[S];
+#pragma unroll
+  for (int i = 0; i < S; ++i) col[i] = skinny + i, stride[i] = s_cols;
+  const int64_t row0 = blockIdx.x * rows_per_chunk;
+  skinny_chunk<S, false>(wide, w, col, stride, s_cols < S, partial + static_cast<size_t>(blockIdx.x) * S * w, row0,
+                         min(m, row0 + rows_per_chunk), true, threadIdx.x, red);
+}
+
+__device__ __forceinline__ bool skinny_chunk_sum(const float* __restrict__ partial, int total_out, int chunks, int idx,
+                                                 float (*part)[16], float* sum) {
+  const int o = threadIdx.x & 15, lane = threadIdx.x >> 4;
+  float acc = 0.f;
+  if (idx < total_out) {
+#pragma unroll 8
+    for (int c = lane; c < chunks; c += 16) acc += partial[static_cast<size_t>(c) * total_out + idx];
+  }
+  part[lane][o] = acc;
+  __syncthreads();
+  if (lane != 0 || idx >= total_out) return false;
+  float total = part[0][o];
+#pragma unroll
+  for (int l = 1; l < 16; ++l) total += part[l][o];
+  *sum = total;
+  return true;
 }
 
 __global__ __launch_bounds__(kBlock) void skinny_sum_kernel(const float* __restrict__ partial,
@@ -241,25 +347,49 @@
                                                            float* __restrict__ dst1, int rows, int s_cols,
                                                            int w, int chunks, int transposed) {
   __shared__ float part[16][16];
-  const int o = threadIdx.x & 15, lane = threadIdx.x >> 4;
-  const int idx = blockIdx.x * 16 + o;
-  const int total_out = rows * w;
-  float acc = 0.f;
-  if (idx < total_out) {
-#pragma unroll 8
-    for (int c = lane; c < chunks; c += 16) acc += partial[static_cast<size_t>(c) * total_out + idx];
-  }
-  part[lane][o] = acc;
-  __syncthreads();
-  if (lane != 0 || idx >= total_out) return;
-  float sum = part[0][o];
-#pragma unroll
-  for (int l = 1; l < 16; ++l) sum += part[l][o];
+  const int idx = blockIdx.x * 16 + (threadIdx.x & 15);
+  float sum;
+  if (!skinny_chunk_sum(partial, rows * w, chunks, idx, part, &sum)) return;
   const int i = idx / w, j = idx - i * w;
   if (i < s_cols)
     dst0[transposed ? j * s_cols + i : i * w + j] = sum;
   else if (dst1 != nullptr)
     dst1[j] = sum;
+}
+
+struct FinishArgs {
+  const float* slabs[2 * kMaxProblems];
+  float* out[2 * kMaxProblems];
+  int n4[2 * kMaxProblems];
+  int splits, slab_blocks_x, slab_blocks;
+  const float* partial[kNarrowPasses];
+  float* dst[kNarrowPasses * kSkinnyMax];
+  int dst_stride[kNarrowPasses * kSkinnyMax];
+  int rows[kNarrowPasses], w[kNarrowPasses];
+  int first_block[kNarrowPasses + 1];
+  int chunks, n_passes;
+};
+
+__global__ __launch_bounds__(kBlock) void wgrad_finish_kernel(const FinishArgs p) {
+  __shared__ v4f lds[4][64];
+  if (static_cast<int>(blockIdx.x) < p.slab_blocks) {
+    const int q = blockIdx.x / p.slab_blocks_x;
+    reduce_slabs(kernarg_entry<const float*>(offsetof(FinishArgs, slabs), q), kernarg_entry<float*>(offsetof(FinishArgs, out), q),
+                 kernarg_entry<int>(offsetof(FinishArgs, n4), q), p.splits, blockIdx.x - q * p.slab_blocks_x, lds);
+    return;
+  }
+  const int b = blockIdx.x - p.slab_blocks;
+  int s = 0;
+  while (s + 1 < p.n_passes && b >= kernarg_entry<int>(offsetof(FinishArgs, first_block), s + 1)) ++s;
+  const float* partial = kernarg_entry<const float*>(offsetof(FinishArgs, partial), s);
+  const int w = kernarg_entry<int>(offsetof(FinishArgs, w), s);
+  const int total_out = kernarg_entry<int>(offsetof(FinishArgs, rows), s) * w;
+  const int idx = (b - kernarg_entry<int>(offsetof(FinishArgs, first_block), s)) * 16 + (threadIdx.x & 15);
+  float sum;
+  if (!skinny_chunk_sum(partial, total_out, p.chunks, idx, reinterpret_cast<float(*)[16]>(lds), &sum)) return;
+  const int i = idx / w, j = idx - i * w;
+  float* dst = kernarg_entry<float*>(offsetof(FinishArgs, dst), s * kSkinnyMax + i);
+  dst[static_cast<size_t>(j) * kernarg_entry<int>(offsetof(FinishArgs, dst_stride), s * kSkinnyMax + i)] = sum;
 }
 
 inline int64_t skinny_workspace_floats(int64_t m, int64_t n, int64_t k) {
@@ -311,11 +441,13 @@
   int variant, bm, bn, splits;
 };
 
+constexpr int kStreamTileSlots = 256;
+
 inline void wgrad_candidate(int variant, int64_t k, int* bm, int* bn, int64_t* slots) {
   *bm = 128, *bn = k <= 64 ? 64 : 128, *slots = 512;
   if (k <= 64) return;
   if (variant == 2) *bn = 256;
-  if (variant == 4 || variant == 6) *bm = 256, *bn = 256, *slots = 256;
+  if (variant == 4 || variant == 6) *bm = 256, *bn = 256, *slots = kStreamTileSlots;
 }
 
 inline WgradPlan wgrad_plan(int64_t m, int64_t n, int64_t k, int n_problems) {
@@ -344,7 +476,16 @@
   return best;
 }
 
-inline int launch_wgrad(const GemmArgs& p, const WgradPlan& plan, hipStream_t st) {
+inline int stream_tile_groups(const GemmArgs& p, const WgradPlan& plan, int* free_slots) {
+  *free_slots = 0;
+  if (p.rb <= 64 || plan.variant != 6) return 0;
+  const int64_t groups = static_cast<int64_t>((p.ra + 255) / 256) * ((p.rb + 255) / 256) * p.n_problems * plan.splits;
+  if (groups < kStreamTileSlots) *free_slots = static_cast<int>(kStreamTileSlots - groups);
+  return static_cast<int>(groups);
+}
+
+inline int launch_wgrad(const GemmArgs& p, const WgradPlan& plan, hipStream_t st, const NarrowArgs* narrow = nullptr,
+                        int riders = 0) {
   const int np = p.n_problems, splits = plan.splits;
   if (p.rb <= 64) return launch_tiles<128, 64, 2, 2, false, false>(p, np, splits, st);
   switch (plan.variant) {
@@ -353,13 +494,100 @@
     case 6: {
       GemmArgs q = p;
       q.tiles_n = (p.rb + 255) / 256;
-      dim3 grid((p.ra + 255) / 256, q.tiles_n * np, splits);
-      wgrad_stream_kernel<><<<grid, 1024, 0, st>>>(q);
+      int free_slots;
+      const int groups = stream_tile_groups(p, plan, &free_slots);
+      wgrad_stream_kernel<><<<groups + (narrow ? riders : 0), 1024, 0, st>>>(q, narrow ? *narrow : NarrowArgs{});
       return launch_status();
     }
     default: return launch_tiles<128, 128, 2, 4, false, false>(p, np, splits, st);
   }
 }
 
-}
-}
+static_assert(GTS_WGRAD_NARROW_SIDE + 1 == kSkinnyMax, "a narrow side and the ones column fill a pass");
+inline bool narrow_problem(int64_t n, int64_t k) {
+  return (n < k ? n : k) <= GTS_WGRAD_NARROW_SIDE && (n < k ? k : n) >= GTS_WGRAD_NARROW_WIDE;
+}
+
+inline void narrow_chunking(int64_t m, int64_t* rows_per_chunk, int* chunks) {
+  *rows_per_chunk = (m + kSkinnyChunks - 1) / kSkinnyChunks;
+  *chunks = static_cast<int>((m + *rows_per_chunk - 1) / *rows_per_chunk);
+}
+
+inline int64_t narrow_workspace_floats(int64_t m, int64_t n, int64_t k) {
+  int64_t rpc;
+  int chunks;
+  narrow_chunking(m, &rpc, &chunks);
+  const int64_t small = n < k ? n : k, big = n < k ? k : n;
+  return chunks * ((small + 1) * big + (n < k ? n : 0));
+}
+
+struct NarrowPlan {
+  NarrowArgs run;
+  FinishArgs finish;
+  int n_passes;
+  int64_t offset[kNarrowPasses], floats;
+  void bind(float* partials) {
+    for (int s = 0; s < n_passes; ++s) run.partial[s] = partials + offset[s], finish.partial[s] = run.partial[s];
+  }
+};
+
+inline void plan_narrow(const float* const* g, const float* const* a, float* const* gw, float* const* gb, const int64_t* n,
+                        const int64_t* k, int count, int64_t m, NarrowPlan* plan) {
+  *plan = NarrowPlan{};
+  NarrowArgs& run = plan->run;
+  FinishArgs& fin = plan->finish;
+  float* ones_dst[kNarrowPasses] = {};
+  int loaded[kNarrowPasses] = {};
+  int np = 0;
+  auto pass_for = [&](const float* wide, int w, int s_cols, bool want_ones) {
+    for (int s = 0; s < np; ++s) {
+      const bool has_ones = ones_dst[s] != nullptr;
+      if (run.wide[s] == wide && run.w[s] == w && !(has_ones && want_ones) &&
+          loaded[s] + s_cols + (has_ones || want_ones ? 1 : 0) <= kSkinnyMax)
+        return s;
+    }
+    run.wide[np] = wide, run.w[np] = w;
+    return np++;
+  };
+  for (int q = 0; q < count; ++q) {
+    const bool g_is_skinny = n[q] < k[q];
+    const float* skinny = g_is_skinny ? g[q] : a[q];
+    const int s_cols = static_cast<int>(g_is_skinny ? n[q] : k[q]), w = static_cast<int>(g_is_skinny ? k[q] : n[q]);
+    float* bias = gb ? gb[q] : nullptr;
+    const bool want_ones = !g_is_skinny && bias != nullptr;
+    const int s = pass_for(g_is_skinny ? a[q] : g[q], w, s_cols, want_ones);
+    for (int i = 0; i < s_cols; ++i) {
+      const int at = s * kSkinnyMax + loaded[s]++;
+      run.col[at] = skinny + i, run.stride[at] = s_cols;
+      if (gw != nullptr) fin.dst[at] = g_is_skinny ? gw[q] + static_cast<size_t>(i) * w : gw[q] + i;
+      fin.dst_stride[at] = g_is_skinny ? 1 : s_cols;
+    }
+    if (want_ones) ones_dst[s] = bias;
+    if (g_is_skinny && bias != nullptr) ones_dst[pass_for(g[q], static_cast<int>(n[q]), 0, true)] = bias;
+  }
+  int64_t rpc;
+  int chunks;
+  narrow_chunking(m, &rpc, &chunks);
+  int blocks = 0;
+  for (int s = 0; s < np; ++s) {
+    run.rows[s] = run.loaded[s] = loaded[s];
+    if (ones_dst[s] != nullptr) {
+      fin.dst[s * kSkinnyMax + run.rows[s]] = ones_dst[s], fin.dst_stride[s * kSkinnyMax + run.rows[s]] = 1;
+      ++run.rows[s];
+    }
+    fin.rows[s] = run.rows[s], fin.w[s] = run.w[s];
+    fin.first_block[s] = blocks;
+    blocks += (run.rows[s] * run.w[s] + 15) / 16;
+    plan->offset[s] = plan->floats;
+    plan->floats += static_cast<int64_t>(chunks) * run.rows[s] * run.w[s];
+  }
+  fin.first_block[np] = blocks;
+  fin.chunks = chunks, fin.n_passes = np;
+  run.m = m, run.rows_per_chunk = rpc, run.chunks = chunks;
+  run.quads_per_pass = (chunks + kNarrowThreads / kBlock - 1) / (kNarrowThreads / kBlock);
+  run.n_quads = run.quads_per_pass * np;
+  plan->n_passes = np;
+}
+
+}
+}
diff --git a/gnn-tumor-seg_amd/csrc/gts_project.hip b/gnn-tumor-seg_amd/csrc/gts_project.hip
--- a/gnn-tumor-seg_amd/csrc/gts_project.hip
+++ b/gnn-tumor-seg_amd/csrc/gts_project.hip
@@ -172,7 +172,7 @@
 }
 }
 
-extern "C" int32_t gts_abi_version(void) { return 33; }
+extern "C" int32_t gts_abi_version(void) { return 34; }
 
 extern "C" const char* gts_error_string(int32_t code) {
   switch (code) {
diff --git a/gnn-tumor-seg_amd/csrc/gts_stack.hip b/gnn-tumor-seg_amd/csrc/gts_stack.hip
--- a/gnn-tumor-seg_amd/csrc/gts_stack.hip
+++ b/gnn-tumor-seg_amd/csrc/gts_stack.hip
@@ -82,6 +82,70 @@
   }
 };
 
+struct DeferredWgrads {
+  ByShape wide;
+  std::vector<const float*> ng, na;
+  std::vector<float*> ngw, ngb;
+  std::vector<int64_t> nn, nk;
+  void add(int64_t rows, int64_t cols, const float* g, const float* a, float* gw, float* gb) {
+    const bool narrow = std::min(rows, cols) <= GTS_WGRAD_NARROW_SIDE && std::max(rows, cols) >= GTS_WGRAD_NARROW_WIDE;
+    if (!narrow) return wide.add(rows, cols, g, a, gw, gb);
+    ng.push_back(g), na.push_back(a), ngw.push_back(gw), ngb.push_back(gb), nn.push_back(rows), nk.push_back(cols);
+  }
+  int n_narrow() const { return static_cast<int>(nn.size()); }
+  int joint() const {
+    int best = -1;
+    for (int i = 0; i < static_cast<int>(wide.groups.size()); ++i)
+      if (best < 0 || wide.groups[i].count() > wide.groups[best].count()) best = i;
+    return best;
+  }
+  int64_t workspace(int64_t n_rows) const {
+    int64_t ws = 0;
+    const int j = joint();
+    for (int i = 0; i < static_cast<int>(wide.groups.size()); ++i) {
+      const auto& grp = wide.groups[i];
+      for (int first = i == j ? gts::kMaxProblems : 0; first < grp.count(); first += gts::kMaxProblems)
+        ws = std::max(ws, gts_linear_bwd_weight_workspace(n_rows, grp.rows, grp.cols,
+                                                          std::min(gts::kMaxProblems, grp.count() - first)));
+    }
+    for (int first = 0; first < std::max(n_narrow(), 1); first += GTS_WGRAD_MAX_NARROW) {
+      const bool with_wide = first == 0 && j >= 0;
+      const int count = std::min(GTS_WGRAD_MAX_NARROW, n_narrow() - first);
+      if (count == 0 && !with_wide) break;
+      ws = std::max(ws, gts_wgrad_stack_workspace(n_rows, with_wide ? wide.groups[j].rows : 0, with_wide ? wide.groups[j].cols : 0,
+                                                  with_wide ? std::min(gts::kMaxProblems, wide.groups[j].count()) : 0,
+                                                  nn.data() + first, nk.data() + first, count));
+    }
+    return ws;
+  }
+  int32_t run(int64_t n_rows, float* workspace, int64_t workspace_bytes, void* stream) const {
+    const int j = joint();
+    for (int i = 0; i < static_cast<int>(wide.groups.size()); ++i) {
+      const auto& grp = wide.groups[i];
+      for (int first = i == j ? gts::kMaxProblems : 0; first < grp.count(); first += gts::kMaxProblems) {
+        const int32_t rc = gts_linear_bwd_weight_f32(grp.in[0].data() + first, grp.in[1].data() + first, grp.out[0].data() + first,
+                                                     grp.out[1].data() + first, std::min(gts::kMaxProblems, grp.count() - first),
+                                                     workspace, workspace_bytes, n_rows, grp.rows, grp.cols, stream);
+        if (rc != GTS_OK) return rc;
+      }
+    }
+    for (int first = 0; first < std::max(n_narrow(), 1); first += GTS_WGRAD_MAX_NARROW) {
+      const bool with_wide = first == 0 && j >= 0;
+      const int count = std::min(GTS_WGRAD_MAX_NARROW, n_narrow() - first);
+      if (count == 0 && !with_wide) break;
+      const ByShape::Group* grp = with_wide ? &wide.groups[j] : nullptr;
+      const int32_t rc = gts_wgrad_stack_f32(grp ? grp->in[0].data() : nullptr, grp ? grp->in[1].data() : nullptr,
+                                             grp ? grp->out[0].data() : nullptr, grp ? grp->out[1].data() : nullptr,
+                                             grp ? std::min(gts::kMaxProblems, grp->count()) : 0, grp ? grp->rows : 0,
+                                             grp ? grp->cols : 0, ng.data() + first, na.data() + first, ngw.data() + first,
+                                             ngb.data() + first, nn.data() + first, nk.data() + first, count, workspace,
+                                             workspace_bytes, n_rows, stream);
+      if (rc != GTS_OK) return rc;
+    }
+    return GTS_OK;
+  }
+};
+
 constexpr int kWeightSlot[3] = {0, 2, 3};
 inline int64_t weight_rows(const int64_t* w, int i, int q) { return q == 0 ? w[i] : w[i + 1]; }
 
@@ -89,7 +153,7 @@
   BwdPlan p{};
   int64_t at = 0, widest = 0;
   auto take = [&](int64_t bytes) { const int64_t o = at; at += align256(bytes); return o; };
-  ByShape wgrads;
+  DeferredWgrads wgrads;
   for (int i = 0; i < n_layers; ++i) {
     const int64_t fin = w[i];
     widest = std::max(widest, fin);
@@ -98,15 +162,12 @@
       p.wtp[i][q] = p.wt[i][q] >= 0 ? take(4 * gts_packed_weight_floats(fin, weight_rows(w, i, q))) : -1;
     p.g[i] = i > 0 ? take(4 * n * fin) : -1;
     p.gp[i] = take(4 * n * fin);
-    for (int q = 0; q < 3; ++q) wgrads.add(weight_rows(w, i, q), fin, nullptr, nullptr, nullptr, nullptr);
-  }
+  }
+  for (int i = n_layers - 1; i >= 0; --i)
+    for (int q = 0; q < 3; ++q) wgrads.add(weight_rows(w, i, q), w[i], nullptr, nullptr, nullptr, nullptr);
   p.gm[0] = take(4 * n * widest);
   p.gm[1] = take(4 * n * widest);
-  int64_t ws = 0;
-  if (n > 0)
-    for (const auto& grp : wgrads.groups)
-      for (int first = 0; first < grp.count(); first += gts::kMaxProblems)
-        ws = std::max(ws, gts_linear_bwd_weight_workspace(n, grp.rows, grp.cols, std::min(gts::kMaxProblems, grp.count() - first)));
+  const int64_t ws = n > 0 ? wgrads.workspace(n) : 0;
   p.workspace_bytes = ws;
   p.workspace = take(ws);
   p.counters = take(4 * GTS_CLUSTER_COUNTER_WORDS);
@@ -278,7 +339,7 @@
     return gts_linear_bwd_input_f32(g0, w0, g1, g1 ? w1 : nullptr, relu_mask, gin, n_rows, k, n0, g1 ? n1 : 0, stream);
   };
 
-  ByShape wgrads;
+  DeferredWgrads wgrads;
 
   const float* g = gout;
   const float* gm = nullptr;
@@ -326,10 +387,6 @@
       GTS_TRY(igrad(g, w_self, wt(i, 1), fout, gp, w_pool, wt(i, 0), fin, nullptr, nullptr, gx, fin, wtp(i, 1), wtp(i, 0)));
     }
   }
-  for (const auto& grp : wgrads.groups)
-    for (int first = 0; first < grp.count(); first += gts::kMaxProblems)
-      GTS_TRY(gts_linear_bwd_weight_f32(grp.in[0].data() + first, grp.in[1].data() + first, grp.out[0].data() + first,
-                                        grp.out[1].data() + first, std::min(gts::kMaxProblems, grp.count() - first),
-                                        f32(plan.workspace), plan.workspace_bytes, n_rows, grp.rows, grp.cols, stream));
+  GTS_TRY(wgrads.run(n_rows, f32(plan.workspace), plan.workspace_bytes, stream));
   return GTS_OK;
 }
diff --git a/gnn-tumor-seg_amd/gts/_lib.py b/gnn-tumor-seg_amd/gts/_lib.py
--- a/gnn-tumor-seg_amd/gts/_lib.py
+++ b/gnn-tumor-seg_amd/gts/_lib.py
@@ -5,7 +5,7 @@
 _HERE = os.path.dirname(os.path.abspath(__file__))
 LIB_PATH = os.environ.get("GTS_LIB_PATH") or os.path.join(_HERE, "libgts_hip.so")
 HEADER_PATH = os.path.join(os.path.dirname(os.path.dirname(_HERE)), "include", "gts_hip.h")
-ABI_VERSION = 33
+ABI_VERSION = 34
 
 _p = ctypes.c_void_p
 _i32 = ctypes.c_int32
diff --git a/gnn-tumor-seg_amd/gts/dense.py b/gnn-tumor-seg_amd/gts/dense.py
--- a/gnn-tumor-seg_amd/gts/dense.py
+++ b/gnn-tumor-seg_amd/gts/dense.py
@@ -368,6 +368,58 @@
     return out
 
 
+WGRAD_NARROW_SIDE = _lib.const("GTS_WGRAD_NARROW_SIDE")
+WGRAD_NARROW_WIDE = _lib.const("GTS_WGRAD_NARROW_WIDE")
+WGRAD_MAX_NARROW = _lib.const("GTS_WGRAD_MAX_NARROW")
+
+
+def wgrad_is_narrow(n, k):
+    return min(n, k) <= WGRAD_NARROW_SIDE and max(n, k) >= WGRAD_NARROW_WIDE
+
+
+def wgrad_stack(wide, narrow):
+    import ctypes
+
+    if len(wide) > MAX_WGRAD_PROBLEMS or len(narrow) > WGRAD_MAX_NARROW or not (wide or narrow):
+        raise _lib.GtsError(f"wgrad_stack takes up to {MAX_WGRAD_PROBLEMS} wide and {WGRAD_MAX_NARROW} narrow problems")
+    gs, acts = [g for g, _, _ in wide], [a for _, a, _ in wide]
+    ngs, nacts = [g for g, _, _ in narrow], [a for _, a, _ in narrow]
+    dev = _operands(*gs, *acts, *ngs, *nacts)
+    m = (gs + ngs)[0].shape[0]
+    n, k = (gs[0].shape[1], acts[0].shape[1]) if wide else (0, 0)
+    for g, a in zip(gs, acts):
+        if g.shape != (m, n) or a.shape != (m, k):
+            raise _lib.GtsError("batched weight gradients need identical shapes")
+    for g, a in zip(ngs, nacts):
+        if g.shape[0] != m or a.shape[0] != m or not wgrad_is_narrow(g.shape[1], a.shape[1]):
+            raise _lib.GtsError(f"a narrow weight gradient has {m} rows, a side of at most {WGRAD_NARROW_SIDE} and one of at least "
+                                f"{WGRAD_NARROW_WIDE}")
+
+    def outputs(problems):
+        gws = [torch.empty((g.shape[1], a.shape[1]), dtype=torch.float32, device=dev) for g, a, _ in problems]
+        gbs = [torch.empty(g.shape[1], dtype=torch.float32, device=dev) if want else None for g, _, want in problems]
+        return gws, gbs
+
+    (gws, gbs), (ngws, ngbs) = outputs(wide), outputs(narrow)
+    if m == 0:
+        for t in gws + ngws + [b for b in gbs + ngbs if b is not None]:
+            t.zero_()
+    else:
+        lib = _lib.load()
+        table = lambda ts: (ctypes.c_void_p * max(len(ts), 1))(*[ptr(t) for t in ts])
+        sizes = lambda ts: (ctypes.c_int64 * max(len(ts), 1))(*[t.shape[1] for t in ts])
+        nn, nk = sizes(ngs), sizes(nacts)
+        nbytes = lib.gts_wgrad_stack_workspace(m, n, k, len(wide), nn, nk, len(narrow))
+        ws = _gemm_ws.get(dev, nbytes)
+        flops = 2.0 * m * (n * k * len(wide) + sum(g.shape[1] * a.shape[1] for g, a in zip(ngs, nacts)))
+        _timed("wgrad", flops, lambda: check(
+            lib.gts_wgrad_stack_f32(table(gs), table(acts), table(gws), table(gbs), len(wide), n, k,
+                                    table(ngs), table(nacts), table(ngws), table(ngbs), nn, nk, len(narrow),
+                                    ptr(ws), ws.numel() * 4, m, current_stream()),
+            "gts_wgrad_stack_f32"))
+    return list(zip(gws, gbs)), list(zip(ngws, ngbs))
+
+
 def linear_bwd_weight(g, a, want_bias_grad=False):
     return linear_bwd_weight_multi([(g, a, want_bias_grad)])[0]
 
diff --git a/gnn-tumor-seg_amd/gts/nn.py b/gnn-tumor-seg_amd/gts/nn.py
--- a/gnn-tumor-seg_amd/gts/nn.py
+++ b/gnn-tumor-seg_amd/gts/nn.py
@@ -186,6 +186,7 @@
         g = gout.contiguous()
         gx = None
         deferred = {}
+        in_order = []
 
         turned, turned_fragment = _pack_by_shape(
             [w for w in (params[5 * i + j] for i in range(n) for j in (0, 2, 3))
@@ -201,6 +202,7 @@
         def defer(grad_out, act, slot, bias_slot):
             key = (grad_out.shape[1], act.shape[1])
             deferred.setdefault(key, []).append((grad_out, act, bias_slot is not None, slot, bias_slot))
+            in_order.append(deferred[key][-1])
 
         gm = None
         for i in reversed(range(n)):
@@ -224,12 +226,35 @@
                     g = igrad(g, w_self, gp, w_pool, relu_mask=h, relu_bits=hbits)
             elif ctx.needs_input_grad[1]:
                 gx = igrad(g, w_self, gp, w_pool)
-        for problems in deferred.values():
-            results = dense.linear_bwd_weight_multi([(go, act, want) for go, act, want, _, _ in problems])
+        def keep(results, problems):
             for (gw, gb), (_, _, _, slot, bias_slot) in zip(results, problems):
                 grads[slot] = gw
                 if bias_slot is not None:
                     grads[bias_slot] = gb
+
+        def multi(problems):
+            keep(dense.linear_bwd_weight_multi([(go, act, want) for go, act, want, _, _ in problems]), problems)
+
+        if any(dim % 4 for key in deferred for dim in key):
+            for problems in deferred.values():
+                multi(problems)
+            return (None, gx, None, *grads)
+        per_call = dense.WGRAD_MAX_NARROW
+        wide = {key: problems for key, problems in deferred.items() if not dense.wgrad_is_narrow(*key)}
+        narrow = [p for p in in_order if dense.wgrad_is_narrow(p[0].shape[1], p[1].shape[1])]
+        joint = max(wide, key=lambda key: len(wide[key]), default=None)
+        for key, problems in wide.items():
+            rest = problems[dense.MAX_WGRAD_PROBLEMS:] if key == joint else problems
+            for first in range(0, len(rest), dense.MAX_WGRAD_PROBLEMS):
+                multi(rest[first:first + dense.MAX_WGRAD_PROBLEMS])
+        for first in range(0, max(len(narrow), 1), per_call):
+            with_wide = wide[joint][:dense.MAX_WGRAD_PROBLEMS] if first == 0 and joint is not None else []
+            batch = narrow[first:first + per_call]
+            if not with_wide and not batch:
+                break
+            as_args = lambda problems: [(go, act, want) for go, act, want, _, _ in problems]
+            r_wide, r_narrow = dense.wgrad_stack(as_args(with_wide), as_args(batch))
+            keep(r_wide, with_wide), keep(r_narrow, batch)
         return (None, gx, None, *grads)
 
 
diff --git a/include/gts_hip.h b/include/gts_hip.h
--- a/include/gts_hip.h
+++ b/include/gts_hip.h
@@ -170,6 +170,19 @@
                                   float* const* gb, int32_t n_problems, float* workspace,
                                   int64_t workspace_bytes, int64_t m, int64_t n, int64_t k,
                                   void* stream);
+#define GTS_WGRAD_NARROW_SIDE 8
+#define GTS_WGRAD_NARROW_WIDE 64
+#define GTS_WGRAD_MAX_NARROW 8
+int64_t gts_wgrad_stack_workspace(int64_t m, int64_t n, int64_t k, int32_t n_wide, const int64_t* narrow_n,
+                                  const int64_t* narrow_k, int32_t n_narrow);
+int32_t gts_wgrad_stack_plan(int64_t m, int64_t n, int64_t k, int32_t n_wide, const float* const* narrow_g,
+                             const float* const* narrow_a, float* const* narrow_gb, const int64_t* narrow_n,
+                             const int64_t* narrow_k, int32_t n_narrow, int32_t* plan);
+int32_t gts_wgrad_stack_f32(const float* const* g, const float* const* a, float* const* gw, float* const* gb,
+                            int32_t n_wide, int64_t n, int64_t k, const float* const* narrow_g,
+                            const float* const* narrow_a, float* const* narrow_gw, float* const* narrow_gb,
+                            const int64_t* narrow_n, const int64_t* narrow_k, int32_t n_narrow, float* workspace,
+                            int64_t workspace_bytes, int64_t m, void* stream);
 
 int64_t gts_sage_pool_stack_fwd_arena(int64_t n_rows, const int64_t* widths, int32_t n_layers, int32_t training,
                                       int32_t arg_bytes, int32_t relu_bits, int64_t* offsets);
```

Measured after the change: 976.4 graphs/s, median of 6. 1.02x the previous value.
